# k-sheridan/ekf_vio

Hardware: AMD Instinct MI355X
Metric: filter steps/sec (predict+update) (higher is better)
Workload: dtype f32

## Files before the change

### ekf_vio_amd/capi.py

```python
import ctypes as C
import os

from . import _build

OK, EINVAL, ENUMERIC, ECAPACITY, EDEVICE, ESTATE, EABORTED = range(7)
_ERR = {EINVAL: "EKFVIO_EINVAL", ENUMERIC: "EKFVIO_ENUMERIC", ECAPACITY: "EKFVIO_ECAPACITY",
        EDEVICE: "EKFVIO_EDEVICE", ESTATE: "EKFVIO_ESTATE", EABORTED: "EKFVIO_EABORTED"}
PREDICT_STRUCTURED, PREDICT_DENSE = 0, 1


class Config(C.Structure):
    _fields_ = [("max_features", C.c_int32), ("default_point_depth", C.c_float),
                ("default_point_depth_variance", C.c_float), ("default_point_homogenous_variance", C.c_float),
                ("predict_mode", C.c_int32), ("klt_window_size", C.c_int32), ("klt_max_pyramid_level", C.c_int32),
                ("klt_max_iterations", C.c_int32), ("klt_epsilon", C.c_float), ("klt_min_eigen", C.c_float),
                ("kill_pad", C.c_int32), ("max_image_width", C.c_int32), ("max_image_height", C.c_int32),
                ("use_principal_point", C.c_int32), ("inverse_image_scale", C.c_int32), ("fast_threshold", C.c_int32),
                ("min_new_feature_dist", C.c_int32), ("fast_blur_sigma", C.c_float), ("replenish", C.c_int32),
                ("sample_based_uncertainty", C.c_int32), ("use_imu", C.c_int32), ("imu_gyro_variance", C.c_float),
                ("imu_accel_variance", C.c_float), ("gravity", C.c_float * 3),
                ("klt_fb_max_px", C.c_float), ("remove_lost", C.c_int32)]


class EkfvioError(RuntimeError):
    def __init__(self, code, msg=""):
        super().__init__("%s %s" % (_ERR.get(code, str(code)), msg))
        self.code = code


SYMBOLS = ["ekfvio_default_config", "ekfvio_create", "ekfvio_destroy", "ekfvio_reset", "ekfvio_last_error",
           "ekfvio_add_features", "ekfvio_process", "ekfvio_linearize", "ekfvio_update", "ekfvio_measurement_map",
           "ekfvio_num_features", "ekfvio_dim", "ekfvio_get_base_mu", "ekfvio_get_features", "ekfvio_get_sigma",
           "ekfvio_get_feature_cov", "ekfvio_get_depth_variance", "ekfvio_set_feature_cov", "ekfvio_metric2pixel_map",
           "ekfvio_pixel2metric_map", "ekfvio_get_odometry", "ekfvio_get_points", "ekfvio_check_sigma", "ekfvio_set_state",
           "ekfvio_remove_features", "ekfvio_klt_push_frame", "ekfvio_klt_track", "ekfvio_klt_track_points", "ekfvio_klt_get_level",
           "ekfvio_klt_uncertainty_points", "ekfvio_step_image", "ekfvio_replenish", "ekfvio_fast_detect", "ekfvio_imu", "ekfvio_imu_update",
           "ekfvio_upload_measurements", "ekfvio_run_uploaded", "ekfvio_synchronize", "ekfvio_profile_enable",
           "ekfvio_profile_reset", "ekfvio_profile_count", "ekfvio_profile_name", "ekfvio_profile_get",
           "ekfvio_profile_update_gemms", "ekfvio_get_counters", "ekfvio_set_gate", "ekfvio_get_gate",
           "ekfvio_set_klt_fb", "ekfvio_get_klt_fb", "ekfvio_klt_track_points_fb", "ekfvio_set_distortion", "ekfvio_rectify_map"]
HOOK_SYMBOLS = ["ekfvio_test_klt_padded_level", "ekfvio_test_blurred_level0", "ekfvio_test_gemm", "ekfvio_test_gemm_bench", "ekfvio_test_potrf_stamps",
                "ekfvio_test_sweep_stamps", "ekfvio_test_sweep_fault", "ekfvio_test_sweep_delay", "ekfvio_test_cholesky_solve", "ekfvio_test_plan", "ekfvio_test_persist_grid", "ekfvio_test_t2_pair",
                "ekfvio_test_gemm_plan", "ekfvio_test_predict_plan"]

_libs = {}


def lib_path():
    return _build.LIB_PATH


def load(build_if_missing=True, hooks=False):
    if hooks in _libs:
        return _libs[hooks]
    path = _build.HOOKS_LIB_PATH if hooks else _build.LIB_PATH
    if build_if_missing:
        _build.build(hooks=hooks)
    elif not os.path.exists(path):
        raise FileNotFoundError(path + " not built; run python -m ekf_vio_amd._build")
    lib = C.CDLL(path)
    vp, i32, f32 = C.c_void_p, C.c_int32, C.c_float
    fp, u8p, ip = C.POINTER(C.c_float), C.POINTER(C.c_uint8), C.POINTER(C.c_int32)
    sig = {
        "ekfvio_default_config": [C.POINTER(Config)],
        "ekfvio_create": [C.POINTER(Config), C.c_int, vp, C.POINTER(vp)],
        "ekfvio_destroy": [vp], "ekfvio_reset": [vp],
        "ekfvio_add_features": [vp, fp, i32], "ekfvio_process": [vp, f32], "ekfvio_linearize": [vp, f32, fp],
        "ekfvio_update": [vp, fp, fp, u8p, i32], "ekfvio_measurement_map": [vp, u8p, i32, ip, ip],
        "ekfvio_num_features": [vp], "ekfvio_dim": [vp], "ekfvio_get_base_mu": [vp, fp],
        "ekfvio_get_features": [vp, fp, fp, u8p], "ekfvio_get_sigma": [vp, fp, i32],
        "ekfvio_get_feature_cov": [vp, i32, fp], "ekfvio_get_depth_variance": [vp, i32, fp],
        "ekfvio_set_feature_cov": [vp, i32, fp], "ekfvio_metric2pixel_map": [fp, fp], "ekfvio_pixel2metric_map": [fp, fp],
        "ekfvio_get_odometry": [vp, fp, fp, fp, fp], "ekfvio_get_points": [vp, fp, fp],
        "ekfvio_check_sigma": [vp, fp, fp], "ekfvio_set_state": [vp, i32, fp, fp, fp, u8p, fp, i32],
        "ekfvio_remove_features": [vp, u8p, i32, ip],
        "ekfvio_klt_push_frame": [vp, u8p, i32, i32, i32, fp], "ekfvio_klt_track": [vp, fp, fp, u8p],
        "ekfvio_klt_track_points": [vp, fp, fp, i32, fp, u8p],
        "ekfvio_klt_uncertainty_points": [vp, fp, fp, i32, fp],
        "ekfvio_klt_get_level": [vp, i32, ip, ip, u8p, C.POINTER(C.c_int16)],
        "ekfvio_step_image": [vp, C.c_double, u8p, i32, i32, i32, fp], "ekfvio_imu": [vp, C.c_double, fp, fp], "ekfvio_imu_update": [vp, fp, fp],
        "ekfvio_replenish": [vp, ip, ip], "ekfvio_fast_detect": [vp, i32, i32, i32, ip, ip, ip],
        "ekfvio_upload_measurements": [vp, i32, fp, fp, u8p], "ekfvio_run_uploaded": [vp, i32, i32, f32],
        "ekfvio_synchronize": [vp], "ekfvio_profile_enable": [vp, i32], "ekfvio_profile_reset": [vp],
        "ekfvio_profile_count": [], "ekfvio_profile_name": [i32],
        "ekfvio_profile_get": [vp, i32, C.POINTER(C.c_double), C.POINTER(C.c_int64), C.POINTER(C.c_double)],
        "ekfvio_profile_update_gemms": [vp, i32, C.POINTER(C.c_double), C.POINTER(C.c_double)],
        "ekfvio_get_counters": [vp, C.POINTER(C.c_int64)],
        "ekfvio_set_gate": [vp, f32], "ekfvio_get_gate": [vp, fp, u8p, ip, ip, C.POINTER(C.c_int64)],
        "ekfvio_set_klt_fb": [vp, f32], "ekfvio_get_klt_fb": [vp, fp, u8p, ip, ip, C.POINTER(C.c_int64)],
        "ekfvio_klt_track_points_fb": [vp, fp, fp, i32, fp, u8p, fp, fp, u8p],
        "ekfvio_set_distortion": [vp, C.POINTER(C.c_double), i32],
        "ekfvio_rectify_map": [fp, C.POINTER(C.c_double), i32, i32, i32, ip, ip],
    }
    if hooks:
        sig.update({
            "ekfvio_test_klt_padded_level": [vp, i32, ip, u8p, C.POINTER(C.c_int16)],
            "ekfvio_test_blurred_level0": [vp, u8p],
            "ekfvio_test_gemm": [vp, i32, i32, i32, i32, f32, fp, i32, fp, i32, f32, fp, i32, i32],
            "ekfvio_test_cholesky_solve": [vp, i32, i32, fp, fp, fp, fp, ip],
            "ekfvio_test_potrf_stamps": [vp, C.POINTER(C.c_int64)],
            "ekfvio_test_sweep_stamps": [vp, C.c_int, C.POINTER(C.c_int64)],
            "ekfvio_test_sweep_fault": [vp, i32, i32],
            "ekfvio_test_sweep_delay": [vp, i32, i32, i32],
            "ekfvio_test_gemm_bench": [vp, i32, i32, i32, i32, i32, i32, i32, C.POINTER(C.c_double)],
            "ekfvio_test_plan": [i32] * 8 + [f32, ip],
            "ekfvio_test_persist_grid": [i32] * 8 + [f32, ip, i32, ip],
            "ekfvio_test_t2_pair": [i32, ip],
            "ekfvio_test_gemm_plan": [i32] * 11 + [ip],
            "ekfvio_test_predict_plan": [i32] * 5 + [ip],
        })
    for name, args in sig.items():
        fn = getattr(lib, name)
        fn.argtypes = args
        fn.restype = C.c_int
    lib.ekfvio_last_error.argtypes = [vp]
    lib.ekfvio_last_error.restype = C.c_char_p
    lib.ekfvio_profile_name.restype = C.c_char_p
    _libs[hooks] = lib
    return lib
```

### ekf_vio_amd/csrc/api.hip

```cpp
#include <math.h>
#include <stdio.h>
#include <string.h>

#include <algorithm>
#include <atomic>
#include <chrono>

#include <unistd.h>

#include "common.h"

namespace {
template <class T>
hipError_t dev_alloc(hipStream_t s, T** p, size_t count) {
    hipError_t e = hipMalloc((void**)p, sizeof(T) * (count ? count : 1));
    if (e == hipSuccess) e = hipMemsetAsync(*p, 0, sizeof(T) * (count ? count : 1), s);
    return e;
}

__global__ void init_sigma_kernel(float* P, int ld) {
    int i = threadIdx.x;
    if (i >= 7 && i <= 15) P[(size_t)i * ld + i] = 30.f;
    if (i >= 16 && i <= 21) P[(size_t)i * ld + i] = 0.5f;
}
// ... 122 lines not shown
    c->imu_gyro_variance = 1e-4f;
    c->imu_accel_variance = 1e-2f;
    c->gravity[0] = 0.f;
    c->gravity[1] = 9.81f;
    c->gravity[2] = 0.f;
    c->klt_fb_max_px = 0.f;
    c->remove_lost = 0;
    return EKFVIO_OK;
}

static int create_body(ekfvio_filter* f, const ekfvio_config* cfg, int device, void* stream) {
    HIP_TRY(f, hipSetDevice(device));
    if (stream) {
        f->stream = (hipStream_t)stream;
    } else {
        HIP_TRY(f, hipStreamCreateWithFlags(&f->stream, hipStreamNonBlocking));
        f->own_stream = true;
    }
    const int maxf = cfg->max_features;
    const FilterDims dims = filter_dims(maxf);
    f->n_cap = dims.n_cap, f->ldp = dims.ldp, f->m_cap = dims.m_cap, f->ld_aug = dims.ld_aug, f->sweep_sync_words = dims.sweep_sync_words;
    f->tune = tuning_from_env();
    const size_t pp = (size_t)f->ldp * f->ldp, pm = (size_t)f->ldp * f->m_cap;
    HIP_TRY(f, dev_alloc(f->stream, &f->mu, f->ldp));
    HIP_TRY(f, dev_alloc(f->stream, &f->mu_next, f->ldp));
    HIP_TRY(f, dev_alloc(f->stream, &f->last_klt, 2 * (size_t)maxf));
    HIP_TRY(f, dev_alloc(f->stream, &f->del_flag, (size_t)maxf));
    HIP_TRY(f, dev_alloc(f->stream, &f->P, pp));
    HIP_TRY(f, dev_alloc(f->stream, &f->P2, pp));
    HIP_TRY(f, dev_alloc(f->stream, &f->FA, EKF_BASE * EKF_BASE));
    HIP_TRY(f, dev_alloc(f->stream, &f->FB, 27 * (size_t)maxf));
    HIP_TRY(f, dev_alloc(f->stream, &f->FD, 9 * (size_t)maxf));
    HIP_TRY(f, dev_alloc(f->stream, &f->Fdense, pp));
    HIP_TRY(f, dev_alloc(f->stream, &f->idx, (size_t)f->m_cap));
    HIP_TRY(f, dev_alloc(f->stream, &f->inv_idx, (size_t)f->ldp));
    HIP_TRY(f, dev_alloc(f->stream, &f->zmeas, 2 * (size_t)maxf));
    HIP_TRY(f, dev_alloc(f->stream, &f->Rmeas, 4 * (size_t)maxf));
    HIP_TRY(f, dev_alloc(f->stream, &f->pass, (size_t)maxf));
    HIP_TRY(f, dev_alloc(f->stream, &f->yres, (size_t)f->m_cap));
    HIP_TRY(f, dev_alloc(f->stream, &f->Rm, 2 * (size_t)f->m_cap));
    HIP_TRY(f, dev_alloc(f->stream, &f->Saug, (size_t)f->ld_aug * f->m_cap));
    HIP_TRY(f, dev_alloc(f->stream, &f->Laug, (size_t)f->ld_aug * f->m_cap));
    HIP_TRY(f, dev_alloc(f->stream, &f->Linv, 64 * (size_t)f->m_cap));
    HIP_TRY(f, dev_alloc(f->stream, &f->Lsign, (size_t)(f->m_cap / 64 > 256 ? f->m_cap / 64 : 256)));
    HIP_TRY(f, dev_alloc(f->stream, &f->sweep_sync, f->sweep_sync_words));
    {
        hipDeviceProp_t prop;
        HIP_TRY(f, hipGetDeviceProperties(&prop, device));
        f->num_cus = prop.multiProcessorCount;
    }
    HIP_TRY(f, dev_alloc(f->stream, &f->Km, pm));
    HIP_TRY(f, dev_alloc(f->stream, &f->Wt, pm));
    HIP_TRY(f, dev_alloc(f->stream, &f->Gm, pm));
    HIP_TRY(f, dev_alloc(f->stream, &f->info, 4));
    HIP_TRY(f, dev_alloc(f->stream, &f->remove_words, 4));
    HIP_TRY(f, hipHostMalloc((void**)&f->h_info, 16 * sizeof(int), hipHostMallocMapped | hipHostMallocCoherent));
    memset(f->h_info, 0, 16 * sizeof(int));
    HIP_TRY(f, hipHostGetDevicePointer((void**)&f->d_hinfo, f->h_info, 0));
    {
        const size_t words = EKF_BASE + 4 * (size_t)(f->cfg.max_features > 0 ? f->cfg.max_features : 1);
        HIP_TRY(f, hipHostMalloc((void**)&f->h_out, words * sizeof(float), hipHostMallocMapped | hipHostMallocCoherent));
        HIP_TRY(f, hipHostGetDevicePointer((void**)&f->d_out, f->h_out, 0));
    }
    {
        const size_t cap = (size_t)(f->cfg.max_features > 0 ? f->cfg.max_features : 1);
        HIP_TRY(f, hipHostMalloc((void**)&f->h_meas, 25 * cap, hipHostMallocDefault));
        HIP_TRY(f, hipMalloc((void**)&f->d_meas, 25 * cap));
    }
    HIP_TRY(f, hipEventCreate(&f->ev0));
    HIP_TRY(f, hipEventCreate(&f->ev1));
    int rc = klt_alloc(f);
    if (rc != EKFVIO_OK) return rc;
    rc = fast_alloc(f);
    if (rc != EKFVIO_OK) return rc;
    return ekfvio_reset(f);
}

}

static std::atomic<int>* live_registry() {
    static std::atomic<int>* reg = [] {
        char name[64], val[32];
        snprintf(name, sizeof(name), "EKFVIO_LIVE_HANDLES_%ld", (long)getpid());
        if (const char* e = getenv(name)) {
            void* p = nullptr;
            if (sscanf(e, "%p", &p) == 1 && p) return static_cast<std::atomic<int>*>(p);
        }
        auto* a = new std::atomic<int>[64];
        for (int i = 0; i < 64; i++) a[i].store(0, std::memory_order_relaxed);
        snprintf(val, sizeof(val), "%p", static_cast<void*>(a));
        setenv(name, val, 1);
        return a;
    }();
    return reg;
}
int live_handles_on(int device) { return (device >= 0 && device < 64) ? live_registry()[device].load(std::memory_order_relaxed) : 2; }

extern "C" {

int ekfvio_create(const ekfvio_config* cfg, int device, void* stream, ekfvio_filter** out) {
    if (!out) return EKFVIO_EINVAL;
    *out = nullptr;
    if (!cfg || cfg->max_features < 0) return EKFVIO_EINVAL;
    if (cfg->remove_lost != 0 && cfg->remove_lost != 1) return EKFVIO_EINVAL;
    if (cfg->remove_lost && (size_t)cfg->max_features * 17 > 64 * 1024) return EKFVIO_ECAPACITY;
    if (!(cfg->klt_fb_max_px >= 0.f)) return EKFVIO_EINVAL;
    int ndev = 0;
    if (hipGetDeviceCount(&ndev) != hipSuccess || device < 0 || device >= ndev) return EKFVIO_EDEVICE;
    ekfvio_filter* f = new ekfvio_filter();
    f->cfg = *cfg;
    f->device = device;
    if (device < 64) live_registry()[device].fetch_add(1, std::memory_order_relaxed);
    const int rc = create_body(f, cfg, device, stream);
    if (rc != EKFVIO_OK) {
        fprintf(stderr, "ekfvio_create: %s\n", f->last_error.c_str());
        (void)ekfvio_destroy(f);
        return rc;
    }
    *out = f;
    return EKFVIO_OK;
}

int ekfvio_destroy(ekfvio_filter* f) {
    if (!f) return EKFVIO_EINVAL;
    (void)hipSetDevice(f->device);
    if (f->stream) (void)hipStreamSynchronize(f->stream);
    void* ptrs[] = {f->mu, f->mu_next, f->last_klt, f->del_flag, f->P,  f->P2, f->FA, f->FB, f->FD,   f->Fdense,
                    f->idx, f->inv_idx, f->zmeas,  f->Rmeas,    f->pass,     f->yres, f->Rm, f->Saug,  f->Laug,  f->Linv, f->Lsign, f->Km, f->sweep_sync, f->sweep_dbg,
                    f->Wt,  f->Gm,     f->info,     f->remove_words, f->seq_z,    f->seq_R, f->seq_pass, f->gate_words, f->fb_words};
    for (void* p : ptrs)
        if (p) hipFree(p);
    if (f->h_info) hipHostFree(f->h_info);
    if (f->h_out) hipHostFree(f->h_out);
    if (f->h_meas) hipHostFree(f->h_meas);
    if (f->d_meas) (void)hipFree(f->d_meas);
    klt_free(f);
    fast_free(f);
    drop_graph(f);
    if (f->ev0) hipEventDestroy(f->ev0);
    if (f->ev1) hipEventDestroy(f->ev1);
    if (f->own_stream && f->stream) hipStreamDestroy(f->stream);
    if (f->device >= 0 && f->device < 64) live_registry()[f->device].fetch_sub(1, std::memory_order_relaxed);
    delete f;
    return EKFVIO_OK;
}

const char* ekfvio_last_error(const ekfvio_filter* f) {
    return f ? f->last_error.c_str() : "null handle (a failed ekfvio_create leaves none behind: its return code says why)";
}

int ekfvio_reset(ekfvio_filter* f) {
    if (!f) return EKFVIO_EINVAL;
    f->out_fresh = false;
    HIP_TRY(f, hipSetDevice(f->device));
    f->N = 0;
    f->n = EKF_BASE;
    HIP_TRY(f, hipMemsetAsync(f->P, 0, sizeof(float) * (size_t)f->ldp * f->ldp, f->stream));
    HIP_TRY(f, hipMemsetAsync(f->P2, 0, sizeof(float) * (size_t)f->ldp * f->ldp, f->stream));
    HIP_TRY(f, hipMemsetAsync(f->mu, 0, sizeof(float) * f->ldp, f->stream));
    const float one = 1.f;
    HIP_TRY(f, hipMemcpyAsync(f->mu + 3, &one, sizeof(float), hipMemcpyHostToDevice, f->stream));
    hipLaunchKernelGGL(init_sigma_kernel, dim3(1), dim3(32), 0, f->stream, f->P, f->ldp);
    HIP_TRY(f, hipMemsetAsync(f->info, 0, 4 * sizeof(int), f->stream));
    if (f->gate_words) HIP_TRY(f, hipMemsetAsync(f->gate_words, 0, 4 * sizeof(int), f->stream));
    if (f->fb_words) HIP_TRY(f, hipMemsetAsync(f->fb_words, 0, 8 * sizeof(int), f->stream));
    HIP_TRY(f, hipStreamSynchronize(f->stream));
    f->have_stamp = false;
    f->frames[0].valid = f->frames[1].valid = false;
    return EKFVIO_OK;
}

int ekfvio_add_features(ekfvio_filter* f, const float* uv, int32_t count) {
    if (!f || count < 0 || (count > 0 && !uv)) return EKFVIO_EINVAL;
    f->out_fresh = false;
    if (count == 0) return EKFVIO_OK;
    if (f->N + count > f->cfg.max_features) return EKFVIO_ECAPACITY;
    HIP_TRY(f, hipSetDevice(f->device));
    HIP_TRY(f, hipMemcpyAsync(f->zmeas, uv, sizeof(float) * 2 * count, hipMemcpyHostToDevice, f->stream));
    return add_features_device(f, count);
}

int ekfvio_process(ekfvio_filter* f, float dt) {
// ... 654 lines not shown
    long long* dst;
    HIP_TRY(f, dev_alloc(f->stream, &dS, hs.size()));
    HIP_TRY(f, dev_alloc(f->stream, &dL, hs.size()));
    HIP_TRY(f, dev_alloc(f->stream, &dLi, 4096));
    HIP_TRY(f, dev_alloc(f->stream, &dst, 80));
    HIP_TRY(f, hipMemsetAsync(dst, 0, sizeof(long long) * 80, f->stream));
    HIP_TRY(f, hipMemcpyAsync(dS, hs.data(), sizeof(float) * hs.size(), hipMemcpyHostToDevice, f->stream));
    for (int rep = 0; rep < 3; rep++) launch_potrf_stamps(f, dS, 64, dL, dLi, dst);
    HIP_TRY(f, hipMemcpyAsync(stamps, dst, sizeof(long long) * 80, hipMemcpyDeviceToHost, f->stream));
    std::vector<uint32_t> hl(64 * 64), hi(4096);
    HIP_TRY(f, hipMemcpyAsync(hl.data(), dL, sizeof(float) * hl.size(), hipMemcpyDeviceToHost, f->stream));
    HIP_TRY(f, hipMemcpyAsync(hi.data(), dLi, sizeof(float) * hi.size(), hipMemcpyDeviceToHost, f->stream));
    HIP_TRY(f, hipStreamSynchronize(f->stream));
    uint64_t h1 = 1469598103934665603ull, h2 = h1;
    for (uint32_t v : hl) h1 = (h1 ^ v) * 1099511628211ull;
    for (uint32_t v : hi) h2 = (h2 ^ v) * 1099511628211ull;
    stamps[12] = (int64_t)h1;
    stamps[13] = (int64_t)h2;
    hipFree(dS); hipFree(dL); hipFree(dLi); hipFree(dst);
    return EKFVIO_OK;
}

int ekfvio_test_sweep_stamps(ekfvio_filter* f, int enable, int64_t* stamps ) {
    if (!f) return EKFVIO_EINVAL;
    HIP_TRY(f, hipSetDevice(f->device));
    if (enable && !f->sweep_dbg) {
        HIP_TRY(f, dev_alloc(f->stream, &f->sweep_dbg, 1024));
        HIP_TRY(f, hipMemsetAsync(f->sweep_dbg, 0, 1024 * sizeof(long long), f->stream));
    }
    if (stamps && f->sweep_dbg) {
        HIP_TRY(f, hipMemcpyAsync(stamps, f->sweep_dbg, 1024 * sizeof(long long), hipMemcpyDeviceToHost, f->stream));
        HIP_TRY(f, hipStreamSynchronize(f->stream));
    }
    return EKFVIO_OK;
}

int ekfvio_test_sweep_fault(ekfvio_filter* f, int32_t spin_limit, int32_t stall_workgroup) {
    if (!f || spin_limit < 0) return EKFVIO_EINVAL;
    f->sweep_spin_limit = spin_limit;
    f->sweep_stall_wg = stall_workgroup;
    drop_graph(f);
    return EKFVIO_OK;
}

int ekfvio_test_sweep_delay(ekfvio_filter* f, int32_t workgroup, int32_t point, int32_t ticks) {
    if (!f || (point != 0 && point != 1) || ticks < 0 || ticks > EKFVIO_TEST_SWEEP_DELAY_MAX_TICKS) return EKFVIO_EINVAL;
    f->sweep_delay_wg = workgroup >= 0 ? workgroup : -1;
    f->sweep_delay_point = point;
    f->sweep_delay_ticks = ticks;
    drop_graph(f);
    return EKFVIO_OK;
}

int ekfvio_test_cholesky_solve(ekfvio_filter* f, int32_t m, int32_t nrhs, const float* S, const float* Crhs,
                               float* L_out, float* X_out, int32_t* info) {
    if (!f || m <= 0 || nrhs <= 0 || !S || !Crhs) return EKFVIO_EINVAL;
    HIP_TRY(f, hipSetDevice(f->device));
    const int mp = round_up(m, 64), rp = round_up(nrhs, 64);
    const int ld = mp + rp + mp;
    std::vector<float> hs((size_t)ld * mp, 0.f);
    for (int c = 0; c < mp; c++) {
        for (int r = 0; r < mp; r++) hs[(size_t)c * ld + r] = (r < m && c < m) ? S[(size_t)c * m + r] : (r == c ? 1.f : 0.f);
        if (c < m)
            for (int r = 0; r < nrhs; r++) hs[(size_t)c * ld + mp + r] = Crhs[(size_t)c * nrhs + r];
        hs[(size_t)c * ld + mp + rp + c] = 1.f;
    }
    float *dS, *dL, *dLi, *dK, *dW;
    HIP_TRY(f, dev_alloc(f->stream, &dS, hs.size()));
    HIP_TRY(f, dev_alloc(f->stream, &dL, hs.size()));
    HIP_TRY(f, dev_alloc(f->stream, &dLi, (size_t)64 * mp));
    HIP_TRY(f, dev_alloc(f->stream, &dK, (size_t)rp * mp));
    HIP_TRY(f, dev_alloc(f->stream, &dW, (size_t)rp * mp));
    HIP_TRY(f, hipMemcpyAsync(dS, hs.data(), sizeof(float) * hs.size(), hipMemcpyHostToDevice, f->stream));
    UpdatePlan plan = plan_raw_sweep(f->tune, plan_shape(f), mp, rp);
    launch_chol_sweep(f, plan, dS, dL, dLi, ld, plan.persistent() && !f->sweep_flags_clean);
    if (plan.persistent()) f->sweep_flags_clean = false;
    std::vector<unsigned long long> hsign(mp / 64);
    HIP_TRY(f, hipMemcpyAsync(hsign.data(), f->Lsign, sizeof(unsigned long long) * hsign.size(), hipMemcpyDeviceToHost, f->stream));
    HIP_TRY(f, hipStreamSynchronize(f->stream));
    int refine = 1;
    for (unsigned long long v : hsign) refine &= (v == 0ull);
    if (refine) plan.gain = GAIN_GEMM;
    launch_gain_from_sweep(f, plan, dL, ld, nrhs, dK, dW, rp, refine);
    std::vector<float> hl(hs.size()), hk((size_t)rp * mp);
    HIP_TRY(f, hipMemcpyAsync(hl.data(), dL, sizeof(float) * hl.size(), hipMemcpyDeviceToHost, f->stream));
    HIP_TRY(f, hipMemcpyAsync(hk.data(), dK, sizeof(float) * hk.size(), hipMemcpyDeviceToHost, f->stream));
    if (info) {
        HIP_TRY(f, hipMemcpyAsync(info, f->info, sizeof(int), hipMemcpyDeviceToHost, f->stream));
        HIP_TRY(f, hipMemsetAsync(f->info, 0, sizeof(int), f->stream));
    }
    HIP_TRY(f, hipStreamSynchronize(f->stream));
    if (const char* dp = getenv("EKFVIO_DEBUG_DUMP_LAUG")) {
        if (FILE* fp = fopen(dp, "wb")) {
            const int hdr[3] = {ld, mp, rp};
            fwrite(hdr, sizeof(int), 3, fp);
            fwrite(hl.data(), sizeof(float), hl.size(), fp);
            fclose(fp);
        }
    }
    if (L_out)
        for (int c = 0; c < m; c++)
            for (int r = 0; r < m; r++) L_out[(size_t)c * m + r] = (r >= c) ? hl[(size_t)c * ld + r] : 0.f;
    if (X_out)
        for (int c = 0; c < m; c++)
            for (int r = 0; r < nrhs; r++) X_out[(size_t)c * nrhs + r] = hk[(size_t)c * rp + r];
    hipFree(dS);
// ... 77 lines not shown
```

### ekf_vio_amd/csrc/chol.hip

```cpp
#include "common.h"

#include <type_traits>

namespace {

typedef float f32x16 __attribute__((ext_vector_type(16)));
typedef float f32x4 __attribute__((ext_vector_type(4)));

#define PB 64
#ifndef PLD
#define PLD 68
#endif
#define ILD 17
#define INV_LDS (4 * 16 * ILD)

__device__ __forceinline__ float lane_bcast(float v, int src_lane) {
    return __int_as_float(__builtin_amdgcn_readlane(__float_as_int(v), src_lane));
}
__device__ __forceinline__ double lane_bcast_d(double v, int src_lane) {
    const int lo = __builtin_amdgcn_readlane(__double2loint(v), src_lane);
    const int hi = __builtin_amdgcn_readlane(__double2hiint(v), src_lane);
    return __hiloint2double(hi, lo);
}

// ... 830 lines not shown
    for (int c = 0; c < PB; c++)
        if ((neg >> c) & 1ull) {
            float* p = L + (size_t)(blockIdx.y * PB + c) * ldl + row0 + r;
            *p = -*p;
        }
}


#define SWEEP_SPIN_LIMIT (1 << 30)
#define SWEEP_WAIT_TICKS_UNRECOVERABLE 10000000

#include "chol_persist.inc"
#include "chol_step_la.inc"

}

#ifdef EKFVIO_TEST_HOOKS
void launch_potrf_stamps(ekfvio_filter* f, const float* S, int ld, float* L, float* Linv, long long* d_stamps) {
    const char* e = getenv("EKFVIO_POTRF_FV");
    const int fv = e ? atoi(e) : EKF_POTRF_FV;
    auto kern = fv == 0 ? potrf64_stamp_kernel<0> : fv == 10 ? potrf64_stamp_kernel<10> : fv == 12 ? potrf64_stamp_kernel<12>
              : fv == 13 ? potrf64_stamp_kernel<13> : potrf64_stamp_kernel<8>;
    const char* w = getenv("EKFVIO_POTRF_WARM");
    hipLaunchKernelGGL(kern, dim3(1), dim3(256), 0, f->stream, S, ld, L, ld, Linv, d_stamps, (w && atoi(w)) ? 2 : 1);
}
#endif

#define EKF_GATHER_POTRF_LDS (84 * 1024)
void launch_gather_potrf(ekfvio_filter* f, const UpdatePlan& p) {
    if (!f->gather_attr_set) {
        (void)hipFuncSetAttribute(reinterpret_cast<const void*>(gather_potrf_kernel), hipFuncAttributeMaxDynamicSharedMemorySize,
                                  EKF_GATHER_POTRF_LDS);
        f->gather_attr_set = true;
    }
    GatherArgs ga = make_gather_args(f, p);
    if (p.persistent()) {
        ga.zero_words = f->sweep_sync;
        ga.n_zero = (int)persist_flag_words(p.m_pad, p.n_pad);
    }
    const int nb2 = p.with_wt ? (p.m_pad / 64) * (f->ldp / 64) : 0;
    hipLaunchKernelGGL(gather_potrf_kernel, dim3(1 + ga.nb1 + nb2), dim3(256), EKF_GATHER_POTRF_LDS, f->stream, ga, f->Laug, f->ld_aug,
                       f->Linv, f->info, f->Lsign, f->sweep_dbg);
}

static PersistArgs persist_args(ekfvio_filter* f, const UpdatePlan& p, float* L, int ldl, float* K, int ldk, float* S = nullptr,
                                float* Linv = nullptr) {
    PersistArgs pa = PersistArgs();
    const PersistGrid g = persist_grid(p, f->ldp);
    const PersistFlags fl(p.m_pad, p.n_pad);
    const int mb = g.mb, nX = g.nX;
    pa.L = L, pa.ldl = ldl, pa.mb = mb, pa.idb0 = mb + nX, pa.grid = g;
    pa.K = K, pa.ldk = ldk, pa.Lsign = f->Lsign;
    pa.Sg = f->P, pa.ldsg = f->ldp, pa.T2 = t2_buffer(f), pa.ldt = f->ldp, pa.nstate = f->n;
    if (!S) return pa;
    pa.S = S, pa.lds = ldl, pa.Linv = Linv, pa.info = f->info;
    pa.ready = f->sweep_sync + fl.ready(), pa.fin = f->sweep_sync + fl.fin(), pa.pan = f->sweep_sync + fl.pan(), pa.abort_flag = f->sweep_sync + fl.abort_word();
    pa.dbg = f->sweep_dbg;
    pa.bound.spin_limit = f->sweep_spin_limit > 0 ? f->sweep_spin_limit : SWEEP_SPIN_LIMIT;
    pa.bound.wait_ticks = p.recoverable ? f->tune.sweep_wait_ticks : std::max(f->tune.sweep_wait_ticks, SWEEP_WAIT_TICKS_UNRECOVERABLE);
    pa.early_sources = f->tune.persist_early;
    pa.stall_wg = f->sweep_stall_wg >= 0 ? g.owner_block(f->sweep_stall_wg - 1) : -1;
#ifdef EKFVIO_TEST_HOOKS
    pa.delay_wg = f->sweep_delay_wg >= 0 ? g.owner_block(f->sweep_delay_wg - 1) : -1;
    pa.delay_point = f->sweep_delay_point, pa.delay_ticks = f->sweep_delay_ticks;
#endif
    return pa;
}

#define EKF_PERSIST_FUSED_DYN_LDS (28 * 1024)
const int* launch_persist_fused(ekfvio_filter* f, const UpdatePlan& p, bool zero_flags) {
    const int m_pad = p.m_pad, n_pad = p.n_pad;
    ProfScope ps(f, PC_CHOL, (double)m_pad * m_pad * m_pad / 3.0 + (double)(n_pad + m_pad / 2) * m_pad * m_pad);
    if (!f->persist_attr_set) {
        (void)hipFuncSetAttribute(reinterpret_cast<const void*>(chol_persist_kernel), hipFuncAttributeMaxDynamicSharedMemorySize,
                                  EKF_PERSIST_FUSED_DYN_LDS);
        f->persist_attr_set = true;
    }
    PersistArgs pa = persist_args(f, p, f->Laug, f->ld_aug, f->Km, f->ldp, f->Saug, f->Linv);
    pa.gain = p.gain == GAIN_SWEEP, pa.t2 = p.t2_by_sweep;
    if (zero_flags) (void)hipMemsetAsync(f->sweep_sync, 0, sizeof(int) * persist_flag_words(m_pad, n_pad), f->stream);
    hipLaunchKernelGGL(chol_persist_kernel, dim3(pa.grid.total()), dim3(256), EKF_PERSIST_FUSED_DYN_LDS,
                       f->stream, pa, make_gather_args(f, p));
    f->persistent_sweeps++;
    return pa.abort_flag;
}

const int* launch_chol_sweep(ekfvio_filter* f, const UpdatePlan& p, float* Saug, float* Laug, float* Linv, int ld, bool zero_flags) {
    const int m_pad = p.m_pad, n_pad = p.n_pad;
    const bool schur = p.sweep == SWEEP_SCHUR, split = p.sweep == SWEEP_SPLIT || p.sweep == SWEEP_SPLIT_LA;
    ProfScope ps(f, PC_CHOL, (double)m_pad * m_pad * m_pad / 3.0 + (double)(n_pad + m_pad / 2) * m_pad * m_pad +
                                 (schur ? (double)n_pad * n_pad * m_pad + (double)n_pad * m_pad * m_pad : 0.0));
    const int mb = m_pad / PB, idb0 = mb + n_pad / PB;
    const int rb = n_pad / PB + mb;
    if (!p.fused_gather)
        hipLaunchKernelGGL(potrf64_kernel, dim3(1), dim3(256), 0, f->stream, Saug, ld, Laug, ld, Linv, f->info, f->Lsign);
    if (p.sweep == SWEEP_PERSIST) {
        const PersistArgs pa = persist_args(f, p, Laug, ld, nullptr, 0, Saug, Linv);
        if (zero_flags) (void)hipMemsetAsync(f->sweep_sync, 0, sizeof(int) * persist_flag_words(m_pad, n_pad), f->stream);
        hipLaunchKernelGGL(chol_persist_kernel, dim3(pa.grid.total()), dim3(256), 0, f->stream, pa, GatherArgs());
        f->persistent_sweeps++;
        return pa.abort_flag;
    }
    SchurArgs sc;
    if (schur) {
        f->schur_sweeps++;
        sc.P = f->P, sc.ldp = f->ldp, sc.K = f->Km, sc.ldk = f->ldp, sc.nb = n_pad / PB;
// ... 43 lines not shown
}

__global__ __launch_bounds__(256) void joseph_g_kernel(float* __restrict__ K, int ldk, const float* __restrict__ T, int ldp,
                                                       const int* __restrict__ idx, const float* __restrict__ Rm,
                                                       const float* __restrict__ zrow, const float* __restrict__ mu, int m,
                                                       const int* __restrict__ m_dev, float* __restrict__ G, int ldg,
                                                       float* __restrict__ Kyp) {
    __shared__ float s_t[64 * 65];
    __shared__ float s_part[4][64];
    if (m_dev) m = *m_dev;
    const int rl = threadIdx.x & 63, ph = threadIdx.x >> 6;
    const int i0 = blockIdx.x * 64, c0 = blockIdx.y * 64;
    const int i = i0 + rl;
    float kq[16], kp[16];
#pragma unroll
    for (int u = 0; u < 16; u++) {
        const int q = c0 + ph + 4 * u;
        kq[u] = K[(size_t)q * ldk + i];
        kp[u] = K[(size_t)(q ^ 1) * ldk + i];
    }
    {
        const int q = c0 + rl;
        const int sq = (q < m) ? idx[q] : 0;
        float tv[16];
#pragma unroll
        for (int u = 0; u < 16; u++) tv[u] = T[(size_t)(i0 + ph + 4 * u) * ldp + sq];
#pragma unroll
        for (int u = 0; u < 16; u++) s_t[(ph + 4 * u) * 65 + rl] = tv[u];
    }
    __syncthreads();
    float acc = 0.f;
#pragma unroll
    for (int u = 0; u < 16; u++) {
        const int q = c0 + ph + 4 * u;
        const float a = (fabsf(kq[u]) > EKF_FLUSH_THRESH) ? kq[u] : 0.f;
        const float b = (fabsf(kp[u]) > EKF_FLUSH_THRESH) ? kp[u] : 0.f;
        K[(size_t)q * ldk + i] = a;
        float g = 0.f;
        if (q < m) {
            const float x = a * Rm[2 * q], y = b * Rm[2 * (q ^ 1) + 1];
            const float kr = ((q ^ 1) < q) ? (y + x) : (x + y);
            g = kr - s_t[rl * 65 + ph + 4 * u];
            acc = acc + a * (zrow[q] - mu[idx[q]]);
        }
        G[(size_t)q * ldg + i] = g;
    }
    s_part[ph][rl] = acc;
    __syncthreads();
    if (ph == 0) Kyp[(size_t)blockIdx.y * ldg + i] = ((s_part[0][rl] + s_part[1][rl]) + s_part[2][rl]) + s_part[3][rl];
}

void launch_gain2_tiles(ekfvio_filter* f, const UpdatePlan& p) {
    const int m_pad = p.m_pad, n_pad = p.n_pad;
    ProfScope ps(f, PC_SOLVE, 2.0 * n_pad * (double)m_pad * m_pad + (double)n_pad * n_pad * m_pad);
    const PersistArgs pa = persist_args(f, p, f->Laug, f->ld_aug, f->Km, f->ldp);
    const int gain_wgs = pa.grid.nX * pa.mb;
    const int total = gain_wgs + t2_pairs(pa.grid.nX);
    const int dyn = total <= f->num_cus ? 30 * 1024 : 0;
    if (dyn && !f->gain2_attr_set) {
        (void)hipFuncSetAttribute(reinterpret_cast<const void*>(gain2_t2_tiles_kernel), hipFuncAttributeMaxDynamicSharedMemorySize, 30 * 1024);
        f->gain2_attr_set = true;
    }
    hipLaunchKernelGGL(gain2_t2_tiles_kernel, dim3(total), dim3(256), dyn, f->stream, pa, make_gather_args(f, p), gain_wgs);
}

void launch_joseph_g(ekfvio_filter* f, int m, int m_pad, int n_pad, bool m_on_device, const float* T) {
    ProfScope ps(f, PC_SOLVE, 3.0 * n_pad * (double)m_pad);
    hipLaunchKernelGGL(joseph_g_kernel, dim3(n_pad / 64, m_pad / 64), dim3(256), 0, f->stream, f->Km, f->ldp, T ? T : f->P, f->ldp, f->idx,
                       f->Rm, f->yres, f->mu, m, m_on_device ? f->info + 2 : nullptr, f->Gm, f->ldp, f->Wt);
}

void launch_gain_from_sweep(ekfvio_filter* f, const UpdatePlan& p, const float* Laug, int ld, int n, float* K, float* scratch, int ldk, int refine) {
    const int m_pad = p.m_pad, n_pad = p.n_pad;
    ProfScope ps(f, PC_SOLVE, (refine ? 3.0 : 1.0) * n * (double)m_pad * m_pad);
    if (p.gain == GAIN_TILES) {
        const PersistArgs pa = persist_args(f, p, const_cast<float*>(Laug), ld, K, ldk);
        hipLaunchKernelGGL(gain_tiles_kernel, dim3((n_pad / PB) * pa.mb), dim3(256), 0, f->stream, pa);
        return;
    }
    const float* Lf = Laug;
    const float* Y = Laug + m_pad;
    const float* LinvT = Laug + m_pad + n_pad;
    GemmCall g;
    g.M = n, g.N = g.K = m_pad, g.transB = true, g.lowerB = true;
    g.A = Y, g.lda = ld, g.B = LinvT, g.ldb = ld, g.C = K, g.ldc = ldk, g.flush = !refine;
    launch_gemm(f, g);
    if (refine) {
        GemmCall r = g;
        r.transB = false, r.alpha = -1.f, r.A = K, r.lda = ldk, r.B = Lf, r.beta = 1.f, r.Cin = Y, r.ldcin = ld, r.C = scratch, r.flush = false;
        launch_gemm(f, r);
        g.A = scratch, g.lda = ldk, g.beta = 1.f, g.Cin = K, g.ldcin = ldk, g.flush = true;
        launch_gemm(f, g);
    }
}
```

### ekf_vio_amd/csrc/chol_persist.inc

```

#ifndef PERSIST_POLL_SLEEP_LAZY
#define PERSIST_POLL_SLEEP_LAZY 12
#endif
#ifndef PERSIST_POLL_SLEEP
#define PERSIST_POLL_SLEEP 2
#endif

struct PollBound {
    int spin_limit, wait_ticks;
};
struct PersistArgs {
    float* S;
    int lds;
    float* L;
    int ldl;
    float* Linv;
    int mb, idb0;
    int* info;
    unsigned long long* Lsign;
    int* ready;
    int* fin;
    int* abort_flag;
    long long* dbg;
    PersistGrid grid;
    int gain;
    float* K;
    int ldk;
    int* pan;
    int early_sources;
    PollBound bound;
    int stall_wg;
    int t2;
    const float* Sg;
    int ldsg;
    float* T2;
    int ldt;
    int nstate;
#ifdef EKFVIO_TEST_HOOKS
    int delay_wg;
    int delay_point;
    int delay_ticks;
#endif
};

typedef unsigned int u32x4 __attribute__((ext_vector_type(4)));
__device__ __forceinline__ __amdgpu_buffer_rsrc_t persist_rsrc(const float* p, unsigned floats) {
    return __builtin_amdgcn_make_buffer_rsrc(const_cast<float*>(p), 0, floats * 4u, 0x00020000);
}
__device__ __forceinline__ float4 ld_sc1(__amdgpu_buffer_rsrc_t b, unsigned off) {
    const f32x4 v = __builtin_bit_cast(f32x4, __builtin_amdgcn_raw_buffer_load_b128(b, off * 4u, 0, 16));
    return make_float4(v[0], v[1], v[2], v[3]);
}
__device__ __forceinline__ void st_sc1(__amdgpu_buffer_rsrc_t b, unsigned off, float4 q) {
    const f32x4 v = {q.x, q.y, q.z, q.w};
    __builtin_amdgcn_raw_buffer_store_b128(__builtin_bit_cast(u32x4, v), b, off * 4u, 0, 16);
}
__device__ __forceinline__ void wait_vm0() { asm volatile("s_waitcnt vmcnt(0)" ::: "memory"); }

struct RegTile {
    float4 v[4];
    __device__ __forceinline__ void request(__amdgpu_buffer_rsrc_t b, unsigned base, int ld, int tid) {
#pragma unroll
        for (int it = 0; it < 4; it++) {
            const int e = tid + it * 256;
            v[it] = ld_sc1(b, base + (unsigned)(e >> 4) * (unsigned)ld + (unsigned)(e & 15) * 4u);
        }
    }
    __device__ __forceinline__ void put(float* T, int tid) const {
#pragma unroll
        for (int it = 0; it < 4; it++) {
            const int e = tid + it * 256;
            *reinterpret_cast<float4*>(T + (e >> 4) * PLD + (e & 15) * 4) = v[it];
        }
    }
};
__device__ __forceinline__ void inv_put(float4 v, float* Tinv, int tid) {
    const int p = tid >> 6, c = (tid >> 2) & 15, r4 = (tid & 3) * 4;
    float* t = Tinv + p * 16 * ILD + c * ILD + r4;
    t[0] = v.x; t[1] = v.y; t[2] = v.z; t[3] = v.w;
}
__device__ __forceinline__ void load_tile_sc1(float* T, __amdgpu_buffer_rsrc_t b, unsigned base, int ld, int tid) {
    RegTile t;
    t.request(b, base, ld, tid);
    t.put(T, tid);
}
__device__ __forceinline__ void load_inv_sc1(float* Tinv, __amdgpu_buffer_rsrc_t b, unsigned base, int tid) {
    inv_put(ld_sc1(b, base + tid * 4), Tinv, tid);
}
template <bool LOWER>
__device__ __forceinline__ void store_tile_sc1(const float* T, __amdgpu_buffer_rsrc_t b, unsigned base, int ld, int tid) {
#pragma unroll
    for (int it = 0; it < 4; it++) {
        const int e = tid + it * 256;
        const int c = e >> 4, r4 = (e & 15) * 4;
        const float4 q = *reinterpret_cast<const float4*>(T + c * PLD + r4);
// ... 102 lines not shown
    const __amdgpu_buffer_rsrc_t bL = persist_rsrc(a.L, (unsigned)ldl * (unsigned)(mb * PB));
    float kv[16];
#pragma unroll
    for (int q = 0; q < 16; q++) kv[q] = 0.f;
    const int iy = mb + ib, iz = a.idb0 + cb;
    for (int kb = cb; kb < mb; kb++) {
        bool signed_last = false;
        unsigned long long negl = 0ull;
        if (kb == mb - 1) {
            const __amdgpu_buffer_rsrc_t bS = persist_rsrc(a.S, (unsigned)a.lds * (unsigned)(mb * PB));
            const __amdgpu_buffer_rsrc_t bI = persist_rsrc(a.Linv, (unsigned)(mb * PB * PB));
            const bool zi = a.grid.compact() && cb == kb;
            persist_wait(a, nullptr, a.fin + iy * mb + kb, zi ? nullptr : a.fin + iz * mb + kb, tid, 1, true);
            load_tile_sc1(Ti, bS, (unsigned)(kb * PB) * (unsigned)a.lds + (unsigned)(iy * PB), a.lds, tid);
            if (zi) identity_tile(Tj, tid);
            else load_tile_sc1(Tj, bS, (unsigned)(kb * PB) * (unsigned)a.lds + (unsigned)(iz * PB), a.lds, tid);
            persist_wait(a, a.ready + kb, nullptr, nullptr, tid, 4, false);
            load_tile_sc1(Tl, bL, (unsigned)(kb * PB) * (unsigned)ldl + (unsigned)(kb * PB), ldl, tid);
            load_inv_sc1(Tinv, bI, (unsigned)(kb * PB * PB), tid);
            negl = ld_sign_sc1(a.Lsign + kb);
            __syncthreads();
            tri_solve_fwd2(Ti, Tj, Tl, Tinv, wave, lane);
            if (a.dbg && tid == 0 && ib * mb + cb < 104) a.dbg[400 + ib * mb + cb] = (long long)__builtin_amdgcn_s_memrealtime();
            signed_last = negl != 0ull;
        } else {
            persist_wait(a, nullptr, a.pan + iy * mb + kb, a.pan + iz * mb + kb, tid, 1, true);
            load_tile_sc1(Ti, bL, (unsigned)(kb * PB) * (unsigned)ldl + (unsigned)(iy * PB), ldl, tid);
            load_tile_sc1(Tj, bL, (unsigned)(kb * PB) * (unsigned)ldl + (unsigned)(iz * PB), ldl, tid);
        }
        __syncthreads();
        const f32x16 up = signed_last ? mma64_signed(Ti, 1, PLD, Tj, 1, PLD, wr, wc, lane, negl) : mma64(Ti, 1, PLD, Tj, 1, PLD, wr, wc, lane);
#pragma unroll
        for (int q = 0; q < 16; q++) kv[q] = kv[q] + up[q];
    }
    float* Kt = a.K + (size_t)(cb * PB) * a.ldk + (size_t)ib * PB;
#pragma unroll
    for (int q = 0; q < 16; q++) {
        const int c = mma64_col(wc, lane, q);
        Kt[(size_t)c * a.ldk + r] = (fabsf(kv[q]) > EKF_FLUSH_THRESH) ? kv[q] : 0.f;
    }
}

__device__ __forceinline__ void sign_cols(float* dst, const float* src, unsigned long long neg, int tid) {
#pragma unroll
    for (int it = 0; it < 4; it++) {
        const int e = tid + it * 256;
        const int c = e >> 4, r4 = (e & 15) * 4;
        const float sg = ((neg >> c) & 1ull) ? -1.f : 1.f;
        const float4 v = *reinterpret_cast<const float4*>(src + c * PLD + r4);
        *reinterpret_cast<float4*>(dst + c * PLD + r4) = make_float4(sg * v.x, sg * v.y, sg * v.z, sg * v.w);
    }
}

template <bool WAIT>
__device__ __forceinline__ void gain_tile2(const PersistArgs& a, const GatherArgs& ga, float* Ti, float* Tj, float* Tl, float* Tinv, float* Th, float* tab,
                                           int ib, int cb, int tid) {
    const int lane = tid & 63, wave = tid >> 6, wr = wave & 1, wc = wave >> 1;
    const int r = wr * 32 + (lane & 31);
    const int mb = a.mb, ldl = a.ldl;
    const int m = ga.m_dev ? *ga.m_dev : ga.m;
    const __amdgpu_buffer_rsrc_t bL = persist_rsrc(a.L, (unsigned)ldl * (unsigned)(mb * PB));
    const __amdgpu_buffer_rsrc_t bS = persist_rsrc(a.S, (unsigned)a.lds * (unsigned)(mb * PB));
    const int iy = mb + ib, iz = a.idb0 + cb;
    const int cq = cb * PB + lane;
    const int sq = (cq < m) ? ga.idx[cq] : -1;
    const unsigned sqc = (unsigned)max(sq, 0);
    int alo = 0, ahi = -1;
    if (cb * PB < m) {
        alo = ga.idx[cb * PB] / PB;
        ahi = ga.idx[min(cb * PB + PB - 1, m - 1)] / PB;
    }
    if (tid < 64) {
        float yq = 0.f, rd = 0.f, ro = 0.f;
        if (sq >= 0) {
            yq = ga.zrow[cq] - ga.mu[sq];
            rd = ga.Rm[2 * cq];
            ro = ga.Rm[2 * (cq ^ 1) + 1];
        }
        tab[tid] = yq, tab[64 + tid] = rd, tab[128 + tid] = ro;
    }
    auto column_flags = [&](int kb, const int* zflag) -> PollLane {
        const int ax = alo + tid - 2;
        return {tid == 0 ? a.pan + iy * mb + kb : tid == 1 ? zflag : (tid >= 2 && ax <= ahi) ? a.pan + (mb + ax) * mb + kb : nullptr, 1};
    };
    float kv[16], w2[16];
    {
        float wv[16];
        const int scl = max(sq, 0);
#pragma unroll
        for (int ps = 0; ps < 16; ps++) wv[ps] = ga.P[(size_t)min(ib * PB + wave + 4 * ps, ga.n - 1) * ga.ld + scl];
#pragma unroll
        for (int ps = 0; ps < 16; ps++) asm volatile("" : "+v"(wv[ps]));
#pragma unroll
        for (int ps = 0; ps < 16; ps++) Th[(wave + 4 * ps) * 65 + lane] = (sq >= 0 && ib * PB + wave + 4 * ps < ga.n) ? wv[ps] : 0.f;
        __syncthreads();
#pragma unroll
        for (int q = 0; q < 16; q++) {
            kv[q] = 0.f;
            w2[q] = Th[r * 65 + mma64_col(wc, lane, q)];
        }
    }
    auto fetch = [&](int kb) -> unsigned long long {
        const bool gk = kb >= cb;
        float hv[16];
        unsigned long long neg;
        if constexpr (WAIT) {
            persist_wait(a, column_flags(kb, gk ? a.pan + iz * mb + kb : nullptr), tid, kb < mb - 2);
            load_tile_sc1(Ti, bL, (unsigned)(kb * PB) * (unsigned)ldl + (unsigned)(iy * PB), ldl, tid);
            if (gk) load_tile_sc1(Tj, bL, (unsigned)(kb * PB) * (unsigned)ldl + (unsigned)(iz * PB), ldl, tid);
#pragma unroll
            for (int ps = 0; ps < 16; ps++)
                hv[ps] = __builtin_bit_cast(float, __builtin_amdgcn_raw_buffer_load_b32(bL, ((unsigned)(kb * PB + wave + 4 * ps) * (unsigned)ldl + (unsigned)(mb * PB) + sqc) * 4u, 0, 16));
#pragma unroll
            for (int ps = 0; ps < 16; ps++) hv[ps] = (sq >= 0) ? hv[ps] : 0.f;
#pragma unroll
            for (int ps = 0; ps < 16; ps++) Th[(wave + 4 * ps) * PLD + lane] = hv[ps];
            neg = ld_sign_sc1(a.Lsign + kb);
        } else {
            load_tile(Ti, a.L + (size_t)kb * PB * ldl + (size_t)iy * PB, ldl, tid);
            if (gk) load_tile(Tj, a.L + (size_t)kb * PB * ldl + (size_t)iz * PB, ldl, tid);
#pragma unroll
            for (int ps = 0; ps < 16; ps++) hv[ps] = a.L[(size_t)(kb * PB + wave + 4 * ps) * ldl + (size_t)(mb * PB) + sqc];
#pragma unroll
            for (int ps = 0; ps < 16; ps++) hv[ps] = (sq >= 0) ? hv[ps] : 0.f;
#pragma unroll
            for (int ps = 0; ps < 16; ps++) Th[(wave + 4 * ps) * PLD + lane] = hv[ps];
            neg = a.Lsign[kb];
        }
        return neg;
    };
    auto products = [&](int kb, unsigned long long neg, bool z_unsigned) {
        if (kb >= cb) {
            const f32x16 up = (z_unsigned && neg != 0ull) ? mma64_signed(Ti, 1, PLD, Tj, 1, PLD, wr, wc, lane, neg) : mma64(Ti, 1, PLD, Tj, 1, PLD, wr, wc, lane);
#pragma unroll
            for (int q = 0; q < 16; q++) kv[q] = kv[q] + up[q];
        }
        if (alo <= ahi) {
            f32x16 up;
            if constexpr (WAIT) {
                up = (neg == 0ull) ? mma64(Ti, 1, PLD, Th, 1, PLD, wr, wc, lane) : mma64_signed(Ti, 1, PLD, Th, 1, PLD, wr, wc, lane, neg);
            } else {
                if (__builtin_amdgcn_readfirstlane((int)(neg != 0ull))) {
                    __syncthreads();
                    sign_cols(Ti, Ti, neg, tid);
                    __syncthreads();
                }
                up = mma64(Ti, 1, PLD, Th, 1, PLD, wr, wc, lane);
            }
#pragma unroll
            for (int q = 0; q < 16; q++) w2[q] = w2[q] - up[q];
        }
        if (WAIT && a.dbg && tid == 0 && mb <= 8 && (ib == 0 || ib == 6) && (cb == 0 || cb == 3 || cb == 7))
            a.dbg[100 + 8 * ((ib ? 3 : 0) + (cb == 0 ? 0 : cb == 3 ? 1 : 2)) + kb] = (long long)__builtin_amdgcn_s_memrealtime();
    };
    if constexpr (WAIT) {
        for (int kb = 0; kb < mb - 2; kb++) {
            __syncthreads();
            const unsigned long long neg = fetch(kb);
            __syncthreads();
            products(kb, neg, false);
        }
    } else {
        for (int kb = 0; kb < mb; kb++) {
            __syncthreads();
            const unsigned long long neg = fetch(kb);
            __syncthreads();
            products(kb, neg, false);
        }
    }
    if constexpr (WAIT) {
        const int kl = mb - 1, k6 = mb - 2;
        const bool gk6 = k6 >= cb;
        const __amdgpu_buffer_rsrc_t bI = persist_rsrc(a.Linv, (unsigned)(mb * PB * PB));
        const bool zi = a.grid.compact() && cb == kl;
        __syncthreads();
        persist_wait(a, column_flags(k6, gk6 ? a.pan + iz * mb + k6 : (zi ? nullptr : a.fin + iz * mb + kl)), tid, false);
        RegTile ql, qi, qj;
        float hq[16];
        unsigned long long neg6;
        {
            RegTile pi6, pj6;
            float h6[16];
            pi6.request(bL, (unsigned)(k6 * PB) * (unsigned)ldl + (unsigned)(iy * PB), ldl, tid);
            if (gk6) pj6.request(bL, (unsigned)(k6 * PB) * (unsigned)ldl + (unsigned)(iz * PB), ldl, tid);
#pragma unroll
            for (int ps = 0; ps < 16; ps++)
                h6[ps] = __builtin_bit_cast(float, __builtin_amdgcn_raw_buffer_load_b32(bL, ((unsigned)(k6 * PB + wave + 4 * ps) * (unsigned)ldl + (unsigned)(mb * PB) + sqc) * 4u, 0, 16));
            neg6 = ld_sign_sc1(a.Lsign + k6);
            pi6.put(Ti, tid);
            if (gk6) pj6.put(Tj, tid);
#pragma unroll
            for (int ps = 0; ps < 16; ps++) Th[(wave + 4 * ps) * PLD + lane] = (sq >= 0) ? h6[ps] : 0.f;
        }
        persist_wait(a, a.ready + kl, nullptr, nullptr, tid, 4, false);
        ql.request(bL, (unsigned)(kl * PB) * (unsigned)ldl + (unsigned)(kl * PB), ldl, tid);
        qi.request(bS, (unsigned)(kl * PB) * (unsigned)a.lds + (unsigned)(iy * PB), a.lds, tid);
        if (!zi) qj.request(bS, (unsigned)(kl * PB) * (unsigned)a.lds + (unsigned)(iz * PB), a.lds, tid);
        const float4 qv = ld_sc1(bI, (unsigned)(kl * PB * PB) + tid * 4);
        const unsigned long long neg7 = ld_sign_sc1(a.Lsign + kl);
#pragma unroll
        for (int ps = 0; ps < 16; ps++)
            hq[ps] = __builtin_bit_cast(float, __builtin_amdgcn_raw_buffer_load_b32(bS, ((unsigned)(kl * PB + wave + 4 * ps) * (unsigned)a.lds + (unsigned)(mb * PB) + sqc) * 4u, 0, 16));
        products(mb - 2, neg6, false);
        __syncthreads();
        ql.put(Tl, tid);
        qi.put(Ti, tid);
        if (zi) identity_tile(Tj, tid);
        else qj.put(Tj, tid);
        inv_put(qv, Tinv, tid);
#pragma unroll
        for (int ps = 0; ps < 16; ps++) Th[(wave + 4 * ps) * PLD + lane] = (sq >= 0) ? hq[ps] : 0.f;
        __syncthreads();
        float* const t3[3] = {Ti, Tj, Th};
        tri_solve_fwd_n<3>(t3, Tl, Tinv, wave, lane);
        __syncthreads();
        products(kl, neg7, true);
    }
#pragma unroll
    for (int q = 0; q < 16; q++) kv[q] = (fabsf(kv[q]) > EKF_FLUSH_THRESH) ? kv[q] : 0.f;
    float* Kt = a.K + (size_t)(cb * PB) * a.ldk + (size_t)ib * PB;
    float* Gt = ga.G + (size_t)(cb * PB) * ga.ld + (size_t)ib * PB;
    float acc = 0.f;
#pragma unroll
    for (int q = 0; q < 16; q++) {
        const int c = mma64_col(wc, lane, q), cg = cb * PB + c;
        Kt[(size_t)c * a.ldk + r] = kv[q];
        float g = 0.f;
        if (cg < m) {
            const float x = kv[q] * tab[64 + c], y = kv[q ^ 1] * tab[128 + c];
            const float kr = ((cg ^ 1) < cg) ? (y + x) : (x + y);
            g = kr - w2[q];
            acc = acc + kv[q] * tab[c];
        }
        Gt[(size_t)c * ga.ld + r] = g;
    }
    __syncthreads();
    float* part = Th;
    part[(wc * 2 + (lane >> 5)) * 64 + r] = acc;
    __syncthreads();
    if (tid < 64) ga.Wt[(size_t)cb * ga.ld + (size_t)ib * PB + tid] = ((part[tid] + part[64 + tid]) + part[128 + tid]) + part[192 + tid];
}

template <bool WAIT>
__device__ __forceinline__ void t2_tile(const PersistArgs& a, float* Ti, float* Tj, float* Tl, float* Tinv, int ta, int tb, int tid, long long* dbg = nullptr) {
    const int lane = tid & 63, wave = tid >> 6, wr = wave & 1, wc = wave >> 1;
    const int r = wr * 32 + (lane & 31);
    const int mb = a.mb, ldl = a.ldl;
    const bool diag = ta == tb;
    const __amdgpu_buffer_rsrc_t bL = persist_rsrc(a.L, (unsigned)ldl * (unsigned)(mb * PB));
    float tab[16], tba[16];
    {
        const float* sab = a.Sg + (size_t)tb * PB * a.ldsg + (size_t)ta * PB;
        const float* sba = a.Sg + (size_t)ta * PB * a.ldsg + (size_t)tb * PB;
#pragma unroll
        for (int q = 0; q < 16; q++) {
            const int c = mma64_col(wc, lane, q);
            tab[q] = sab[(size_t)c * a.ldsg + r];
            tba[q] = diag ? 0.f : sba[(size_t)c * a.ldsg + r];
        }
    }
    const int ia = mb + ta, ib = mb + tb;
    auto apply = [&](int kb, unsigned long long neg) {
        const float* Bj = diag ? Ti : Tj;
        f32x16 up;
        if constexpr (WAIT) {
            up = (neg == 0ull) ? mma64(Ti, 1, PLD, Bj, 1, PLD, wr, wc, lane) : mma64_signed(Ti, 1, PLD, Bj, 1, PLD, wr, wc, lane, neg);
        } else if (__builtin_amdgcn_readfirstlane((int)(neg != 0ull))) {
            sign_cols(Tl, Ti, neg, tid);
            __syncthreads();
            up = mma64(Tl, 1, PLD, Bj, 1, PLD, wr, wc, lane);
            __syncthreads();
        } else {
            up = mma64(Ti, 1, PLD, Bj, 1, PLD, wr, wc, lane);
        }
#pragma unroll
        for (int q = 0; q < 16; q++) tab[q] = tab[q] - up[q];
        if (!diag) {
#pragma unroll
            for (int q = 0; q < 16; q++) Tl[r * PLD + mma64_col(wc, lane, q)] = up[q];
            __syncthreads();
#pragma unroll
            for (int q = 0; q < 16; q++) tba[q] = tba[q] - Tl[mma64_col(wc, lane, q) * PLD + r];
        }
        if (dbg && tid == 0) dbg[kb] = (long long)__builtin_amdgcn_s_memrealtime();
    };
    if constexpr (WAIT) {
        for (int kb = 0; kb < mb - 2; kb++) {
            __syncthreads();
            persist_wait(a, nullptr, a.pan + ia * mb + kb, diag ? nullptr : a.pan + ib * mb + kb, tid, 1, true);
            load_tile_sc1(Ti, bL, (unsigned)(kb * PB) * (unsigned)ldl + (unsigned)(ia * PB), ldl, tid);
            if (!diag) load_tile_sc1(Tj, bL, (unsigned)(kb * PB) * (unsigned)ldl + (unsigned)(ib * PB), ldl, tid);
            const unsigned long long neg = ld_sign_sc1(a.Lsign + kb);
            __syncthreads();
            apply(kb, neg);
        }
    } else {
        for (int kb = 0; kb < mb; kb++) {
            __syncthreads();
            load_tile(Ti, a.L + (size_t)kb * PB * ldl + (size_t)ia * PB, ldl, tid);
            if (!diag) load_tile(Tj, a.L + (size_t)kb * PB * ldl + (size_t)ib * PB, ldl, tid);
            const unsigned long long neg = a.Lsign[kb];
            __syncthreads();
            apply(kb, neg);
        }
    }
    if constexpr (WAIT) {
        const int kl = mb - 1, k6 = mb - 2;
        const __amdgpu_buffer_rsrc_t bS = persist_rsrc(a.S, (unsigned)a.lds * (unsigned)(mb * PB));
        const __amdgpu_buffer_rsrc_t bI = persist_rsrc(a.Linv, (unsigned)(mb * PB * PB));
        __syncthreads();
        persist_wait(a, a.ready + kl, a.pan + ia * mb + k6, diag ? nullptr : a.pan + ib * mb + k6, tid, 4, false);
        RegTile pi6, pj6, ql, qi, qj;
        pi6.request(bL, (unsigned)(k6 * PB) * (unsigned)ldl + (unsigned)(ia * PB), ldl, tid);
        if (!diag) pj6.request(bL, (unsigned)(k6 * PB) * (unsigned)ldl + (unsigned)(ib * PB), ldl, tid);
        const unsigned long long neg6 = ld_sign_sc1(a.Lsign + k6);
        ql.request(bL, (unsigned)(kl * PB) * (unsigned)ldl + (unsigned)(kl * PB), ldl, tid);
        qi.request(bS, (unsigned)(kl * PB) * (unsigned)a.lds + (unsigned)(ia * PB), a.lds, tid);
        if (!diag) qj.request(bS, (unsigned)(kl * PB) * (unsigned)a.lds + (unsigned)(ib * PB), a.lds, tid);
        const float4 qv = ld_sc1(bI, (unsigned)(kl * PB * PB) + tid * 4);
        const unsigned long long neg7 = ld_sign_sc1(a.Lsign + kl);
        pi6.put(Ti, tid);
        if (!diag) pj6.put(Tj, tid);
        __syncthreads();
        apply(k6, neg6);
        __syncthreads();
        ql.put(Tl, tid);
        qi.put(Ti, tid);
        if (!diag) qj.put(Tj, tid);
        inv_put(qv, Tinv, tid);
        __syncthreads();
        if (diag) tri_solve_fwd(Ti, Tl, Tinv, wave, lane);
        else tri_solve_fwd2(Ti, Tj, Tl, Tinv, wave, lane);
        __syncthreads();
        apply(kl, neg7);
    }
    __syncthreads();
#pragma unroll
    for (int q = 0; q < 16; q++) {
        const int c = mma64_col(wc, lane, q);
        Ti[c * PLD + r] = (ta * PB + r < a.nstate && tb * PB + c < a.nstate) ? tab[q] : 0.f;
        if (!diag) Tj[c * PLD + r] = (tb * PB + r < a.nstate && ta * PB + c < a.nstate) ? tba[q] : 0.f;
    }
    __syncthreads();
    store_tile(Ti, a.T2 + (size_t)tb * PB * a.ldt + (size_t)ta * PB, a.ldt, tid);
    if (!diag) store_tile(Tj, a.T2 + (size_t)ta * PB * a.ldt + (size_t)tb * PB, a.ldt, tid);
    if (dbg && tid == 0) dbg[15] = (long long)__builtin_amdgcn_s_memrealtime();
}

template <bool SC1>
__device__ __forceinline__ float persist_ldf(const float* p) {
    if constexpr (SC1) return __hip_atomic_load(p, __ATOMIC_RELAXED, __HIP_MEMORY_SCOPE_AGENT);
    else return *p;
}
template <bool SC1>
__device__ __forceinline__ void persist_tile_x(f32x4 (&x)[4], const float* G, int ld, int wave, int lane) {
    const int li = lane & 15, g = lane >> 4;
#pragma unroll
    for (int b = 0; b < 4; b++)
#pragma unroll
        for (int v = 0; v < 4; v++) x[b][v] = persist_ldf<SC1>(G + (size_t)(16 * b + 4 * g + v) * ld + 16 * wave + li);
}
__device__ __forceinline__ void persist_diag_block(float* D, const float* P, int tr, int tc, int lane, unsigned long long neg) {
    const int li = lane & 15, lk = lane >> 4;
    const int rb = 16 * tr, cb = 16 * tc;
    const float* ap = P + rb + li + lk * PLD;
    const float* bp = P + cb + li + lk * PLD;
    f32x4 u = {0.f, 0.f, 0.f, 0.f};
    if (neg == 0ull) {
#pragma unroll
        for (int q = 0; q < PB; q += 4) u = __builtin_amdgcn_mfma_f32_16x16x4f32(bp[q * PLD], ap[q * PLD], u, 0, 0, 0);
    } else {
#pragma unroll 4
        for (int q = 0; q < PB; q += 4) {
            float av = ap[q * PLD];
            if ((neg >> (q + lk)) & 1ull) av = -av;
            u = __builtin_amdgcn_mfma_f32_16x16x4f32(bp[q * PLD], av, u, 0, 0, 0);
        }
    }
    float t[4];
#pragma unroll
    for (int gq = 0; gq < 4; gq++) t[gq] = D[(cb + 4 * lk + gq) * PLD + rb + li];
#pragma unroll
    for (int gq = 0; gq < 4; gq++) D[(cb + 4 * lk + gq) * PLD + rb + li] = t[gq] - u[gq];
}


struct GTile {
    int ia[16];
    int ib;
    float v[16], rd[16], ro[16];
};
__device__ __forceinline__ void gtile_idx(GTile& t, const GatherArgs& ga, int m, int rb, int cb, int mb, int idb0, int tid) {
    if (rb < mb) {
        const int c = cb * PB + (tid & 63);
        t.ib = (c < m) ? ga.idx[c] : 0;
#pragma unroll
        for (int ps = 0; ps < 16; ps++) {
            const int rc = max(min(rb * PB + (tid >> 6) + 4 * ps, m - 1), 0);
// ... 253 lines not shown
            seen = 1;
            if (k + 2 < mb && lane < 2)
                seen = __hip_atomic_load(lane == 0 ? a.fin + (i + 1) * mb + i : a.fin + (i + 1) * mb + (i + 1), __ATOMIC_RELAXED, __HIP_MEMORY_SCOPE_AGENT);
            if (bad) {
                __syncthreads();
                if (k >= kf) load_tile_sc1(Dn, bS, oii, lds, tid);
                else load_tile(Dn, S + oii, lds, tid);
                __syncthreads();
                const f32x16 up = (neg == 0ull) ? mma64(Ti, 1, PLD, Ti, 1, PLD, wr, wc, lane) : mma64_signed(Ti, 1, PLD, Ti, 1, PLD, wr, wc, lane, neg);
#pragma unroll
                for (int q = 0; q < 16; q++) {
                    const int c = mma64_col(wc, lane, q);
                    Dn[c * PLD + r] = Dn[c * PLD + r] - up[q];
                }
                neg1 = potrf64_signed(Dn, Tinv, tid);
            }
            store_tile_sc1<true>(Dn, bL, (unsigned)(i * PB) * (unsigned)ldl + (unsigned)(i * PB), ldl, tid);
            store_inv_sc1(Tinv, bI, (unsigned)(i * PB * PB), tid);
            if (tid == 0) {
                __hip_atomic_store(a.Lsign + i, neg1, __ATOMIC_RELAXED, __HIP_MEMORY_SCOPE_AGENT);
                if (bad) atomicOr(a.info, 1);
            }
            asm volatile("" ::: "memory");
            neg = neg1;
            float* t = Lk;
            Lk = Dn;
            Dn = t;
        }
        persist_publish_wave(a.ready + (mb - 1), lane);
        PSTAMP(32 + 8 * (mb - 1));
        if (a.dbg && tid == 0) a.dbg[897] = (long long)__builtin_amdgcn_s_memrealtime();
        PEXIT();
    }

    if (role.kind == ROLE_LEAD || role.kind == ROLE_LEAD_GATHER0) {
        if (!compact) gather_body<false>(ga, ga.nb1 + role.n, persist_dyn_lds);
        else if (role.kind == ROLE_LEAD_GATHER0) {
            const int cb = role.a;
            const int m = ga.m_dev ? *ga.m_dev : ga.m;
            GTile t;
            gtile_idx(t, ga, m, 1, cb, mb, a.idb0, tid);
            gtile_pin(t);
            gtile_val(t, ga, m, 1, cb, mb, a.idb0, tid);
            gtile_pinv(t);
            gtile_put(t, Tl, ga, m, 1, cb, mb, a.idb0, tid);
            __syncthreads();
            store_tile_sc1<false>(Tl, bS, (unsigned)(cb * PB) * (unsigned)lds + (unsigned)PB, lds, tid);
            persist_publish(a.fin + 1 * mb + cb, tid);
        }
        if (a.gain) {
            const int tb = role.n;
            __syncthreads();
            if (role.a < a.idb0 - mb) {
                if (a.t2) gain_tile2<true>(a, ga, Ti, Tj, Tl, Tinv, persist_dyn_lds, persist_dyn_lds + PB * PLD, role.a, role.b, tid);
                else gain_tile(a, Ti, Tj, Tl, Tinv, role.a, role.b, tid);
                if (a.dbg && tid == 0 && tb < 104) a.dbg[200 + tb] = (long long)__builtin_amdgcn_s_memrealtime();
            }
        }
        PEXIT();
    }
    const int idb0 = a.idb0;
    if (role.kind == ROLE_GATHER0) {
        const int cb = role.a;
        const int m = ga.m_dev ? *ga.m_dev : ga.m;
        GTile t;
        gtile_idx(t, ga, m, 1, cb, mb, idb0, tid);
        gtile_pin(t);
        gtile_val(t, ga, m, 1, cb, mb, idb0, tid);
        gtile_pinv(t);
        gtile_put(t, Tl, ga, m, 1, cb, mb, idb0, tid);
        __syncthreads();
        store_tile_sc1<false>(Tl, bS, (unsigned)(cb * PB) * (unsigned)lds + (unsigned)PB, lds, tid);
        persist_publish(a.fin + 1 * mb + cb, tid);
        PEXIT();
    }
    const int i = role.a, j = role.b, hidx = role.n;
    const int k0 = (i >= idb0) ? (i - idb0) : 0;
    const int klast = (i == j) ? j - 2 : j - 1;
    const unsigned oij = (unsigned)(j * PB) * (unsigned)lds + (unsigned)(i * PB);
    float tv[16];
    if (fused) {
        const int m = ga.m_dev ? *ga.m_dev : ga.m;
        const bool step0 = k0 == 0 && klast >= 0;
        GTile tn, ti_, tj_;
        gtile_idx(tn, ga, m, i, j, mb, idb0, tid);
        if (step0) {
            gtile_idx(ti_, ga, m, i, 0, mb, idb0, tid);
            if (i != j) gtile_idx(tj_, ga, m, j, 0, mb, idb0, tid);
        }
        gtile_pin(tn);
        if (step0) gtile_pin(ti_);
        gtile_val(tn, ga, m, i, j, mb, idb0, tid);
        if (step0) {
            gtile_val(ti_, ga, m, i, 0, mb, idb0, tid);
            if (i != j) gtile_val(tj_, ga, m, j, 0, mb, idb0, tid);
        }
        gtile_pinv(tn);
        gtile_put(tn, Tl, ga, m, i, j, mb, idb0, tid);
        if (step0) {
            gtile_put(ti_, Ti, ga, m, i, 0, mb, idb0, tid);
            if (i != j) gtile_put(tj_, Tj, ga, m, j, 0, mb, idb0, tid);
        }
        __syncthreads();
#pragma unroll
        for (int q = 0; q < 16; q++) tv[q] = Tl[mma64_col(wc, lane, q) * PLD + r];
        __syncthreads();
    } else {
// ... 42 lines not shown
        HSTAMP(2);
        if (i != j)
            tri_solve_fwd2(Ti, Tj, Tl, Tinv, wave, lane);
        else
            tri_solve_fwd(Ti, Tl, Tinv, wave, lane);
        __syncthreads();
        HSTAMP(3);
        const float* Bj = (i != j) ? Tj : Ti;
        const f32x16 up = (neg == 0ull) ? mma64(Ti, 1, PLD, Bj, 1, PLD, wr, wc, lane) : mma64_signed(Ti, 1, PLD, Bj, 1, PLD, wr, wc, lane, neg);
#pragma unroll
        for (int q = 0; q < 16; q++) tv[q] = tv[q] - up[q];
        HSTAMP(4);
    }
    k = klast;
    if (klast >= k0 || fused) {
        if (klast < k0) __syncthreads();
#pragma unroll
        for (int q = 0; q < 16; q++) Tl[mma64_col(wc, lane, q) * PLD + r] = tv[q];
        __syncthreads();
        PERSIST_TEST_DELAY(a, 0);
        store_tile_sc1<false>(Tl, bS, oij, lds, tid);
    }
    if ((int)blockIdx.x != a.stall_wg) persist_publish(a.fin + i * mb + j, tid);
    else __syncthreads();
    HSTAMP(5);
    if (a.dbg && tid == 0 && i < mb && (i == j + 1 || i == j)) a.dbg[(i == j ? 740 : 720) + j] = (long long)__builtin_amdgcn_s_memrealtime();
    if (klast >= k0 && i != j) {
        if (a.gain && i >= mb) {
            const unsigned od = (unsigned)(klast * PB) * (unsigned)ldl + (unsigned)(i * PB);
            PERSIST_TEST_DELAY(a, 1);
            if (neg != 0ull && i >= idb0) store_tile_signed_sc1(Ti, bL, od, ldl, tid, neg);
            else store_tile_sc1<false>(Ti, bL, od, ldl, tid);
            persist_publish(a.pan + i * mb + klast, tid);
        } else {
            float* dst = L + (size_t)klast * PB * ldl + (size_t)i * PB;
            if (neg != 0ull && i >= idb0) store_tile_signed(Ti, dst, ldl, tid, neg);
            else store_tile(Ti, dst, ldl, tid);
        }
    }
    if (a.t2) {
        const int p = a.grid.t2_pair_of(hidx);
        if (a.dbg && tid == 0 && hidx < 8) {
            a.dbg[192 + hidx] = (long long)__builtin_amdgcn_s_memrealtime();
        }
        if (p >= 0) {
            int ta, tb;
            t2_pair(p, ta, tb);
            long long* td = nullptr;
            const int np_ = t2_pairs(a.grid.nX);
            if (a.dbg && (p == 0 || p == np_ / 2 || p == np_ - 1)) {
                td = a.dbg + 840 + 16 * (p == 0 ? 0 : p == np_ - 1 ? 2 : 1);
                if (tid == 0) td[14] = (long long)__builtin_amdgcn_s_memrealtime();
            }
            t2_tile<true>(a, Ti, Tj, Tl, Tinv, ta, tb, tid, td);
            if (a.dbg && tid == 0 && p < 91) a.dbg[304 + p] = (long long)__builtin_amdgcn_s_memrealtime();
        }
        PEXIT();
    }
    if (j == mb - 1 && i >= mb) {
        if (i >= idb0 && i - idb0 > j) PEXIT();
        if (a.gain) PEXIT();
        persist_wait(a, a.ready + j, nullptr, nullptr, tid, 4, false);
        load_tile_sc1(Tj, bL, (unsigned)(j * PB) * (unsigned)ldl + (unsigned)(j * PB), ldl, tid);
        load_inv_sc1(Tinv, bI, (unsigned)(j * PB * PB), tid);
        const unsigned long long negl = ld_sign_sc1(a.Lsign + j);
        if (klast < k0) {
#pragma unroll
            for (int q = 0; q < 16; q++) Tl[mma64_col(wc, lane, q) * PLD + r] = tv[q];
        }
        __syncthreads();
        tri_solve_fwd(Tl, Tj, Tinv, wave, lane);
        __syncthreads();
        if (a.gain) {
            const unsigned od = (unsigned)(j * PB) * (unsigned)ldl + (unsigned)(i * PB);
            if (negl != 0ull && i >= idb0) store_tile_signed_sc1(Tl, bL, od, ldl, tid, negl);
            else store_tile_sc1<false>(Tl, bL, od, ldl, tid);
            persist_publish(a.pan + i * mb + j, tid);
        } else {
            float* dst = L + (size_t)j * PB * ldl + (size_t)i * PB;
            if (negl != 0ull && i >= idb0) store_tile_signed(Tl, dst, ldl, tid, negl);
            else store_tile(Tl, dst, ldl, tid);
        }
    }
    PEXIT();
#undef PEXIT
#undef HSTAMP
#undef PSTAMP
}

__global__ __launch_bounds__(256) void gain_tiles_kernel(PersistArgs a) {
    __shared__ __attribute__((aligned(16))) float Ti[PB * PLD];
    __shared__ __attribute__((aligned(16))) float Tj[PB * PLD];
    const int tid = threadIdx.x, lane = tid & 63, wave = tid >> 6, wr = wave & 1, wc = wave >> 1;
    const int r = wr * 32 + (lane & 31);
    const int mb = a.mb, ldl = a.ldl;
    const int ib = (int)blockIdx.x / mb, cb = (int)blockIdx.x % mb;
    const int iy = mb + ib, iz = a.idb0 + cb;
    float kv[16];
#pragma unroll
    for (int q = 0; q < 16; q++) kv[q] = 0.f;
#define GT_DECL(S) float4 ya##S##0, ya##S##1, ya##S##2, ya##S##3, za##S##0, za##S##1, za##S##2, za##S##3;
#define GT_REQ1(S, IT, KB)                                                                                                                    \
    ya##S##IT = *reinterpret_cast<const float4*>(a.L + (size_t)(KB) * PB * ldl + (size_t)iy * PB + (size_t)((tid + IT * 256) >> 4) * ldl + ((tid + IT * 256) & 15) * 4); \
    za##S##IT = *reinterpret_cast<const float4*>(a.L + (size_t)(KB) * PB * ldl + (size_t)iz * PB + (size_t)((tid + IT * 256) >> 4) * ldl + ((tid + IT * 256) & 15) * 4);
#define GT_REQ(S, KB) GT_REQ1(S, 0, KB) GT_REQ1(S, 1, KB) GT_REQ1(S, 2, KB) GT_REQ1(S, 3, KB)
#define GT_PUT1(S, IT)                                                                                        \
    *reinterpret_cast<float4*>(Ti + ((tid + IT * 256) >> 4) * PLD + ((tid + IT * 256) & 15) * 4) = ya##S##IT; \
    *reinterpret_cast<float4*>(Tj + ((tid + IT * 256) >> 4) * PLD + ((tid + IT * 256) & 15) * 4) = za##S##IT;
#define GT_STEP(S, KB)                                                      \
    do {                                                                    \
        __syncthreads();                                                    \
        GT_PUT1(S, 0) GT_PUT1(S, 1) GT_PUT1(S, 2) GT_PUT1(S, 3)             \
        __syncthreads();                                                    \
        if ((KB) + 2 < mb) { GT_REQ(S, (KB) + 2) }                          \
        const f32x16 up = mma64(Ti, 1, PLD, Tj, 1, PLD, wr, wc, lane);      \
        _Pragma("unroll") for (int q = 0; q < 16; q++) kv[q] = kv[q] + up[q]; \
    } while (0)
    GT_DECL(0)
    GT_DECL(1)
    GT_REQ(0, cb)
    if (cb + 1 < mb) { GT_REQ(1, cb + 1) }
    else { ya10 = ya11 = ya12 = ya13 = za10 = za11 = za12 = za13 = make_float4(0.f, 0.f, 0.f, 0.f); }
    for (int kb = cb; kb < mb; kb += 2) {
        GT_STEP(0, kb);
        if (kb + 1 < mb) GT_STEP(1, kb + 1);
    }
#undef GT_DECL
#undef GT_REQ1
#undef GT_REQ
#undef GT_PUT1
#undef GT_STEP
    float* Kt = a.K + (size_t)(cb * PB) * a.ldk + (size_t)ib * PB;
#pragma unroll
    for (int q = 0; q < 16; q++) {
        const int c = mma64_col(wc, lane, q);
        Kt[(size_t)c * a.ldk + r] = (fabsf(kv[q]) > EKF_FLUSH_THRESH) ? kv[q] : 0.f;
    }
}

__global__ __launch_bounds__(256) void gain2_t2_tiles_kernel(PersistArgs a, GatherArgs ga, int gain_wgs) {
    extern __shared__ float g2_dyn_lds[];
    __shared__ __attribute__((aligned(16))) float Ti[PB * PLD];
    __shared__ __attribute__((aligned(16))) float Tj[PB * PLD];
    __shared__ __attribute__((aligned(16))) float Th[PB * PLD];
    __shared__ float tab[192];
    if ((int)blockIdx.x < gain_wgs) {
        gain_tile2<false>(a, ga, Ti, Tj, nullptr, nullptr, Th, tab, (int)blockIdx.x / a.mb, (int)blockIdx.x % a.mb, threadIdx.x);
    } else {
        int ta, tb;
        t2_pair((int)blockIdx.x - gain_wgs, ta, tb);
        t2_tile<false>(a, Ti, Tj, Th, nullptr, ta, tb, threadIdx.x);
    }
}
```

### ekf_vio_amd/csrc/common.h

```cpp
#pragma once
#include <hip/hip_runtime.h>
#include <stdint.h>

#include <chrono>
#include <string>
#include <vector>

#include "../../include/ekfvio.h"
#include "plan.h"
#ifdef EKFVIO_TEST_HOOKS
#include "../../include/ekfvio_test_hooks.h"
#endif

#ifndef EKF_POTRF_FV
#define EKF_POTRF_FV 12
#endif
#define EKF_FLUSH_THRESH (1e-8f * 1e-5f)

#define HIP_TRY(f, expr)                                                           \
    do {                                                                           \
        hipError_t e__ = (expr);                                                   \
        if (e__ != hipSuccess) {                                                   \
            (f)->last_error = std::string(#expr) + ": " + hipGetErrorString(e__);  \
            return EKFVIO_EDEVICE;                                                 \
// ... 44 lines not shown

struct RectifyKey {
    float K[4];
    double D[5];
    int w, h;
};

struct ekfvio_filter {
    ekfvio_config cfg;
    int device = 0;
    hipStream_t stream = nullptr;
    bool own_stream = false;
    std::string last_error;

    int N = 0;
    int n = EKF_BASE;
    int n_cap = 0, ldp = 0, m_cap = 0;
    Tuning tune;

    float* mu = nullptr;
    float* mu_next = nullptr;
    float* last_klt = nullptr;
    uint8_t* del_flag = nullptr;
    float* P = nullptr;
    float* P2 = nullptr;
    float* FA = nullptr;
    float* FB = nullptr;
    float* FD = nullptr;
    float* Fdense = nullptr;
    int* idx = nullptr;
    int* inv_idx = nullptr;
    float* zmeas = nullptr;
    float* Rmeas = nullptr;
    uint8_t* pass = nullptr;
    float* yres = nullptr;
    float* Rm = nullptr;
    float* Saug = nullptr;
    float* Laug = nullptr;
    int ld_aug = 0;
    float* Linv = nullptr;
    unsigned long long* Lsign = nullptr;
    int* sweep_sync = nullptr;
    size_t sweep_sync_words = 0;
    bool sweep_latched_off = false;
    bool prelinearized = false;
    long long persistent_sweeps = 0;
    long long schur_sweeps = 0;
    long long sweep_recoveries = 0;
    long long early_output_frames = 0;
    int sweep_spin_limit = 0;
    int sweep_stall_wg = -1;
#ifdef EKFVIO_TEST_HOOKS
    int sweep_delay_wg = -1, sweep_delay_point = 0, sweep_delay_ticks = 0;
#endif
    bool sweep_retry_armed = false;
    double sweep_retry_pause_s = 0.0;
    int sweep_probation = 0;
    std::chrono::steady_clock::time_point sweep_retry_at;
    bool graph_leaves_flags_clean = false;
    bool sweep_flags_clean = false;
    bool persist_attr_set = false;
    bool gain2_attr_set = false;
    bool gather_attr_set = false;
    long long t2_updates = 0;
    long long graph_steps = 0;
    long long prelinearized_steps = 0;
    int num_cus = 0;
    int last_m = 0;
    long long* sweep_dbg = nullptr;
    long long* gemm_stamps = nullptr;
    float* Km = nullptr;
    float* Wt = nullptr;
    float* Gm = nullptr;
    int* info = nullptr;
    float gate_chi2 = 0.f;
    float* gate_d2 = nullptr;
    uint8_t* gate_flag = nullptr;
    uint8_t* gate_pass = nullptr;
    int* gate_words = nullptr;
    int* fb_words = nullptr;
    float* fb_err2 = nullptr;
    uint8_t* fb_flag = nullptr;
    float* fb_pt_err2 = nullptr;
    float* fb_pt_back = nullptr;
    uint8_t* fb_pt_flag = nullptr;
    int* remove_words = nullptr;
    int* h_info = nullptr;
    int* d_hinfo = nullptr;
    int status_seq = 0;
    float* h_out = nullptr;
    float* d_out = nullptr;
    bool out_fresh = false;
    unsigned char* h_meas = nullptr;
    unsigned char* d_meas = nullptr;
    float* seq_z = nullptr;
    float* seq_R = nullptr;
    uint8_t* seq_pass = nullptr;
    int seq_frames = 0;
    int seq_N = 0;
    std::vector<int> seq_m;
    std::vector<std::vector<uint8_t>> seq_pass_host;

    KltFrame frames[2];
    int cur = 0;
    int klt_border = 0;
    float* klt_prev_px = nullptr;
    float* klt_next_px = nullptr;
    uint8_t* klt_status = nullptr;
    float* klt_cov_px = nullptr;
    uint8_t* staging = nullptr;
    uint8_t* h_image = nullptr;
    size_t src_cap = 0;
    double dist[5] = {0, 0, 0, 0, 0};
    bool rect_on = false;
    int* rect_sx = nullptr;
    int* rect_sy = nullptr;
    uint8_t* rect_img = nullptr;
    size_t rect_cap = 0;
    RectifyKey rect_key;
    bool rect_key_valid = false;
    uint8_t* blurred = nullptr;
    unsigned* fast_row_kp = nullptr;
    int* fast_kp_xy = nullptr;
    short* fast_kp_score = nullptr;
    int fast_kp_cap = 0;
    uint8_t* occ_mask = nullptr;
// ... 9 lines not shown
    hipGraphExec_t step_graph_pair = nullptr;
    int graph_pre = 0, graph_pre_big = 0, graph_pre_pair = 0;
    int graph_N = -1, graph_m = -1, graph_frames = -1;
    bool graph_sole = true;
    float graph_dt = -1.f;
    float* graph_mu = nullptr;
    float* graph_P = nullptr;
    const void* graph_seq = nullptr;

    bool prof_on = false;
    float prof_overhead_ms = 0.f;
    ProfSlot prof[PC_COUNT];
    hipEvent_t ev0 = nullptr, ev1 = nullptr;
};

struct GemmEpi {
    int mode = 0;
    const int* inv_idx = nullptr;
    const float* Rm = nullptr;
    float* G = nullptr;
    int ldg = 0;
    float* mu = nullptr;
    float* Pcol = nullptr;
    const float* Kyp = nullptr;
    int kyp_blocks = 0, kyp_ld = 0;
    int n = 0;
    int* frame_counter = nullptr;
    int frames = 0;
    long long* stamps = nullptr;
    int* zero_words = nullptr;
    int n_zero = 0;
    int order2d = 0;
    int lin_blocks = 0;
    int lin_N = 0;
    float lin_dt = 0.f;
    float* lin_FA = nullptr;
    float* lin_FB = nullptr;
    float* lin_FD = nullptr;
    float* lin_mu_next = nullptr;
    int mean_keep = 0;
    int sym_w = 1;
    int sym = 0;
    const int* abort = nullptr;
};
struct GemmCall {
    int M = 0, N = 0, K = 0;
    bool transB = false;
    bool flush = false, lowerB = false;
    float alpha = 1.f, beta = 0.f;
    const float *A = nullptr, *B = nullptr, *Cin = nullptr;
    float* C = nullptr;
    int lda = 0, ldb = 0, ldcin = 0, ldc = 0;
    GemmEpi epi;
    int variant = 0;
};
inline GemmShape gemm_shape(const GemmCall& c) {
    GemmShape s;
    s.M = c.M, s.N = c.N, s.K = c.K, s.transB = c.transB, s.lowerB = c.lowerB;
    s.epi = c.epi.mode, s.mean = c.epi.n > 0, s.lin_blocks = c.epi.lin_blocks, s.sym = c.epi.sym != 0, s.variant = c.variant;
    return s;
}
void launch_gemm(ekfvio_filter* f, const GemmCall& c);

struct BookArgs {
    int enabled = 0;
    int N = 0, m_pad = 0;
    const float* z = nullptr;
    const float* R = nullptr;
    const uint8_t* pass = nullptr;
    float* last_klt = nullptr;
    uint8_t* del_flag = nullptr;
    int* idx = nullptr;
    int* inv_idx = nullptr;
    float* zrow = nullptr;
    float* Rm = nullptr;
    const int* frame_counter = nullptr;
    int* m_out = nullptr;
    uint8_t* pass_eff = nullptr;
    const float* mu = nullptr;
    const float* P = nullptr;
    int ldp = 0;
    float chi2 = 0.f;
    float* d2 = nullptr;
    uint8_t* gated = nullptr;
    int* gate_words = nullptr;
    int count_total = 0;
};
BookArgs make_book_args(ekfvio_filter* f, int m, const float* d_z, const float* d_R, const uint8_t* d_pass, const int* d_frame_counter);
void launch_linearize(ekfvio_filter* f, float dt, const BookArgs* book = nullptr);
void launch_build_dense_F(ekfvio_filter* f, float* Fdense);
void launch_predict(ekfvio_filter* f, float dt, const BookArgs* book = nullptr);
struct UpdateInputs {
    int m = 0;
    const float *z = nullptr, *R = nullptr;
    const uint8_t* pass = nullptr;
    int* frame_counter = nullptr;
    int frames = 0;
    bool bookkeeping_done = false;
    bool m_on_device = false;
    bool gate_counted = false;
    float next_dt = -1.f;
    int publish_seq = 0;
    int (*between)(ekfvio_filter*, int kyp_blocks) = nullptr;
    bool recoverable = true;
};
struct UpdateResult {
    bool published = false;
    int between_seq = 0;
};
UpdateResult launch_update(ekfvio_filter* f, const UpdateInputs& in);
void launch_check_sigma(ekfvio_filter* f, float* d_out);
int klt_level_pitch(int w);
int klt_border();
void klt_intrinsics(const ekfvio_filter* f, const float* K, float* fx, float* fy, float* cx, float* cy);
struct Level0View {
    const uint8_t* img = nullptr;
    int pitch = 0, w = 0, h = 0;
    float fx = 0.f, fy = 0.f, cx = 0.f, cy = 0.f;
};
Level0View klt_level0(const ekfvio_filter* f);
int push_frame_check(ekfvio_filter* f, const uint8_t* image, int32_t width, int32_t height, int32_t stride, const float K[9]);
int push_frame_enqueue(ekfvio_filter* f, const uint8_t* image, int32_t width, int32_t height, int32_t stride, const float K[9]);
int klt_track_device(ekfvio_filter* f);
void launch_imu_update(ekfvio_filter* f, const float gyro[3], const float accel[3]);
int fast_alloc(ekfvio_filter* f);
void fast_free(ekfvio_filter* f);
int fast_ensure(ekfvio_filter* f, int w, int h);
void launch_publish_status(ekfvio_filter* f, int seq);
int wait_status(ekfvio_filter* f, int* status, const int* extra_dev = nullptr, int* extra_out = nullptr);
int next_status_seq(ekfvio_filter* f);
void sweep_abort_latch(ekfvio_filter* f);
void sweep_clean_update(ekfvio_filter* f);
int read_status(ekfvio_filter* f, int seq, const int* extra_dev, int* bad, int* extra);
int settle_update(ekfvio_filter* f, int bad, void (*rerun)(ekfvio_filter*, void*), void* ctx, bool counts_as_clean);
void sweep_maybe_retry(ekfvio_filter* f);
int poll_status(ekfvio_filter* f, int seq, int* status, int* extra_out);
int add_features_device(ekfvio_filter* f, int k);
void add_features_enqueue_device_count(ekfvio_filter* f, const int* count_dev);
int replenish_enqueue(ekfvio_filter* f, int* enqueued);

int live_handles_on(int device);
inline PlanShape plan_shape(const ekfvio_filter* f) {
    PlanShape s;
    s.num_cus = f->num_cus, s.ldp = f->ldp, s.sweep_sync_words = f->sweep_sync_words, s.N = f->N, s.n = f->n;
    s.dense_predict = f->cfg.predict_mode == EKFVIO_PREDICT_DENSE;
    s.sole_handle = live_handles_on(f->device) <= 1;
    s.latched_off = f->sweep_latched_off;
    return s;
}
inline UpdatePlan plan_update(const ekfvio_filter* f, int m, bool m_on_device = false, float next_dt = -1.f, bool recoverable = true) {
    return plan_update(f->tune, plan_shape(f), m, m_on_device, next_dt, recoverable);
}
int launch_update_gemms_scratch(ekfvio_filter* f, const UpdatePlan& p, int reps, double* last_flops);
const int* launch_chol_sweep(ekfvio_filter* f, const UpdatePlan& p, float* Saug, float* Laug, float* Linv, int ld, bool zero_flags);
const int* launch_persist_fused(ekfvio_filter* f, const UpdatePlan& p, bool zero_flags);
void launch_joseph_g(ekfvio_filter* f, int m, int m_pad, int n_pad, bool m_on_device, const float* T = nullptr);
inline float* t2_buffer(ekfvio_filter* f) { return f->Fdense; }
void launch_gain2_tiles(ekfvio_filter* f, const UpdatePlan& p);
void launch_gather_potrf(ekfvio_filter* f, const UpdatePlan& p);
void launch_potrf_stamps(ekfvio_filter* f, const float* S, int ld, float* L, float* Linv, long long* d_stamps);
void launch_gain_from_sweep(ekfvio_filter* f, const UpdatePlan& p, const float* Laug, int ld, int n, float* K, float* scratch, int ldk, int refine);

void launch_remove_features(ekfvio_filter* f, const uint8_t* remove, const int* added, bool abort_aware, bool host_removed);
size_t remove_lds_bytes(const ekfvio_filter* f);
void remove_applied(ekfvio_filter* f, int delta, int removed);
int rectify_ensure(ekfvio_filter* f, size_t src);
void rectify_free(ekfvio_filter* f);
const uint8_t* rectify_enqueue(ekfvio_filter* f, const uint8_t* src, int w, int h, const float K[9], hipStream_t st);
int klt_alloc(ekfvio_filter* f);
void klt_free(ekfvio_filter* f);

struct ProfScope {
    ekfvio_filter* f;
    int cls;
    int launches;
    ProfScope(ekfvio_filter* f_, int cls_, double flops = 0, int launches_ = 1) : f(f_), cls(cls_), launches(launches_) {
        if (f->prof_on) {
            (void)hipEventRecord(f->ev0, f->stream);
            f->prof[cls].flops += flops;
        }
    }
    ~ProfScope() {
        if (f->prof_on) {
            (void)hipEventRecord(f->ev1, f->stream);
            (void)hipEventSynchronize(f->ev1);
            float ms = 0;
            (void)hipEventElapsedTime(&ms, f->ev0, f->ev1);
            f->prof[cls].ms += ms;
            f->prof[cls].launches += launches;
        }
    }
};
```

### ekf_vio_amd/csrc/ekf_kernels.hip

```cpp
#include <algorithm>
#include <utility>

#include "common.h"

namespace {

#include "motion_model.inc"

template <int NT, bool EFF = false>
__device__ __forceinline__ void bookkeeping_body(const BookArgs& a) {
    __shared__ int s_cnt[32];
    __shared__ int s_total;
    const int tid = threadIdx.x;
    const int N = a.N, m_pad = a.m_pad;
    const float* z = a.z;
    const float* R = a.R;
    const uint8_t* pass = a.pass;
    if (a.frame_counter) {
        const int fi = *a.frame_counter;
        z += (size_t)fi * 2 * N;
        R += (size_t)fi * 4 * N;
        pass += (size_t)fi * N;
    }
    if (EFF) pass = a.pass_eff;
// ... 627 lines not shown
                       Fdense);
}

void launch_predict(ekfvio_filter* f, float dt, const BookArgs* book) {
    const PredictPlan p = plan_predict(f->tune, plan_shape(f), f->prelinearized);
    f->prelinearized = false;
    if (p.pre) f->prelinearized_steps++;
    if (p.lin_in_front) launch_linearize(f, dt, book);
    const int n = f->n, ld = f->ldp;
    if (p.dense) {
        launch_build_dense_F(f, f->Fdense);
        {
            ProfScope ps(f, PC_GEMM_PREDICT, 4.0 * n * (double)n * n);
            GemmCall g;
            g.M = g.N = n, g.K = round_up(n, 32), g.A = f->Fdense, g.lda = ld, g.B = f->P, g.ldb = ld, g.C = f->P2, g.ldc = ld;
            launch_gemm(f, g);
            g.transB = true, g.A = f->P2, g.B = f->Fdense, g.C = f->P;
            launch_gemm(f, g);
        }
        ProfScope ps(f, PC_PREDICT);
        hipLaunchKernelGGL(add_noise_flush_kernel, dim3((n + 255) / 256, n), dim3(256), 0, f->stream, f->P, ld, n, dt);
    } else {
        ProfScope ps(f, PC_PREDICT, 4.0 * n * (358.0 + 36.0 * f->N));
        BookArgs b;
        if (book && p.book_rides()) b = *book;
        const dim3 grid(p.grid(b.enabled != 0));
        if (p.lin_inside)
            hipLaunchKernelGGL(predict_fused_kernel<true>, grid, dim3(256), 0, f->stream, f->P, ld, f->N, n, f->FA, f->FB, f->FD, dt, f->P2,
                               p.ts, p.chunks, f->mu, f->mu_next, b, f->sweep_dbg);
        else
            hipLaunchKernelGGL(predict_fused_kernel<false>, grid, dim3(256), 0, f->stream, f->P, ld, f->N, n, f->FA, f->FB, f->FD, dt, f->P2,
                               p.ts, p.chunks, f->mu, f->mu_next, b, f->sweep_dbg);
        std::swap(f->P, f->P2);
    }
    std::swap(f->mu, f->mu_next);
}

struct TailGemms {
    int count;
    GemmCall g[2];
    GemmCall& last() { return g[count - 1]; }
};
static TailGemms update_tail_gemms(ekfvio_filter* f, const UpdatePlan& p, const float* from, float* to) {
    const int n = f->n, ld = f->ldp;
    TailGemms t;
    GemmCall c;
    c.M = c.N = n, c.K = p.m_pad, c.transB = true, c.lda = c.ldb = c.ldcin = c.ldc = ld, c.beta = 1.f, c.Cin = from, c.C = to;
    t.g[0] = t.g[1] = c;
    GemmCall& g2 = t.g[1];
    if (p.tail != TAIL_JOSEPH) {
        t.count = 1;
        GemmCall& g = t.g[0];
        g.A = f->Km, g.B = f->Gm, g.flush = true, g.epi.mode = EPI_MEAN;
        return t;
    }
    t.count = 2;
    GemmCall& g1 = t.g[0];
    g1.N = n + 1, g1.alpha = -1.f, g1.A = f->Km, g1.B = f->Wt;
    g1.epi.mode = EPI_JOSEPH1, g1.epi.inv_idx = f->inv_idx, g1.epi.Rm = f->Rm, g1.epi.G = f->Gm, g1.epi.ldg = ld;
    g2.A = f->Gm, g2.B = f->Km, g2.Cin = to, g2.flush = true, g2.epi.mode = EPI_MEAN, g2.epi.sym = 1;
    return t;
}

UpdateResult launch_update(ekfvio_filter* f, const UpdateInputs& in) {
    const bool gate = f->gate_chi2 > 0.f && f->N > 0;
    const UpdatePlan p = plan_update(f, in.m, in.m_on_device || (gate && in.m > 0), in.next_dt, in.recoverable);
    const int m = p.m, m_pad = p.m_pad, n_pad = p.n_pad, n = f->n, ld = f->ldp;
    UpdateResult out;
    f->last_m = m;
    {
        ProfScope ps(f, PC_GATHER);
        if (!in.bookkeeping_done) {
            BookArgs bk = make_book_args(f, m, in.z, in.R, in.pass, in.frame_counter);
            if (p.m_on_device) bk.m_out = f->info + 2;
            if (gate) {
                bk.pass_eff = f->gate_pass, bk.mu = f->mu, bk.P = f->P, bk.ldp = ld, bk.chi2 = f->gate_chi2;
                bk.d2 = f->gate_d2, bk.gated = f->gate_flag, bk.gate_words = f->gate_words, bk.count_total = in.gate_counted ? 0 : 1;
                hipLaunchKernelGGL(gate_bookkeeping_kernel, dim3(1), dim3(1024), 0, f->stream, bk);
            } else
                hipLaunchKernelGGL(update_bookkeeping_kernel, dim3(1), dim3(1024), 0, f->stream, bk);
        }
        if (p.fused_gather) {
            launch_gather_potrf(f, p);
        } else if (m > 0 && p.sweep != SWEEP_PERSIST_FUSED) {
            const GatherArgs ga = make_gather_args(f, p);
            const int nb2 = p.with_wt ? (m_pad / 64) * (ld / 64) : 0;
            hipLaunchKernelGGL(gather_kernel, dim3(ga.nb1 + nb2), dim3(256), 0, f->stream, ga);
        }
    }
    if (m <= 0) {
        ProfScope ps(f, PC_UPDATE_MISC);
        hipLaunchKernelGGL(mean_update_kernel, dim3((n + 63) / 64), dim3(256), 0, f->stream, f->Km, ld, n, 0, f->yres, f->mu,
                           in.frame_counter, in.frames);
        return out;
    }
    const bool zero_flags = p.persistent() && !p.fused_gather && !f->sweep_flags_clean;
    const int* abort = p.sweep == SWEEP_PERSIST_FUSED ? launch_persist_fused(f, p, zero_flags)
                                                      : launch_chol_sweep(f, p, f->Saug, f->Laug, f->Linv, f->ld_aug, zero_flags);
    if (in.publish_seq) launch_publish_status(f, in.publish_seq), out.published = true;
    TailGemms tail = update_tail_gemms(f, p, p.tail == TAIL_T2 ? t2_buffer(f) : f->P, f->P);
    GemmEpi& e2 = tail.last().epi;
    e2.mu = f->mu, e2.Pcol = f->P + (size_t)n * ld, e2.n = n;
    e2.frame_counter = in.frame_counter, e2.frames = in.frames;
    e2.abort = abort;
    if (p.persistent()) {
        e2.zero_words = f->sweep_sync, e2.n_zero = persist_zero_words(m_pad, n_pad);
        f->sweep_flags_clean = true;
    }
    if (p.tail == TAIL_T2) f->t2_updates++;
    if (p.gain == GAIN_SCHUR) launch_joseph_g(f, m, m_pad, n_pad, p.m_on_device);
    else if (p.gain == GAIN2_T2_TILES) launch_gain2_tiles(f, p);
    else if (p.gain != GAIN_SWEEP) launch_gain_from_sweep(f, p, f->Laug, f->ld_aug, n, f->Km, f->Gm, ld, 0);
    if (p.tail == TAIL_JOSEPH) {
        tail.g[0].epi.abort = abort;
        ProfScope ps(f, PC_GEMM_UPDATE, 2.0 * n * (double)(n + 1) * m_pad + 2.0 * n * (double)n * m_pad, 2);
        launch_gemm(f, tail.g[0]);
        if (in.between) out.between_seq = in.between(f, 0);
        launch_gemm(f, tail.g[1]);
        return out;
    }
    if (p.tail == TAIL_T2 && in.between) out.between_seq = in.between(f, m_pad / 64);
    ProfScope ps(f, PC_GEMM_UPDATE, 2.0 * n * (double)n * m_pad, 1);
    e2.mode = EPI_MEAN_PARTIAL;
    e2.Kyp = f->Wt, e2.kyp_blocks = m_pad / 64, e2.kyp_ld = ld;
    if (p.lin_blocks) {
        e2.lin_blocks = p.lin_blocks, e2.lin_N = f->N, e2.lin_dt = in.next_dt;
        e2.lin_FA = f->FA, e2.lin_FB = f->FB, e2.lin_FD = f->FD, e2.lin_mu_next = f->mu_next;
        f->prelinearized = true;
    }
    launch_gemm(f, tail.last());
    return out;
}

int launch_update_gemms_scratch(ekfvio_filter* f, const UpdatePlan& p, int reps, double* last_flops) {
    TailGemms tail = update_tail_gemms(f, p, f->P, f->P2);
    for (int r = 0; r < reps; r++)
        for (int k = 0; k < tail.count; k++) launch_gemm(f, tail.g[k]);
    const GemmShape sh = gemm_shape(tail.last());
    *last_flops = gemm_executed_flops(sh, plan_gemm(f->tune, f->num_cus, sh));
    return tail.count;
}

void launch_check_sigma(ekfvio_filter* f, float* d_out) {
    hipLaunchKernelGGL(check_sigma_kernel, dim3(1), dim3(256), 0, f->stream, f->P, f->ldp, f->n, d_out);
}
```

### ekf_vio_amd/csrc/gemm.hip

```cpp
#include "common.h"

#include <algorithm>

typedef float f32x16 __attribute__((ext_vector_type(16)));
typedef float f32x4 __attribute__((ext_vector_type(4)));

namespace {
#include "motion_model.inc"
}

#ifdef EKF_GEMM_STAMPS
#define GSTAMP(i)                                                                                  \
    do {                                                                                           \
        if (stamps_ && (i) < 40) stamps_[i] = (long long)__builtin_amdgcn_s_memtime();             \
    } while (0)
#else
#define GSTAMP(i) do { } while (0)
#endif

#define BM 64
#define BN 64
#define BK 32
#define LDS_A (BM)
#define LDS_BT (BN)
// ... 333 lines not shown
#pragma unroll
    for (int u = 0; u < 4; u++) {
        if (keep) break;
        const int e = min((int)threadIdx.x + 256 * u, epi.n - 1);
        if (EPI == 3) {
            float pk[16];
#pragma unroll
            for (int cb = 0; cb < 16; cb++) pk[cb] = epi.Kyp[(size_t)min(cb, epi.kyp_blocks - 1) * epi.kyp_ld + e];
            const float m0 = epi.mu[e];
            float ky = pk[0];
#pragma unroll
            for (int cb = 1; cb < 16; cb++) ky = (cb < epi.kyp_blocks) ? ky + pk[cb] : ky;
            for (int cb = 16; cb < epi.kyp_blocks; cb++) ky = ky + epi.Kyp[(size_t)cb * epi.kyp_ld + e];
            v4[u] = m0 + ky;
        } else {
            v4[u] = epi.mu[e] + epi.Pcol[e];
        }
    }
    if (aborted) return;
#pragma unroll
    for (int u = 0; u < 4; u++) {
        const int e = (int)threadIdx.x + 256 * u;
        if (e < epi.n && !keep) {
            if (EPI != 3) epi.Pcol[e] = 0.f;
            if (e >= 3 && e <= 6) s_q[e - 3] = v4[u];
            else epi.mu[e] = v4[u];
        }
    }
    for (int e = threadIdx.x + 1024; e < (keep ? 0 : epi.n); e += 256) {
        float v;
        if (EPI == 3) {
            float ky = epi.Kyp[e];
            for (int cb = 1; cb < epi.kyp_blocks; cb++) ky = ky + epi.Kyp[(size_t)cb * epi.kyp_ld + e];
            v = epi.mu[e] + ky;
        } else {
            v = epi.mu[e] + epi.Pcol[e];
            epi.Pcol[e] = 0.f;
        }
        epi.mu[e] = v;
    }
    __builtin_amdgcn_s_waitcnt(0xc07f);
    __builtin_amdgcn_s_barrier();
    if (threadIdx.x < 4 && !keep) {
        const float qn = sqrtf(s_q[0] * s_q[0] + s_q[1] * s_q[1] + s_q[2] * s_q[2] + s_q[3] * s_q[3]);
        epi.mu[3 + threadIdx.x] = s_q[threadIdx.x] / qn;
    }
    if (threadIdx.x == 0 && epi.frame_counter) {
        const int fi = *epi.frame_counter + 1;
        *epi.frame_counter = (fi >= epi.frames) ? 0 : fi;
    }
    for (int e = threadIdx.x; e < epi.n_zero; e += 256) epi.zero_words[e] = 0;
}

template <int BMt, int WPS, int EPI>
__global__ __launch_bounds__(256 * WPS) void gemm16_kernel(int M, int N, int K, float alpha, const float* __restrict__ A, int lda,
                                                     const float* __restrict__ B, int ldb, float beta, const float* Cin,
                                                     int ldcin, float* C, int ldc, int flush, int lowerB, GemmEpi epi,
                                                     int tiles_x, int tiles_y) {
    constexpr int RB = BMt / 16;
    constexpr int SA = (BMt % 32 == 16) ? BMt : BMt + 16;
    constexpr int SB = 80;
    constexpr int BKK = 64;
    constexpr int NT = 256 * WPS;
    constexpr int AVT = BKK * BMt / 4;
    constexpr int AV = (AVT + NT - 1) / NT;
    constexpr int BV = BKK * 64 / 4 / NT;
    constexpr int BKS = NT / 16;
    constexpr int NS = BKK / 4 / WPS;
    __shared__ __attribute__((aligned(16))) float As[3][BKK * SA];
    __shared__ __attribute__((aligned(16))) float Bs[3][BKK * SB];

    if ((EPI == 2 || EPI == 3) && (int)blockIdx.x == tiles_x * tiles_y) {
        if (threadIdx.x >= 256) return;
        if (epi.n > 0) gemm16_finish_mean<EPI>(epi);
        return;
    }
    if (EPI == 3 && (int)blockIdx.x > tiles_x * tiles_y) {
        if (threadIdx.x >= 256) return;
        const int tid = threadIdx.x;
        const int lb = (int)blockIdx.x - tiles_x * tiles_y - 1;
        LinLds& l = *reinterpret_cast<LinLds*>(&As[0][0]);
        static_assert(sizeof(LinLds) <= sizeof(As), "linearisation scratch");
        float* s_mu = &Bs[0][0];
        int aborted = 0;
        if (epi.abort) aborted = *epi.abort;
        constexpr int NE = EKF_BASE + 3 * LIN_LM;
        if (tid < NE) {
            const int e = (tid < EKF_BASE) ? tid : min(EKF_BASE + 3 * LIN_LM * lb + (tid - EKF_BASE), epi.n - 1);
            float pk[16];
#pragma unroll
            for (int cb = 0; cb < 16; cb++) pk[cb] = epi.Kyp[(size_t)min(cb, epi.kyp_blocks - 1) * epi.kyp_ld + e];
            const float m0 = epi.mu[e];
            float ky = pk[0];
#pragma unroll
            for (int cb = 1; cb < 16; cb++) ky = (cb < epi.kyp_blocks) ? ky + pk[cb] : ky;
            for (int cb = 16; cb < epi.kyp_blocks; cb++) ky = ky + epi.Kyp[(size_t)cb * epi.kyp_ld + e];
            s_mu[tid] = aborted ? m0 : m0 + ky;
        }
        __syncthreads();
        if (tid < 4 && !aborted) {
            const float qn = sqrtf(s_mu[3] * s_mu[3] + s_mu[4] * s_mu[4] + s_mu[5] * s_mu[5] + s_mu[6] * s_mu[6]);
            const float qv = s_mu[3 + tid] / qn;
            s_mu[3 + tid] = qv;
        }
        __syncthreads();
        const int e0 = EKF_BASE + 3 * LIN_LM * lb;
        auto mean = [s_mu, e0](int e) { return (e < EKF_BASE) ? s_mu[e] : s_mu[EKF_BASE + (e - e0)]; };
        linearize_block(mean, epi.lin_N, epi.lin_dt, epi.lin_FA, epi.lin_FB, epi.lin_FD, epi.lin_mu_next, lb, epi.lin_blocks - 1, l, tid);
        return;
    }
    const int nwg = tiles_x * tiles_y;
    const int bq = nwg >> 3, br = nwg & 7, xcd = blockIdx.x & 7;
    const int swz = xcd * bq + min(xcd, br) + (blockIdx.x >> 3);
    const int ti = swz % tiles_x, tj = swz / tiles_x;
    const int i0 = ti * BMt;
    const int j0 = tj * 64;

#ifdef EKF_GEMM_STAMPS
    long long* stamps_ = (blockIdx.x == 9 && threadIdx.x == 0) ? epi.stamps : nullptr;
#endif
    GSTAMP(0);
    const int tid = threadIdx.x, lane = tid & 63;
    const int wave = (tid >> 6) & 3;
    const int kg = tid >> 8;
    const int li = lane & 15, g = lane >> 4;
    const int Mread = (M + 63) & ~63;

    const int kbeg = lowerB ? min(j0, K) : 0;
    const int KT = (K - kbeg) / BKK;

#define G16_ACOORD(u)                                                                       \
    const int ea##u = min(tid + NT * u, AVT - 1);                                           \
    const int ao##u = ((ea##u / (BMt / 4)) * lda + min(i0 + (ea##u % (BMt / 4)) * 4, Mread - 4)) * 4;  \
    const int al##u = (ea##u / (BMt / 4)) * SA + (ea##u % (BMt / 4)) * 4;
    G16_ACOORD(0) G16_ACOORD(1) G16_ACOORD(2) G16_ACOORD(3)
#undef G16_ACOORD
    const __amdgpu_buffer_rsrc_t rsA = __builtin_amdgcn_make_buffer_rsrc(const_cast<float*>(A), 0, K * lda * 4, 0x00020000);
    const __amdgpu_buffer_rsrc_t rsB = __builtin_amdgcn_make_buffer_rsrc(const_cast<float*>(B), 0, K * ldb * 4, 0x00020000);
    const int bo = ((tid >> 4) * ldb + j0 + (tid & 15) * 4) * 4;
    const int bl = (tid >> 4) * SB + (tid & 15) * 4;
    const int a_step = BKK * lda * 4, b_step = BKK * ldb * 4, b_rows = BKS * ldb * 4;
    const int a_base = kbeg * lda * 4, b_base = kbeg * ldb * 4;
    static_assert((BV == 4 || BV == 2) && AV >= 1 && AV <= 4, "staging is written for 1..4 float4 of A and 2 or 4 of B per thread");

    f32x4 acc[RB];
#pragma unroll
    for (int a = 0; a < RB; a++) acc[a] = f32x4{0.f, 0.f, 0.f, 0.f};
    int sweep_aborted = 0;
    if (EPI != 0 && epi.abort) sweep_aborted = *epi.abort;

    float cpre[RB][4];
#pragma unroll
    for (int a = 0; a < RB; a++)
#pragma unroll
        for (int v = 0; v < 4; v++) {
            const int i = i0 + 16 * a + li, j = j0 + 16 * wave + 4 * g + v;
            cpre[a][v] = (beta != 0.f && i < M && j < N) ? Cin[(size_t)j * ldcin + i] : 0.f;
        }

    int qv[4] = {-1, -1, -1, -1};
    float kq[RB][4], kp[RB][4];
    if (EPI == 1 && kg == 0) {
        const int jbq = j0 + 16 * wave + 4 * g;
#pragma unroll
        for (int v = 0; v < 4; v++) qv[v] = epi.inv_idx[min(jbq + v, N - 1)];
#pragma unroll
        for (int a = 0; a < RB; a++) {
            const int ic = min(i0 + 16 * a + li, M - 1);
#pragma unroll
            for (int v = 0; v < 4; v++) {
                const int q = max(qv[v], 0);
                kq[a][v] = A[(size_t)q * lda + ic] * epi.Rm[2 * q];
                kp[a][v] = A[(size_t)(q ^ 1) * lda + ic] * epi.Rm[2 * q + 1];
            }
        }
    }
    float4 Xa0, Xa1, Xa2, Xa3, Xb0, Xb1, Xb2, Xb3, Ya0, Ya1, Ya2, Ya3, Yb0, Yb1, Yb2, Yb3;
    float4 Za0, Za1, Za2, Za3, Zb0, Zb1, Zb2, Zb3;
    Xa0 = Xa1 = Xa2 = Xa3 = Xb0 = Xb1 = Xb2 = Xb3 = make_float4(0.f, 0.f, 0.f, 0.f);
    Ya0 = Ya1 = Ya2 = Ya3 = Yb0 = Yb1 = Yb2 = Yb3 = make_float4(0.f, 0.f, 0.f, 0.f);
    Za0 = Za1 = Za2 = Za3 = Zb0 = Zb1 = Zb2 = Zb3 = make_float4(0.f, 0.f, 0.f, 0.f);
#define G16_LOAD(S, kt)                                                                                \
    do {                                                                                               \
        const int sa_ = a_base + (kt) * a_step, sb_ = b_base + (kt) * b_step;                          \
        S##a0 = __builtin_bit_cast(float4, __builtin_amdgcn_raw_buffer_load_b128(rsA, ao0, sa_, 0));                                                               \
        if constexpr (AV > 1) S##a1 = __builtin_bit_cast(float4, __builtin_amdgcn_raw_buffer_load_b128(rsA, ao1, sa_, 0));                                         \
        if constexpr (AV > 2) S##a2 = __builtin_bit_cast(float4, __builtin_amdgcn_raw_buffer_load_b128(rsA, ao2, sa_, 0));                                         \
        if constexpr (AV > 3) S##a3 = __builtin_bit_cast(float4, __builtin_amdgcn_raw_buffer_load_b128(rsA, ao3, sa_, 0));                                         \
        S##b0 = __builtin_bit_cast(float4, __builtin_amdgcn_raw_buffer_load_b128(rsB, bo, sb_, 0));                                                                \
        S##b1 = __builtin_bit_cast(float4, __builtin_amdgcn_raw_buffer_load_b128(rsB, bo + b_rows, sb_, 0));                                                       \
        if constexpr (BV > 2) S##b2 = __builtin_bit_cast(float4, __builtin_amdgcn_raw_buffer_load_b128(rsB, bo + 2 * b_rows, sb_, 0));                             \
        if constexpr (BV > 2) S##b3 = __builtin_bit_cast(float4, __builtin_amdgcn_raw_buffer_load_b128(rsB, bo + 3 * b_rows, sb_, 0));                             \
    } while (0)
#define G16_LOADI(S, j, kt)                                                                            \
    do {                                                                                               \
        const int sa_ = a_base + (kt) * a_step, sb_ = b_base + (kt) * b_step;                          \
        if ((j) == 0) S##a0 = __builtin_bit_cast(float4, __builtin_amdgcn_raw_buffer_load_b128(rsA, ao0, sa_, 0));                                                 \
        if ((j) == 1 && AV > 1) S##a1 = __builtin_bit_cast(float4, __builtin_amdgcn_raw_buffer_load_b128(rsA, ao1, sa_, 0));                                       \
        if ((j) == 2 && AV > 2) S##a2 = __builtin_bit_cast(float4, __builtin_amdgcn_raw_buffer_load_b128(rsA, ao2, sa_, 0));                                       \
        if ((j) == 3 && AV > 3) S##a3 = __builtin_bit_cast(float4, __builtin_amdgcn_raw_buffer_load_b128(rsA, ao3, sa_, 0));                                       \
        if ((j) == AV) S##b0 = __builtin_bit_cast(float4, __builtin_amdgcn_raw_buffer_load_b128(rsB, bo, sb_, 0));                                                 \
        if ((j) == AV + 1) S##b1 = __builtin_bit_cast(float4, __builtin_amdgcn_raw_buffer_load_b128(rsB, bo + b_rows, sb_, 0));                                    \
        if ((j) == AV + 2 && BV > 2) S##b2 = __builtin_bit_cast(float4, __builtin_amdgcn_raw_buffer_load_b128(rsB, bo + 2 * b_rows, sb_, 0));                      \
        if ((j) == AV + 3 && BV > 2) S##b3 = __builtin_bit_cast(float4, __builtin_amdgcn_raw_buffer_load_b128(rsB, bo + 3 * b_rows, sb_, 0));                      \
    } while (0)
#define G16_STAGEI(S, j, buf)                                                                          \
    do {                                                                                               \
        if ((j) == 0) *reinterpret_cast<float4*>(&As[buf][al0]) = S##a0;                               \
        if ((j) == 1 && AV > 1) *reinterpret_cast<float4*>(&As[buf][al1]) = S##a1;                     \
        if ((j) == 2 && AV > 2) *reinterpret_cast<float4*>(&As[buf][al2]) = S##a2;                     \
        if ((j) == 3 && AV > 3) *reinterpret_cast<float4*>(&As[buf][al3]) = S##a3;                     \
        if ((j) == AV) *reinterpret_cast<float4*>(&Bs[buf][bl]) = S##b0;                               \
        if ((j) == AV + 1) *reinterpret_cast<float4*>(&Bs[buf][bl + BKS * SB]) = S##b1;                \
        if ((j) == AV + 2 && BV > 2) *reinterpret_cast<float4*>(&Bs[buf][bl + 2 * BKS * SB]) = S##b2;  \
        if ((j) == AV + 3 && BV > 2) *reinterpret_cast<float4*>(&Bs[buf][bl + 3 * BKS * SB]) = S##b3;  \
    } while (0)
#define G16_STAGE_A(S, buf)                                                                            \
    do {                                                                                               \
        *reinterpret_cast<float4*>(&As[buf][al0]) = S##a0;  \
        if constexpr (AV > 1) *reinterpret_cast<float4*>(&As[buf][al1]) = S##a1;                       \
        if constexpr (AV > 2) *reinterpret_cast<float4*>(&As[buf][al2]) = S##a2;                       \
        if constexpr (AV > 3) *reinterpret_cast<float4*>(&As[buf][al3]) = S##a3;                       \
    } while (0)
#define G16_STAGE_B(S, buf)                                                                            \
    do {                                                                                               \
        *reinterpret_cast<float4*>(&Bs[buf][bl]) = S##b0;                                              \
        *reinterpret_cast<float4*>(&Bs[buf][bl + BKS * SB]) = S##b1;                                   \
        if constexpr (BV > 2) *reinterpret_cast<float4*>(&Bs[buf][bl + 2 * BKS * SB]) = S##b2;         \
        if constexpr (BV > 2) *reinterpret_cast<float4*>(&Bs[buf][bl + 3 * BKS * SB]) = S##b3;         \
    } while (0)
#define G16_MFMA(c, b, a) c = __builtin_amdgcn_mfma_f32_16x16x4f32(b, a, c, 0, 0, 0)
#ifndef G16X_NOLOAD
#define G16X_NOLOAD 0
#endif
#ifndef G16X_NOSTAGE
#define G16X_NOSTAGE 0
#endif
#ifndef G16X_NOBAR
#define G16X_NOBAR 0
#endif
#ifndef G16X_NOFR
#define G16X_NOFR 0
#endif
#define G16_FR(P, st, slot)                                                               \
    do {                                                                                  \
        if (G16X_NOFR) break;                                                             \
        fb[slot] = P##b[(4 * WPS * (st)) * SB];                                           \
        _Pragma("unroll") for (int a = 0; a < RB; a++) fa[slot][a] = P##a[(4 * WPS * (st)) * SA + 16 * a]; \
    } while (0)
#define G16_TILE(S1, S2, tcur)                                                            \
    do {                                                                                  \
        const int nxt = (cb == 2) ? 0 : cb + 1;                                           \
        na = &As[nxt][(g + 4 * kg) * SA + li];                                            \
        nb = &Bs[nxt][(g + 4 * kg) * SB + 16 * wave + li];                                \
        _Pragma("unroll") for (int st = 0; st < NS; st++) {                               \
            if (st + 2 < NS) G16_FR(p, st + 2, (st + 2) % 4);                             \
            _Pragma("unroll") for (int a = 0; a < RB; a++)                                \
                G16_MFMA(acc[a], fb[st % 4], fa[st % 4][a]);                              \
               \
                   \
            if (!G16X_NOLOAD) G16_LOADI(S2, st, (tcur) + 3);                              \
            if (!G16X_NOSTAGE) G16_STAGEI(S1, st, nxt);                                   \
            if (st == BAR && !G16X_NOBAR) __syncthreads();                                \
            if (st == NS - 2) G16_FR(n, 0, 0);                                            \
            if (st == NS - 1) G16_FR(n, 1, 1);                                            \
            __builtin_amdgcn_sched_barrier(0);                                            \
        }                                                                                 \
        cb = nxt;                                                                         \
        pa = na;                                                                          \
        pb = nb;                                                                          \
    } while (0)

    if (KT > 0) {
        constexpr int BAR = AV + BV;
        static_assert(BAR <= NS - 3 && NS % 4 == 0, "step schedule");
        G16_LOAD(Z, 0);
        G16_LOAD(X, 1);
        G16_LOAD(Y, 2);
        G16_STAGE_A(Z, 0);
        G16_STAGE_B(Z, 0);
        __syncthreads();
        float fa[4][RB], fb[4];
        int cb = 0;
        const float* pa = &As[0][(g + 4 * kg) * SA + li];
        const float* pb = &Bs[0][(g + 4 * kg) * SB + 16 * wave + li];
        const float* na = pa;
        const float* nb = pb;
        G16_FR(n, 0, 0);
        G16_FR(n, 1, 1);
        GSTAMP(1);
        int t = 0;
        for (; t + 2 < KT; t += 3) {
            G16_TILE(X, Z, t);
            GSTAMP(2 + t);
            G16_TILE(Y, X, t + 1);
            GSTAMP(3 + t);
            G16_TILE(Z, Y, t + 2);
            GSTAMP(4 + t);
        }
        if (t < KT) {
            G16_TILE(X, Z, t);
            t++;
        }
        if (t < KT) G16_TILE(Y, X, t);
        GSTAMP(36);
        __syncthreads();
    }
#undef G16_TILE
#undef G16_FR
#undef G16_LOAD
#undef G16_LOADI
#undef G16_STAGEI
#undef G16_STAGE_A
#undef G16_STAGE_B
    if constexpr (WPS > 1) {
        float* red = &As[0][0];
        static_assert(3 * BKK * SA >= RB * 4 * 256, "reduction scratch");
        if (kg == 1) {
#pragma unroll
            for (int a = 0; a < RB; a++)
#pragma unroll
                for (int v = 0; v < 4; v++) red[(a * 4 + v) * 256 + (tid & 255)] = acc[a][v];
        }
        __syncthreads();
        if (kg == 1) return;
#pragma unroll
        for (int a = 0; a < RB; a++)
#pragma unroll
            for (int v = 0; v < 4; v++) acc[a][v] += red[(a * 4 + v) * 256 + tid];
    }

    GSTAMP(37);
    if (EPI != 0 && sweep_aborted) return;
    float vout[RB][4];
#pragma unroll
    for (int a = 0; a < RB; a++)
#pragma unroll
        for (int v = 0; v < 4; v++) {
            float x = alpha * acc[a][v];
            x = x + beta * cpre[a][v];
            if (flush) x = (fabsf(x) > EKF_FLUSH_THRESH) ? x : 0.f;
            vout[a][v] = x;
        }
    const int jb = j0 + 16 * wave + 4 * g;
    if (EPI == 1) {
#pragma unroll
        for (int a = 0; a < RB; a++) {
            const int i = i0 + 16 * a + li;
#pragma unroll
            for (int v = 0; v < 4; v++) {
                const int q = qv[v];
                const float kr = ((q ^ 1) < q) ? (kp[a][v] + kq[a][v]) : (kq[a][v] + kp[a][v]);
                if (q >= 0 && jb + v < N && i < M) epi.G[(size_t)q * epi.ldg + i] = kr - vout[a][v];
            }
        }
    }
    float* cp = C + (size_t)jb * ldc + i0 + li;
    if (i0 + BMt <= M && j0 + 64 <= N) {
#pragma unroll
        for (int a = 0; a < RB; a++)
#pragma unroll
            for (int v = 0; v < 4; v++) cp[(size_t)v * ldc + 16 * a] = vout[a][v];
    } else {
#pragma unroll
        for (int a = 0; a < RB; a++) {
            if (i0 + 16 * a + li < M) {
#pragma unroll
                for (int v = 0; v < 4; v++)
                    if (jb + v < N) cp[(size_t)v * ldc + 16 * a] = vout[a][v];
            }
        }
    }
    GSTAMP(38);
}

void launch_gemm(ekfvio_filter* f, const GemmCall& c) {
    const int M = c.M, N = c.N, K = c.K;
    if (M <= 0 || N <= 0 || K <= 0) return;
    GemmEpi e = c.epi;
    const GemmPlan p = plan_gemm(f->tune, f->num_cus, gemm_shape(c));
    hipStream_t s = f->stream;
    e.stamps = f->gemm_stamps;
    e.lin_blocks = p.lin_blocks, e.mean_keep = p.mean_keep;
    const dim3 grid(p.grid_x, p.grid_y), block(p.threads());
    const int flush = c.flush, lowerB = c.lowerB;
    if (p.k16) {
#define GEMM16_GO(BMv, W, EP)                                                                                                     \
    hipLaunchKernelGGL((gemm16_kernel<BMv, W, EP>), grid, block, 0, s, M, N, K, c.alpha, c.A, c.lda, c.B, c.ldb, c.beta, c.Cin, c.ldcin, \
                       c.C, c.ldc, flush, lowerB, e, p.tiles_x, p.tiles_y)
#define GEMM16_BM(W, EP)                            \
    do {                                            \
        if (p.bm == 32) GEMM16_GO(32, W, EP);       \
        else if (p.bm == 48) GEMM16_GO(48, W, EP);  \
        else GEMM16_GO(64, W, EP);                  \
    } while (0)
        if (e.mode == EPI_JOSEPH1) GEMM16_BM(2, 1);
        else if (e.mode == EPI_MEAN) GEMM16_BM(2, 2);
        else if (e.mode == EPI_MEAN_PARTIAL) GEMM16_BM(2, 3);
        else if (p.wps == 2) GEMM16_BM(2, 0);
        else GEMM16_BM(1, 0);
#undef GEMM16_BM
#undef GEMM16_GO
        return;
    }
    e.sym = p.sym, e.sym_w = p.sym_w, e.order2d = p.order2d;
#define GEMM_GO(TB, G, EP)                                                                                                        \
    hipLaunchKernelGGL((gemm_f32_mfma_kernel<TB, G, EP>), grid, block, 0, s, M, N, K, c.alpha, c.A, c.lda, c.B, c.ldb, c.beta, c.Cin, \
                       c.ldcin, c.C, c.ldc, flush, lowerB, e)
    if (e.mode == EPI_JOSEPH1) {
        GEMM_GO(true, 1, 1);
    } else if (e.mode == EPI_MEAN) {
        GEMM_GO(true, 1, 2);
    } else if (e.mode == EPI_MEAN_PARTIAL) {
        GEMM_GO(true, 1, 3);
    } else if (p.groups == 2) {
        if (c.transB) GEMM_GO(true, 2, 0);
        else GEMM_GO(false, 2, 0);
    } else {
        if (c.transB) GEMM_GO(true, 1, 0);
        else GEMM_GO(false, 1, 0);
    }
#undef GEMM_GO
}
```

### ekf_vio_amd/csrc/plan.h

```cpp
#ifndef EKFVIO_PLAN_H_
#define EKFVIO_PLAN_H_
#include <stddef.h>
#include <stdlib.h>

#include <algorithm>

#define EKF_BASE 22
#define EKF_TILE 64
#ifndef EKF_SWEEP_SPLIT_MB
#define EKF_SWEEP_SPLIT_MB 16
#endif
#define LIN_LM 8
#define GC 4
#define GCI 4

static inline int round_up(int x, int m) { return (x + m - 1) / m * m; }

struct Tuning {
    int early_status = 1;
    int upload_kernel = 1;
    int sweep_wait_ticks = 300000;
    double sweep_retry_first_s = 2.0;
    int persist_sweep = 1;
    int sweep_la = 1;
// ... 165 lines not shown
    } else {
        p.grid_x = p.tiles_x, p.grid_y = p.tiles_y;
        p.tiles = p.tiles_x * p.tiles_y;
    }
    p.order2d = (!p.sym && t.gemm_order2d && !s.lowerB && p.tiles >= 2 * cus) ? 1 : 0;
    return p;
}
inline double gemm_executed_flops(const GemmShape& s, const GemmPlan& p) {
    return p.sym ? 2.0 * 64.0 * 64.0 * s.K * p.tiles : 2.0 * s.M * (double)s.N * s.K;
}

#define PREDICT_PT 16
#define PREDICT_PC 3
struct PredictPlan {
    bool dense = false;
    bool pre = false;
    bool lin_inside = false;
    bool lin_in_front = false;
    int ts = 0, chunks = 0;
    bool book_rides() const { return lin_inside || pre; }
    int grid(bool bookkeeping) const { return ts * ts + 1 + 2 * chunks + (bookkeeping && book_rides() ? 1 : 0); }
};
inline PredictPlan plan_predict(const Tuning& t, const PlanShape& s, bool prelinearized) {
    PredictPlan p;
    p.dense = s.dense_predict;
    p.pre = prelinearized && !p.dense;
    p.ts = (s.N + PREDICT_PT - 1) / PREDICT_PT, p.chunks = (s.N + PREDICT_PC - 1) / PREDICT_PC;
    p.lin_inside = !p.pre && !p.dense && t.fuse_linearize && p.ts * p.ts <= 4 * s.num_cus;
    p.lin_in_front = !p.lin_inside && !p.pre;
    return p;
}

inline int gather_gx(int ldp, int m_pad) { return (std::max(ldp, m_pad) + 255) / 256; }
inline int gather_element_wgs(int ldp, int m_pad) { return gather_gx(ldp, m_pad) * ((m_pad + GC * GCI - 1) / (GC * GCI)); }

enum SweepKind { SWEEP_NONE,
                 SWEEP_SCHUR,
                 SWEEP_PERSIST_FUSED,
                 SWEEP_PERSIST,
                 SWEEP_STEP,
                 SWEEP_SPLIT, SWEEP_SPLIT_LA };
enum GainBy { GAIN_SWEEP, GAIN_TILES, GAIN2_T2_TILES, GAIN_GEMM, GAIN_SCHUR };
enum UpdateTail { TAIL_NONE, TAIL_SCHUR, TAIL_T2, TAIL_JOSEPH };
struct UpdatePlan {
    int m = 0, m_pad = 64, n_pad = 0;
    bool m_on_device = false, recoverable = true;
    SweepKind sweep = SWEEP_NONE;
    bool fused_gather = false;
    bool with_wt = false;
    GainBy gain = GAIN_GEMM;
    UpdateTail tail = TAIL_NONE;
    int t2_skip = -1;
    bool t2_by_sweep = false, compact = false;
    int lin_blocks = 0;
    bool persistent() const { return sweep == SWEEP_PERSIST_FUSED || sweep == SWEEP_PERSIST; }
};

enum PersistGridKind { GRID_PLAIN,
                       GRID_FUSED,
                       GRID_COMPACT };
enum PersistRoleKind { ROLE_CHAIN, ROLE_LEAD, ROLE_LEAD_GATHER0, ROLE_GATHER0, ROLE_OWNER, ROLE_NONE };
struct PersistRole {
    int kind, a, b, n;
};
PLAN_HD constexpr int t2_pairs(int nX) { return nX * (nX + 1) / 2; }
PLAN_HD void t2_pair(int p, int& ta, int& tb) {
    ta = 0;
    while ((ta + 1) * (ta + 2) / 2 <= p) ta++;
    tb = p - ta * (ta + 1) / 2;
}
struct PersistGrid {
    int kind = GRID_PLAIN;
    int mb = 0, nX = 0;
    int lead_rows = 0;
    int t2_skip = 0;
    PLAN_HD bool fused() const { return kind != GRID_PLAIN; }
    PLAN_HD bool compact() const { return kind == GRID_COMPACT; }
    PLAN_HD int lead() const { return fused() ? mb * lead_rows : 0; }
    PLAN_HD int gatherers() const { return kind == GRID_FUSED ? 2 : 0; }
    PLAN_HD int a_rows(int j) const { return mb - j - (j == 1 ? 1 : 0); }
    PLAN_HD int column_owners(int j) const { return a_rows(j) + nX + (j + 1 - (compact() ? 1 : 0)); }
    PLAN_HD int owners() const {
        int h = 0;
        for (int j = 1; j < mb; j++) h += column_owners(j);
        return h;
    }
    PLAN_HD int owner_block(int h) const { return 1 + lead() + gatherers() + h; }
    PLAN_HD int total() const { return owner_block(owners()); }
    PLAN_HD int t2_pair_of(int h) const { return (h >= t2_skip && h - t2_skip < t2_pairs(nX)) ? h - t2_skip : -1; }
    PLAN_HD PersistRole role(int block) const {
        if (block == 0) return {ROLE_CHAIN, 0, 0, 0};
        int h = block - 1;
        if (h < lead()) {
            const int ib = h / mb, cb = h % mb;
            if (compact() && cb == mb - 1 && ib < 2) return {ROLE_LEAD_GATHER0, ib, cb, h};
            return {ROLE_LEAD, ib, cb, h};
        }
        h -= lead();
        if (h < gatherers()) return {ROLE_GATHER0, h, 0, h};
        h -= gatherers();
        const int n = h;
        for (int j = 1; j < mb; j++) {
            const int nA = a_rows(j);
            if (h < column_owners(j)) {
                const int i = h < nA ? j + h + (j == 1 ? 1 : 0) : h < nA + nX ? mb + (h - nA) : mb + nX + (h - nA - nX);
                return {ROLE_OWNER, i, j, n};
            }
            h -= column_owners(j);
        }
        return {ROLE_NONE, 0, 0, n};
    }
};
#ifndef EKF_PERSIST_OVERSUB
#define EKF_PERSIST_OVERSUB 1
#endif
inline bool persist_shape(const Tuning& t, const PlanShape& s, int m_pad, int n_pad) {
    const int mb = m_pad / EKF_TILE;
    const int over = t.persist_oversub > 0 ? t.persist_oversub : EKF_PERSIST_OVERSUB;
    return mb >= 3 && mb < EKF_SWEEP_SPLIT_MB && PersistGrid{GRID_PLAIN, mb, n_pad / EKF_TILE}.total() <= (over > 1 ? over : 1) * s.num_cus &&
           persist_flag_words(m_pad, n_pad) <= s.sweep_sync_words;
}
inline bool gain_in_sweep_shape(const Tuning& t, const PlanShape& s, int m_pad, int n_pad) {
    const int mb = m_pad / EKF_TILE;
    return persist_shape(t, s, m_pad, n_pad) && PersistGrid{GRID_FUSED, mb, n_pad / EKF_TILE, s.ldp / 64}.total() <= s.num_cus + 8;
}
inline int t2_skip_owners(const Tuning& t, const PlanShape& s, int m_pad, int n_pad) {
    if (!t.t2_flow || !t.persist_gain || t.schur || !gain_in_sweep_shape(t, s, m_pad, n_pad)) return -1;
    const PersistGrid g{GRID_COMPACT, m_pad / EKF_TILE, n_pad / EKF_TILE, s.ldp / 64};
    if (g.total() > s.num_cus) return -1;
    if (g.nX + 2 > PERSIST_POLL_FLAGS) return -1;
    return (t2_pairs(g.nX) <= g.owners()) ? 0 : -1;
}
inline PersistGrid persist_grid(const UpdatePlan& p, int ldp) {
    return {p.sweep != SWEEP_PERSIST_FUSED ? GRID_PLAIN : p.compact ? GRID_COMPACT : GRID_FUSED, p.m_pad / EKF_TILE, p.n_pad / EKF_TILE, ldp / 64, p.t2_skip};
}
inline SweepKind choose_sweep(const Tuning& t, const PlanShape& s, int m_pad, int n_pad, bool filter_update) {
    const int mb = m_pad / EKF_TILE;
    const bool schur_shape = t.schur && mb < EKF_SWEEP_SPLIT_MB;
    if (schur_shape && filter_update) return SWEEP_SCHUR;
    if (t.persist_sweep && !s.latched_off && !schur_shape && s.sole_handle && persist_shape(t, s, m_pad, n_pad))
        return (filter_update && t.fuse_sweep && t.fuse_gather) ? SWEEP_PERSIST_FUSED : SWEEP_PERSIST;
    return mb < EKF_SWEEP_SPLIT_MB ? SWEEP_STEP : t.sweep_la ? SWEEP_SPLIT_LA : SWEEP_SPLIT;
}
inline bool gain_tiles_shape(const Tuning& t, const PlanShape& s, int m_pad, int n_pad) { return t.persist_gain && gain_in_sweep_shape(t, s, m_pad, n_pad); }

inline UpdatePlan plan_raw_sweep(const Tuning& t, const PlanShape& s, int m_pad, int n_pad) {
    UpdatePlan p;
    p.m = p.m_pad = m_pad, p.n_pad = n_pad;
    p.sweep = choose_sweep(t, s, m_pad, n_pad, false);
    p.gain = gain_tiles_shape(t, s, m_pad, n_pad) ? GAIN_TILES : GAIN_GEMM;
    return p;
}

inline GemmShape tail_gemm_shape(int n, int m_pad, int lin_blocks) {
    GemmShape g;
    g.M = g.N = n, g.K = m_pad, g.transB = true, g.epi = EPI_MEAN_PARTIAL, g.mean = true, g.lin_blocks = lin_blocks;
    return g;
}
inline UpdatePlan plan_update(const Tuning& t, const PlanShape& s, int m, bool m_on_device = false, float next_dt = -1.f, bool recoverable = true) {
    UpdatePlan p;
    if (m_on_device) m = 2 * s.N;
    const int n = s.n, ld = s.ldp, m_pad = round_up(m > 0 ? m : 1, EKF_TILE), n_pad = round_up(n, EKF_TILE);
    p.m = m, p.m_pad = m_pad, p.n_pad = n_pad, p.m_on_device = m_on_device, p.recoverable = recoverable;
    if (m <= 0) return p;
    p.sweep = choose_sweep(t, s, m_pad, n_pad, true);
    const bool schur = p.sweep == SWEEP_SCHUR, fused = p.sweep == SWEEP_PERSIST_FUSED;
    p.with_wt = !schur;
    if (t.fuse_gather && !fused)
        p.fused_gather = 1 + gather_element_wgs(ld, m_pad) + (schur ? 0 : (m_pad / 64) * (ld / 64)) <= s.num_cus;
    if (schur) return p.gain = GAIN_SCHUR, p.tail = TAIL_SCHUR, p;
    p.t2_skip = t2_skip_owners(t, s, m_pad, n_pad);
    if (p.t2_skip < 0) {
        p.gain = !gain_tiles_shape(t, s, m_pad, n_pad) ? GAIN_GEMM : fused ? GAIN_SWEEP : GAIN_TILES;
        return p.tail = TAIL_JOSEPH, p;
    }
    p.tail = TAIL_T2;
    p.t2_by_sweep = p.compact = fused;
    p.gain = fused ? GAIN_SWEEP : GAIN2_T2_TILES;
    const int lin_blocks = (s.N + LIN_LM - 1) / LIN_LM + 1;
    if (next_dt >= 0.f && t.lin_overlap && !s.dense_predict && t.fuse_linearize)
        p.lin_blocks = plan_gemm(t, s.num_cus, tail_gemm_shape(n, m_pad, lin_blocks)).lin_blocks;
    return p;
}
#endif
```

### ekf_vio_amd/filter.py

```python
import ctypes as C

import numpy as np

from . import capi

BASE_STATE_SIZE = 22


def _fp(a):
    return a.ctypes.data_as(C.POINTER(C.c_float))


def _u8(a):
    return a.ctypes.data_as(C.POINTER(C.c_uint8))


class TightlyCoupledEKF:
    def __init__(self, max_features=100, device=0, stream=None, predict_mode=capi.PREDICT_STRUCTURED,
                 default_point_depth=0.5, default_point_depth_variance=100.0,
                 default_point_homogenous_variance=1e-5, hooks=False, gate_chi2=0.0, klt_fb_max_px=0.0, distortion=None, **cfg_overrides):
        self.hooks = bool(hooks)
        self.lib = capi.load(hooks=self.hooks)
        cfg = capi.Config()
        self._chk(self.lib.ekfvio_default_config(C.byref(cfg)))
# ... 200 lines not shown
        if on:
            self._chk(self.lib.ekfvio_profile_reset(self.h))

    def profile_report(self):
        out = {}
        for c in range(self.lib.ekfvio_profile_count()):
            ms, n, fl = C.c_double(0), C.c_int64(0), C.c_double(0)
            self._chk(self.lib.ekfvio_profile_get(self.h, c, C.byref(ms), C.byref(n), C.byref(fl)))
            out[self.lib.ekfvio_profile_name(c).decode()] = dict(ms=ms.value, launches=n.value, flops=fl.value)
        return out

    def profile_update_gemms(self, reps=50):
        us, fl = C.c_double(0), C.c_double(0)
        self._chk(self.lib.ekfvio_profile_update_gemms(self.h, int(reps), C.byref(us), C.byref(fl)))
        return us.value, fl.value

    def test_gemm(self, A, B, C0, alpha=1.0, beta=0.0, transB=True, variant=0):
        self._need_hooks()
        A = np.asarray(A, np.float32)
        B = np.asarray(B, np.float32)
        M, K = A.shape
        N = B.shape[0] if transB else B.shape[1]
        Ac, Bc = np.array(A.T, order="C", copy=True), np.array(B.T, order="C", copy=True)
        Cc = np.array(np.asarray(C0, np.float32).T, order="C", copy=True)
        self._chk(self.lib.ekfvio_test_gemm(self.h, int(transB), M, N, K, alpha, _fp(Ac), M, _fp(Bc), B.shape[0], beta,
                                            _fp(Cc), M, int(variant)))
        return Cc.T.copy()

    def counters(self):
        c = (C.c_int64 * 8)()
        self._chk(self.lib.ekfvio_get_counters(self.h, c))
        return dict(persistent=int(c[0]), schur=int(c[1]), recoveries=int(c[2]), mode=int(c[3]), early_output_frames=int(c[4]), t2_updates=int(c[5]),
                    graph_steps=int(c[6]), prelinearized_steps=int(c[7]))

    def _need_hooks(self):
        if not self.hooks:
            raise RuntimeError("this entry point exists only in the hooks build: construct the filter with hooks=True")

    def persistent_sweeps(self):
        return self.counters()["persistent"]

    def sweep_counts(self):
        c = self.counters()
        return {k: c[k] for k in ("persistent", "schur", "recoveries", "mode")}

    def sweep_fault(self, spin_limit=0, stall_workgroup=-1):
        self._need_hooks()
        self._chk(self.lib.ekfvio_test_sweep_fault(self.h, int(spin_limit), int(stall_workgroup)))

    def sweep_delay(self, workgroup=-1, point=0, ticks=0):
        self._need_hooks()
        self._chk(self.lib.ekfvio_test_sweep_delay(self.h, int(workgroup), int(point), int(ticks)))

    def test_cholesky_solve(self, S, Crhs):
        self._need_hooks()
        S = np.asarray(S, np.float32)
        Crhs = np.asarray(Crhs, np.float32)
        m, nr = S.shape[0], Crhs.shape[0]
        Sc, Cc = np.array(S.T, order="C", copy=True), np.array(Crhs.T, order="C", copy=True)
        L = np.zeros((m, m), np.float32)
        X = np.zeros((m, nr), np.float32)
        info = C.c_int32(0)
        self._chk(self.lib.ekfvio_test_cholesky_solve(self.h, m, nr, _fp(Sc), _fp(Cc), _fp(L), _fp(X), C.byref(info)))
        return L.T.copy(), X.T.copy(), info.value


class KLTTracker:

    def __init__(self, ekf):
        self.ekf = ekf
        self.lib = ekf.lib

    def push_frame(self, img, K):
        img = np.ascontiguousarray(img, dtype=np.uint8)
        h, w = img.shape
        K = np.ascontiguousarray(K, dtype=np.float32).reshape(9)
        self.ekf._chk(self.lib.ekfvio_klt_push_frame(self.ekf.h, _u8(img), w, h, w, _fp(K)))

    def findNewFeaturePositions(self):
        N = self.ekf.num_features
        z = np.zeros((N, 2), np.float32)
        R = np.zeros((N, 4), np.float32)
        p = np.zeros(N, np.uint8)
        self.ekf._chk(self.lib.ekfvio_klt_track(self.ekf.h, _fp(z), _fp(R), _u8(p)))
        return z, R, p

    def track_points(self, prev_px, init_px):
        pp = np.ascontiguousarray(prev_px, dtype=np.float32).reshape(-1, 2)
        ii = np.ascontiguousarray(init_px, dtype=np.float32).reshape(-1, 2)
        out = np.zeros_like(pp)
        st = np.zeros(pp.shape[0], np.uint8)
        self.ekf._chk(self.lib.ekfvio_klt_track_points(self.ekf.h, _fp(pp), _fp(ii), pp.shape[0], _fp(out), _u8(st)))
        return out, st

    def track_points_fb(self, prev_px, init_px):
        pp = np.ascontiguousarray(prev_px, dtype=np.float32).reshape(-1, 2)
        ii = np.ascontiguousarray(init_px, dtype=np.float32).reshape(-1, 2)
        out, back = np.zeros_like(pp), np.zeros_like(pp)
        st, ok = np.zeros(pp.shape[0], np.uint8), np.zeros(pp.shape[0], np.uint8)
        e2 = np.zeros(pp.shape[0], np.float32)
        self.ekf._chk(self.lib.ekfvio_klt_track_points_fb(self.ekf.h, _fp(pp), _fp(ii), pp.shape[0], _fp(out), _u8(st), _fp(back), _fp(e2),
                                                          _u8(ok)))
        return out, st, back, e2, ok

    def uncertainty_points(self, ref_px, cur_px):
        rp = np.ascontiguousarray(ref_px, dtype=np.float32).reshape(-1, 2)
# ... 143 lines not shown
```

### include/ekfvio_test_hooks.h

```cpp
#ifndef EKFVIO_TEST_HOOKS_H_
#define EKFVIO_TEST_HOOKS_H_
#include "ekfvio.h"
#ifdef __cplusplus
extern "C" {
#endif

EKFVIO_API int ekfvio_test_klt_padded_level(ekfvio_filter* f, int32_t level, int32_t* border, uint8_t* img, int16_t* deriv);
EKFVIO_API int ekfvio_test_blurred_level0(ekfvio_filter* f, uint8_t* out);
EKFVIO_API int ekfvio_test_gemm(ekfvio_filter* f, int32_t transB, int32_t M, int32_t N, int32_t K, float alpha, const float* A,
                     int32_t lda, const float* B, int32_t ldb, float beta, float* C, int32_t ldc, int32_t variant);
EKFVIO_API int ekfvio_test_gemm_bench(ekfvio_filter* f, int32_t transB, int32_t lowerB, int32_t M, int32_t N, int32_t K,
                           int32_t reps, int32_t variant, double* mean_us);
EKFVIO_API int ekfvio_test_potrf_stamps(ekfvio_filter* f, int64_t stamps[80]);
EKFVIO_API int ekfvio_test_sweep_stamps(ekfvio_filter* f, int enable, int64_t stamps[1024]);
EKFVIO_API int ekfvio_test_sweep_fault(ekfvio_filter* f, int32_t spin_limit, int32_t stall_workgroup);
#define EKFVIO_TEST_SWEEP_DELAY_MAX_TICKS 100000
EKFVIO_API int ekfvio_test_sweep_delay(ekfvio_filter* f, int32_t workgroup, int32_t point, int32_t ticks);
EKFVIO_API int ekfvio_test_cholesky_solve(ekfvio_filter* f, int32_t m, int32_t nrhs, const float* S, const float* Crhs,
                               float* L_out, float* X_out, int32_t* info);
EKFVIO_API int ekfvio_test_plan(int32_t num_cus, int32_t max_features, int32_t N, int32_t m, int32_t m_on_device, int32_t sole_handle,
                                int32_t latched_off, int32_t dense_predict, float next_dt, int32_t plan[12]);
EKFVIO_API int ekfvio_test_gemm_plan(int32_t num_cus, int32_t M, int32_t N, int32_t K, int32_t transB, int32_t lowerB, int32_t epi, int32_t mean,
                                     int32_t lin_blocks, int32_t sym, int32_t variant, int32_t plan[18]);
EKFVIO_API int ekfvio_test_predict_plan(int32_t num_cus, int32_t N, int32_t dense_predict, int32_t prelinearized, int32_t bookkeeping,
                                        int32_t plan[8]);
EKFVIO_API int ekfvio_test_persist_grid(int32_t num_cus, int32_t max_features, int32_t N, int32_t m, int32_t m_on_device, int32_t sole_handle,
                                        int32_t latched_off, int32_t dense_predict, float next_dt, int32_t* roles, int32_t max_blocks,
                                        int32_t out[10]);
EKFVIO_API int ekfvio_test_t2_pair(int32_t p, int32_t pair[2]);

#ifdef __cplusplus
}
#endif
#endif
```

Measured before the change: 11040.

## Move W2 subtraction from gain tiles into tail GEMM on-load path

```diff
diff --git a/ekf_vio_amd/capi.py b/ekf_vio_amd/capi.py
--- a/ekf_vio_amd/capi.py
+++ b/ekf_vio_amd/capi.py
@@ -40,7 +40,7 @@
            "ekfvio_profile_update_gemms", "ekfvio_get_counters", "ekfvio_set_gate", "ekfvio_get_gate",
            "ekfvio_set_klt_fb", "ekfvio_get_klt_fb", "ekfvio_klt_track_points_fb", "ekfvio_set_distortion", "ekfvio_rectify_map"]
 HOOK_SYMBOLS = ["ekfvio_test_klt_padded_level", "ekfvio_test_blurred_level0", "ekfvio_test_gemm", "ekfvio_test_gemm_bench", "ekfvio_test_potrf_stamps",
-                "ekfvio_test_sweep_stamps", "ekfvio_test_sweep_fault", "ekfvio_test_sweep_delay", "ekfvio_test_cholesky_solve", "ekfvio_test_plan", "ekfvio_test_persist_grid", "ekfvio_test_t2_pair",
+                "ekfvio_test_sweep_stamps", "ekfvio_test_sweep_fault", "ekfvio_test_sweep_delay", "ekfvio_test_w2_in_tile", "ekfvio_test_cholesky_solve", "ekfvio_test_plan", "ekfvio_test_persist_grid", "ekfvio_test_t2_pair",
                 "ekfvio_test_gemm_plan", "ekfvio_test_predict_plan"]
 
 _libs = {}
@@ -102,6 +102,7 @@
             "ekfvio_test_sweep_stamps": [vp, C.c_int, C.POINTER(C.c_int64)],
             "ekfvio_test_sweep_fault": [vp, i32, i32],
             "ekfvio_test_sweep_delay": [vp, i32, i32, i32],
+            "ekfvio_test_w2_in_tile": [vp, i32],
             "ekfvio_test_gemm_bench": [vp, i32, i32, i32, i32, i32, i32, i32, C.POINTER(C.c_double)],
             "ekfvio_test_plan": [i32] * 8 + [f32, ip],
             "ekfvio_test_persist_grid": [i32] * 8 + [f32, ip, i32, ip],
diff --git a/ekf_vio_amd/csrc/api.hip b/ekf_vio_amd/csrc/api.hip
--- a/ekf_vio_amd/csrc/api.hip
+++ b/ekf_vio_amd/csrc/api.hip
@@ -198,6 +198,7 @@
     HIP_TRY(f, dev_alloc(f->stream, &f->Km, pm));
     HIP_TRY(f, dev_alloc(f->stream, &f->Wt, pm));
     HIP_TRY(f, dev_alloc(f->stream, &f->Gm, pm));
+    HIP_TRY(f, dev_alloc(f->stream, &f->Wm, pm));
     HIP_TRY(f, dev_alloc(f->stream, &f->info, 4));
     HIP_TRY(f, dev_alloc(f->stream, &f->remove_words, 4));
     HIP_TRY(f, hipHostMalloc((void**)&f->h_info, 16 * sizeof(int), hipHostMallocMapped | hipHostMallocCoherent));
@@ -273,7 +274,7 @@
     if (f->stream) (void)hipStreamSynchronize(f->stream);
     void* ptrs[] = {f->mu, f->mu_next, f->last_klt, f->del_flag, f->P,  f->P2, f->FA, f->FB, f->FD,   f->Fdense,
                     f->idx, f->inv_idx, f->zmeas,  f->Rmeas,    f->pass,     f->yres, f->Rm, f->Saug,  f->Laug,  f->Linv, f->Lsign, f->Km, f->sweep_sync, f->sweep_dbg,
-                    f->Wt,  f->Gm,     f->info,     f->remove_words, f->seq_z,    f->seq_R, f->seq_pass, f->gate_words, f->fb_words};
+                    f->Wt,  f->Gm,     f->Wm,  f->info,     f->remove_words, f->seq_z,    f->seq_R, f->seq_pass, f->gate_words, f->fb_words};
     for (void* p : ptrs)
         if (p) hipFree(p);
     if (f->h_info) hipHostFree(f->h_info);
@@ -1034,6 +1035,13 @@
     return EKFVIO_OK;
 }
 
+int ekfvio_test_w2_in_tile(ekfvio_filter* f, int32_t on) {
+    if (!f || on < -1 || on > 1) return EKFVIO_EINVAL;
+    f->w2_force = on;
+    drop_graph(f);
+    return EKFVIO_OK;
+}
+
 int ekfvio_test_cholesky_solve(ekfvio_filter* f, int32_t m, int32_t nrhs, const float* S, const float* Crhs,
                                float* L_out, float* X_out, int32_t* info) {
     if (!f || m <= 0 || nrhs <= 0 || !S || !Crhs) return EKFVIO_EINVAL;
diff --git a/ekf_vio_amd/csrc/chol.hip b/ekf_vio_amd/csrc/chol.hip
--- a/ekf_vio_amd/csrc/chol.hip
+++ b/ekf_vio_amd/csrc/chol.hip
@@ -906,6 +906,8 @@
     pa.L = L, pa.ldl = ldl, pa.mb = mb, pa.idb0 = mb + nX, pa.grid = g;
     pa.K = K, pa.ldk = ldk, pa.Lsign = f->Lsign;
     pa.Sg = f->P, pa.ldsg = f->ldp, pa.T2 = t2_buffer(f), pa.ldt = f->ldp, pa.nstate = f->n;
+    pa.W = f->Wm, pa.ldw = f->ldp, pa.inv_idx = f->inv_idx;
+    pa.w2_in_tile = p.w_on_load ? 0 : 1;
     if (!S) return pa;
     pa.S = S, pa.lds = ldl, pa.Linv = Linv, pa.info = f->info;
     pa.ready = f->sweep_sync + fl.ready(), pa.fin = f->sweep_sync + fl.fin(), pa.pan = f->sweep_sync + fl.pan(), pa.abort_flag = f->sweep_sync + fl.abort_word();
@@ -1055,7 +1057,7 @@
 
 void launch_gain2_tiles(ekfvio_filter* f, const UpdatePlan& p) {
     const int m_pad = p.m_pad, n_pad = p.n_pad;
-    ProfScope ps(f, PC_SOLVE, 2.0 * n_pad * (double)m_pad * m_pad + (double)n_pad * n_pad * m_pad);
+    ProfScope ps(f, PC_SOLVE, (double)n_pad * m_pad * m_pad + (double)n_pad * n_pad * m_pad);
     const PersistArgs pa = persist_args(f, p, f->Laug, f->ld_aug, f->Km, f->ldp);
     const int gain_wgs = pa.grid.nX * pa.mb;
     const int total = gain_wgs + t2_pairs(pa.grid.nX);
diff --git a/ekf_vio_amd/csrc/chol_persist.inc b/ekf_vio_amd/csrc/chol_persist.inc
--- a/ekf_vio_amd/csrc/chol_persist.inc
+++ b/ekf_vio_amd/csrc/chol_persist.inc
@@ -36,11 +36,15 @@
     float* T2;
     int ldt;
     int nstate;
+    float* W;
+    int ldw;
+    const int* inv_idx;
 #ifdef EKFVIO_TEST_HOOKS
     int delay_wg;
     int delay_point;
     int delay_ticks;
 #endif
+    int w2_in_tile;
 };
 
 typedef unsigned int u32x4 __attribute__((ext_vector_type(4)));
@@ -249,25 +253,10 @@
     }
 }
 
-template <bool WAIT>
-__device__ __forceinline__ void gain_tile2(const PersistArgs& a, const GatherArgs& ga, float* Ti, float* Tj, float* Tl, float* Tinv, float* Th, float* tab,
-                                           int ib, int cb, int tid) {
-    const int lane = tid & 63, wave = tid >> 6, wr = wave & 1, wc = wave >> 1;
-    const int r = wr * 32 + (lane & 31);
-    const int mb = a.mb, ldl = a.ldl;
-    const int m = ga.m_dev ? *ga.m_dev : ga.m;
-    const __amdgpu_buffer_rsrc_t bL = persist_rsrc(a.L, (unsigned)ldl * (unsigned)(mb * PB));
-    const __amdgpu_buffer_rsrc_t bS = persist_rsrc(a.S, (unsigned)a.lds * (unsigned)(mb * PB));
-    const int iy = mb + ib, iz = a.idb0 + cb;
-    const int cq = cb * PB + lane;
-    const int sq = (cq < m) ? ga.idx[cq] : -1;
-    const unsigned sqc = (unsigned)max(sq, 0);
-    int alo = 0, ahi = -1;
-    if (cb * PB < m) {
-        alo = ga.idx[cb * PB] / PB;
-        ahi = ga.idx[min(cb * PB + PB - 1, m - 1)] / PB;
-    }
+__device__ __forceinline__ void gain_tile2_tab(const GatherArgs& ga, float* tab, int cb, int m, int tid) {
     if (tid < 64) {
+        const int cq = cb * PB + tid;
+        const int sq = (cq < m) ? ga.idx[cq] : -1;
         float yq = 0.f, rd = 0.f, ro = 0.f;
         if (sq >= 0) {
             yq = ga.zrow[cq] - ga.mu[sq];
@@ -276,147 +265,17 @@
         }
         tab[tid] = yq, tab[64 + tid] = rd, tab[128 + tid] = ro;
     }
-    auto column_flags = [&](int kb, const int* zflag) -> PollLane {
-        const int ax = alo + tid - 2;
-        return {tid == 0 ? a.pan + iy * mb + kb : tid == 1 ? zflag : (tid >= 2 && ax <= ahi) ? a.pan + (mb + ax) * mb + kb : nullptr, 1};
-    };
-    float kv[16], w2[16];
-    {
-        float wv[16];
-        const int scl = max(sq, 0);
-#pragma unroll
-        for (int ps = 0; ps < 16; ps++) wv[ps] = ga.P[(size_t)min(ib * PB + wave + 4 * ps, ga.n - 1) * ga.ld + scl];
-#pragma unroll
-        for (int ps = 0; ps < 16; ps++) asm volatile("" : "+v"(wv[ps]));
-#pragma unroll
-        for (int ps = 0; ps < 16; ps++) Th[(wave + 4 * ps) * 65 + lane] = (sq >= 0 && ib * PB + wave + 4 * ps < ga.n) ? wv[ps] : 0.f;
-        __syncthreads();
-#pragma unroll
-        for (int q = 0; q < 16; q++) {
-            kv[q] = 0.f;
-            w2[q] = Th[r * 65 + mma64_col(wc, lane, q)];
-        }
-    }
-    auto fetch = [&](int kb) -> unsigned long long {
-        const bool gk = kb >= cb;
-        float hv[16];
-        unsigned long long neg;
-        if constexpr (WAIT) {
-            persist_wait(a, column_flags(kb, gk ? a.pan + iz * mb + kb : nullptr), tid, kb < mb - 2);
-            load_tile_sc1(Ti, bL, (unsigned)(kb * PB) * (unsigned)ldl + (unsigned)(iy * PB), ldl, tid);
-            if (gk) load_tile_sc1(Tj, bL, (unsigned)(kb * PB) * (unsigned)ldl + (unsigned)(iz * PB), ldl, tid);
-#pragma unroll
-            for (int ps = 0; ps < 16; ps++)
-                hv[ps] = __builtin_bit_cast(float, __builtin_amdgcn_raw_buffer_load_b32(bL, ((unsigned)(kb * PB + wave + 4 * ps) * (unsigned)ldl + (unsigned)(mb * PB) + sqc) * 4u, 0, 16));
-#pragma unroll
-            for (int ps = 0; ps < 16; ps++) hv[ps] = (sq >= 0) ? hv[ps] : 0.f;
-#pragma unroll
-            for (int ps = 0; ps < 16; ps++) Th[(wave + 4 * ps) * PLD + lane] = hv[ps];
-            neg = ld_sign_sc1(a.Lsign + kb);
-        } else {
-            load_tile(Ti, a.L + (size_t)kb * PB * ldl + (size_t)iy * PB, ldl, tid);
-            if (gk) load_tile(Tj, a.L + (size_t)kb * PB * ldl + (size_t)iz * PB, ldl, tid);
-#pragma unroll
-            for (int ps = 0; ps < 16; ps++) hv[ps] = a.L[(size_t)(kb * PB + wave + 4 * ps) * ldl + (size_t)(mb * PB) + sqc];
-#pragma unroll
-            for (int ps = 0; ps < 16; ps++) hv[ps] = (sq >= 0) ? hv[ps] : 0.f;
-#pragma unroll
-            for (int ps = 0; ps < 16; ps++) Th[(wave + 4 * ps) * PLD + lane] = hv[ps];
-            neg = a.Lsign[kb];
-        }
-        return neg;
-    };
-    auto products = [&](int kb, unsigned long long neg, bool z_unsigned) {
-        if (kb >= cb) {
-            const f32x16 up = (z_unsigned && neg != 0ull) ? mma64_signed(Ti, 1, PLD, Tj, 1, PLD, wr, wc, lane, neg) : mma64(Ti, 1, PLD, Tj, 1, PLD, wr, wc, lane);
-#pragma unroll
-            for (int q = 0; q < 16; q++) kv[q] = kv[q] + up[q];
-        }
-        if (alo <= ahi) {
-            f32x16 up;
-            if constexpr (WAIT) {
-                up = (neg == 0ull) ? mma64(Ti, 1, PLD, Th, 1, PLD, wr, wc, lane) : mma64_signed(Ti, 1, PLD, Th, 1, PLD, wr, wc, lane, neg);
-            } else {
-                if (__builtin_amdgcn_readfirstlane((int)(neg != 0ull))) {
-                    __syncthreads();
-                    sign_cols(Ti, Ti, neg, tid);
-                    __syncthreads();
-                }
-                up = mma64(Ti, 1, PLD, Th, 1, PLD, wr, wc, lane);
-            }
-#pragma unroll
-            for (int q = 0; q < 16; q++) w2[q] = w2[q] - up[q];
-        }
-        if (WAIT && a.dbg && tid == 0 && mb <= 8 && (ib == 0 || ib == 6) && (cb == 0 || cb == 3 || cb == 7))
-            a.dbg[100 + 8 * ((ib ? 3 : 0) + (cb == 0 ? 0 : cb == 3 ? 1 : 2)) + kb] = (long long)__builtin_amdgcn_s_memrealtime();
-    };
-    if constexpr (WAIT) {
-        for (int kb = 0; kb < mb - 2; kb++) {
-            __syncthreads();
-            const unsigned long long neg = fetch(kb);
-            __syncthreads();
-            products(kb, neg, false);
-        }
-    } else {
-        for (int kb = 0; kb < mb; kb++) {
-            __syncthreads();
-            const unsigned long long neg = fetch(kb);
-            __syncthreads();
-            products(kb, neg, false);
-        }
-    }
-    if constexpr (WAIT) {
-        const int kl = mb - 1, k6 = mb - 2;
-        const bool gk6 = k6 >= cb;
-        const __amdgpu_buffer_rsrc_t bI = persist_rsrc(a.Linv, (unsigned)(mb * PB * PB));
-        const bool zi = a.grid.compact() && cb == kl;
-        __syncthreads();
-        persist_wait(a, column_flags(k6, gk6 ? a.pan + iz * mb + k6 : (zi ? nullptr : a.fin + iz * mb + kl)), tid, false);
-        RegTile ql, qi, qj;
-        float hq[16];
-        unsigned long long neg6;
-        {
-            RegTile pi6, pj6;
-            float h6[16];
-            pi6.request(bL, (unsigned)(k6 * PB) * (unsigned)ldl + (unsigned)(iy * PB), ldl, tid);
-            if (gk6) pj6.request(bL, (unsigned)(k6 * PB) * (unsigned)ldl + (unsigned)(iz * PB), ldl, tid);
-#pragma unroll
-            for (int ps = 0; ps < 16; ps++)
-                h6[ps] = __builtin_bit_cast(float, __builtin_amdgcn_raw_buffer_load_b32(bL, ((unsigned)(k6 * PB + wave + 4 * ps) * (unsigned)ldl + (unsigned)(mb * PB) + sqc) * 4u, 0, 16));
-            neg6 = ld_sign_sc1(a.Lsign + k6);
-            pi6.put(Ti, tid);
-            if (gk6) pj6.put(Tj, tid);
-#pragma unroll
-            for (int ps = 0; ps < 16; ps++) Th[(wave + 4 * ps) * PLD + lane] = (sq >= 0) ? h6[ps] : 0.f;
-        }
-        persist_wait(a, a.ready + kl, nullptr, nullptr, tid, 4, false);
-        ql.request(bL, (unsigned)(kl * PB) * (unsigned)ldl + (unsigned)(kl * PB), ldl, tid);
-        qi.request(bS, (unsigned)(kl * PB) * (unsigned)a.lds + (unsigned)(iy * PB), a.lds, tid);
-        if (!zi) qj.request(bS, (unsigned)(kl * PB) * (unsigned)a.lds + (unsigned)(iz * PB), a.lds, tid);
-        const float4 qv = ld_sc1(bI, (unsigned)(kl * PB * PB) + tid * 4);
-        const unsigned long long neg7 = ld_sign_sc1(a.Lsign + kl);
-#pragma unroll
-        for (int ps = 0; ps < 16; ps++)
-            hq[ps] = __builtin_bit_cast(float, __builtin_amdgcn_raw_buffer_load_b32(bS, ((unsigned)(kl * PB + wave + 4 * ps) * (unsigned)a.lds + (unsigned)(mb * PB) + sqc) * 4u, 0, 16));
-        products(mb - 2, neg6, false);
-        __syncthreads();
-        ql.put(Tl, tid);
-        qi.put(Ti, tid);
-        if (zi) identity_tile(Tj, tid);
-        else qj.put(Tj, tid);
-        inv_put(qv, Tinv, tid);
-#pragma unroll
-        for (int ps = 0; ps < 16; ps++) Th[(wave + 4 * ps) * PLD + lane] = (sq >= 0) ? hq[ps] : 0.f;
-        __syncthreads();
-        float* const t3[3] = {Ti, Tj, Th};
-        tri_solve_fwd_n<3>(t3, Tl, Tinv, wave, lane);
-        __syncthreads();
-        products(kl, neg7, true);
-    }
+}
+template <bool INTILE>
+__device__ __forceinline__ void gain_tile2_finish(const PersistArgs& a, const GatherArgs& ga, float (&kv)[16], const float (&w2)[16], float* part, const float* tab,
+                                                  int ib, int cb, int m, int tid) {
+    const int lane = tid & 63, wave = tid >> 6, wr = wave & 1, wc = wave >> 1;
+    const int r = wr * 32 + (lane & 31);
 #pragma unroll
     for (int q = 0; q < 16; q++) kv[q] = (fabsf(kv[q]) > EKF_FLUSH_THRESH) ? kv[q] : 0.f;
     float* Kt = a.K + (size_t)(cb * PB) * a.ldk + (size_t)ib * PB;
     float* Gt = ga.G + (size_t)(cb * PB) * ga.ld + (size_t)ib * PB;
+    float* Wz = a.W + (size_t)(cb * PB) * a.ldw + (size_t)ib * PB;
     float acc = 0.f;
 #pragma unroll
     for (int q = 0; q < 16; q++) {
@@ -426,25 +285,106 @@
         if (cg < m) {
             const float x = kv[q] * tab[64 + c], y = kv[q ^ 1] * tab[128 + c];
             const float kr = ((cg ^ 1) < cg) ? (y + x) : (x + y);
-            g = kr - w2[q];
+            g = INTILE ? kr - w2[q] : kr;
             acc = acc + kv[q] * tab[c];
+        } else if (!INTILE) {
+            Wz[(size_t)c * a.ldw + r] = 0.f;
         }
         Gt[(size_t)c * ga.ld + r] = g;
     }
     __syncthreads();
-    float* part = Th;
     part[(wc * 2 + (lane >> 5)) * 64 + r] = acc;
     __syncthreads();
     if (tid < 64) ga.Wt[(size_t)cb * ga.ld + (size_t)ib * PB + tid] = ((part[tid] + part[64 + tid]) + part[128 + tid]) + part[192 + tid];
 }
 
 template <bool WAIT>
-__device__ __forceinline__ void t2_tile(const PersistArgs& a, float* Ti, float* Tj, float* Tl, float* Tinv, int ta, int tb, int tid, long long* dbg = nullptr) {
+__device__ __forceinline__ void gain_tile2(const PersistArgs& a, const GatherArgs& ga, float* Ti, float* Tj, float* Tl, float* Tinv, float* part, float* tab,
+                                           int ib, int cb, int tid) {
+    const int lane = tid & 63, wave = tid >> 6, wr = wave & 1, wc = wave >> 1;
+    const int mb = a.mb, ldl = a.ldl;
+    const int m = ga.m_dev ? *ga.m_dev : ga.m;
+    const __amdgpu_buffer_rsrc_t bL = persist_rsrc(a.L, (unsigned)ldl * (unsigned)(mb * PB));
+    const int iy = mb + ib, iz = a.idb0 + cb;
+    gain_tile2_tab(ga, tab, cb, m, tid);
+    float kv[16];
+#pragma unroll
+    for (int q = 0; q < 16; q++) kv[q] = 0.f;
+    auto product = [&](int kb, unsigned long long neg, bool z_unsigned) {
+        const f32x16 up = (z_unsigned && neg != 0ull) ? mma64_signed(Ti, 1, PLD, Tj, 1, PLD, wr, wc, lane, neg) : mma64(Ti, 1, PLD, Tj, 1, PLD, wr, wc, lane);
+#pragma unroll
+        for (int q = 0; q < 16; q++) kv[q] = kv[q] + up[q];
+        if (WAIT && a.dbg && tid == 0 && mb <= 8 && (ib == 0 || ib == 6) && (cb == 0 || cb == 3 || cb == 7))
+            a.dbg[100 + 8 * ((ib ? 3 : 0) + (cb == 0 ? 0 : cb == 3 ? 1 : 2)) + kb] = (long long)__builtin_amdgcn_s_memrealtime();
+    };
+    if constexpr (WAIT) {
+        for (int kb = cb; kb < mb - 2; kb++) {
+            __syncthreads();
+            persist_wait(a, nullptr, a.pan + iy * mb + kb, a.pan + iz * mb + kb, tid, 1, true);
+            load_tile_sc1(Ti, bL, (unsigned)(kb * PB) * (unsigned)ldl + (unsigned)(iy * PB), ldl, tid);
+            load_tile_sc1(Tj, bL, (unsigned)(kb * PB) * (unsigned)ldl + (unsigned)(iz * PB), ldl, tid);
+            __syncthreads();
+            product(kb, 0ull, false);
+        }
+        if (cb > mb - 3) persist_wait(a, nullptr, a.pan + iy * mb + (mb - 3), nullptr, tid, 1, true);
+    } else {
+        for (int kb = cb; kb < mb; kb++) {
+            __syncthreads();
+            load_tile(Ti, a.L + (size_t)kb * PB * ldl + (size_t)iy * PB, ldl, tid);
+            load_tile(Tj, a.L + (size_t)kb * PB * ldl + (size_t)iz * PB, ldl, tid);
+            __syncthreads();
+            product(kb, 0ull, false);
+        }
+    }
+    if constexpr (WAIT) {
+        const int kl = mb - 1, k6 = mb - 2;
+        const bool gk6 = k6 >= cb;
+        const __amdgpu_buffer_rsrc_t bS = persist_rsrc(a.S, (unsigned)a.lds * (unsigned)(mb * PB));
+        const __amdgpu_buffer_rsrc_t bI = persist_rsrc(a.Linv, (unsigned)(mb * PB * PB));
+        const bool zi = a.grid.compact() && cb == kl;
+        __syncthreads();
+        RegTile ql, qi, qj;
+        if (gk6) {
+            persist_wait(a, nullptr, a.pan + iy * mb + k6, a.pan + iz * mb + k6, tid, 1, false);
+            RegTile pi6, pj6;
+            pi6.request(bL, (unsigned)(k6 * PB) * (unsigned)ldl + (unsigned)(iy * PB), ldl, tid);
+            pj6.request(bL, (unsigned)(k6 * PB) * (unsigned)ldl + (unsigned)(iz * PB), ldl, tid);
+            pi6.put(Ti, tid);
+            pj6.put(Tj, tid);
+        }
+        persist_wait(a, a.ready + kl, gk6 ? nullptr : a.fin + iy * mb + kl, (gk6 || zi) ? nullptr : a.fin + iz * mb + kl, tid, 4, false);
+        ql.request(bL, (unsigned)(kl * PB) * (unsigned)ldl + (unsigned)(kl * PB), ldl, tid);
+        qi.request(bS, (unsigned)(kl * PB) * (unsigned)a.lds + (unsigned)(iy * PB), a.lds, tid);
+        if (!zi) qj.request(bS, (unsigned)(kl * PB) * (unsigned)a.lds + (unsigned)(iz * PB), a.lds, tid);
+        const float4 qv = ld_sc1(bI, (unsigned)(kl * PB * PB) + tid * 4);
+        const unsigned long long neg7 = ld_sign_sc1(a.Lsign + kl);
+        if (gk6) product(k6, 0ull, false);
+        __syncthreads();
+        ql.put(Tl, tid);
+        qi.put(Ti, tid);
+        if (zi) identity_tile(Tj, tid);
+        else qj.put(Tj, tid);
+        inv_put(qv, Tinv, tid);
+        __syncthreads();
+        tri_solve_fwd2(Ti, Tj, Tl, Tinv, wave, lane);
+        __syncthreads();
+        product(kl, neg7, true);
+    }
+    const float no_w2[16] = {};
+    gain_tile2_finish<false>(a, ga, kv, no_w2, part, tab, ib, cb, m, tid);
+}
+
+#include "chol_persist_w2_intile.inc"
+
+template <bool WAIT>
+__device__ __forceinline__ void t2_tile(const PersistArgs& a, float* Ti, float* Tj, float* Tl, float* Tinv, int* qtab, int ta, int tb, int tid, long long* dbg = nullptr) {
     const int lane = tid & 63, wave = tid >> 6, wr = wave & 1, wc = wave >> 1;
     const int r = wr * 32 + (lane & 31);
     const int mb = a.mb, ldl = a.ldl;
     const bool diag = ta == tb;
     const __amdgpu_buffer_rsrc_t bL = persist_rsrc(a.L, (unsigned)ldl * (unsigned)(mb * PB));
+    const int qs = (tid < PB ? ta : tb) * PB + (tid & (PB - 1));
+    int qrow = a.w2_in_tile ? -1 : a.inv_idx[min(qs, a.nstate - 1)];
     float tab[16], tba[16];
     {
         const float* sab = a.Sg + (size_t)tb * PB * a.ldsg + (size_t)ta * PB;
@@ -456,6 +396,7 @@
             tba[q] = diag ? 0.f : sba[(size_t)c * a.ldsg + r];
         }
     }
+    if (!a.w2_in_tile && tid < 2 * PB) qtab[tid] = (qs < a.nstate) ? qrow : -1;
     const int ia = mb + ta, ib = mb + tb;
     auto apply = [&](int kb, unsigned long long neg) {
         const float* Bj = diag ? Ti : Tj;
@@ -541,6 +482,20 @@
     __syncthreads();
     store_tile(Ti, a.T2 + (size_t)tb * PB * a.ldt + (size_t)ta * PB, a.ldt, tid);
     if (!diag) store_tile(Tj, a.T2 + (size_t)ta * PB * a.ldt + (size_t)tb * PB, a.ldt, tid);
+    if (!a.w2_in_tile) {
+        const int c4 = (tid & 15) * 4;
+#pragma unroll
+        for (int it = 0; it < 4; it++) {
+            const int rr = (tid >> 4) + 16 * it;
+            const int qa = qtab[rr], qb = diag ? -1 : qtab[PB + rr];
+            if (qa >= 0)
+                *reinterpret_cast<float4*>(a.W + (size_t)qa * a.ldw + tb * PB + c4) =
+                    make_float4(Ti[c4 * PLD + rr], Ti[(c4 + 1) * PLD + rr], Ti[(c4 + 2) * PLD + rr], Ti[(c4 + 3) * PLD + rr]);
+            if (qb >= 0)
+                *reinterpret_cast<float4*>(a.W + (size_t)qb * a.ldw + ta * PB + c4) =
+                    make_float4(Tj[c4 * PLD + rr], Tj[(c4 + 1) * PLD + rr], Tj[(c4 + 2) * PLD + rr], Tj[(c4 + 3) * PLD + rr]);
+        }
+    }
     if (dbg && tid == 0) dbg[15] = (long long)__builtin_amdgcn_s_memrealtime();
 }
 
@@ -900,7 +855,10 @@
             const int tb = role.n;
             __syncthreads();
             if (role.a < a.idb0 - mb) {
-                if (a.t2) gain_tile2<true>(a, ga, Ti, Tj, Tl, Tinv, persist_dyn_lds, persist_dyn_lds + PB * PLD, role.a, role.b, tid);
+                if (a.t2) {
+                    if (a.w2_in_tile) gain_tile2_intile<true>(a, ga, Ti, Tj, Tl, Tinv, persist_dyn_lds, persist_dyn_lds + PB * PLD, role.a, role.b, tid);
+                    else gain_tile2<true>(a, ga, Ti, Tj, Tl, Tinv, persist_dyn_lds, persist_dyn_lds + PB * PLD, role.a, role.b, tid);
+                }
                 else gain_tile(a, Ti, Tj, Tl, Tinv, role.a, role.b, tid);
                 if (a.dbg && tid == 0 && tb < 104) a.dbg[200 + tb] = (long long)__builtin_amdgcn_s_memrealtime();
             }
@@ -1049,7 +1007,7 @@
                 td = a.dbg + 840 + 16 * (p == 0 ? 0 : p == np_ - 1 ? 2 : 1);
                 if (tid == 0) td[14] = (long long)__builtin_amdgcn_s_memrealtime();
             }
-            t2_tile<true>(a, Ti, Tj, Tl, Tinv, ta, tb, tid, td);
+            t2_tile<true>(a, Ti, Tj, Tl, Tinv, reinterpret_cast<int*>(persist_dyn_lds), ta, tb, tid, td);
             if (a.dbg && tid == 0 && p < 91) a.dbg[304 + p] = (long long)__builtin_amdgcn_s_memrealtime();
         }
         PEXIT();
@@ -1142,10 +1100,11 @@
     __shared__ __attribute__((aligned(16))) float Th[PB * PLD];
     __shared__ float tab[192];
     if ((int)blockIdx.x < gain_wgs) {
-        gain_tile2<false>(a, ga, Ti, Tj, nullptr, nullptr, Th, tab, (int)blockIdx.x / a.mb, (int)blockIdx.x % a.mb, threadIdx.x);
+        if (a.w2_in_tile) gain_tile2_intile<false>(a, ga, Ti, Tj, nullptr, nullptr, Th, tab, (int)blockIdx.x / a.mb, (int)blockIdx.x % a.mb, threadIdx.x);
+        else gain_tile2<false>(a, ga, Ti, Tj, nullptr, nullptr, Th, tab, (int)blockIdx.x / a.mb, (int)blockIdx.x % a.mb, threadIdx.x);
     } else {
         int ta, tb;
         t2_pair((int)blockIdx.x - gain_wgs, ta, tb);
-        t2_tile<false>(a, Ti, Tj, Th, nullptr, ta, tb, threadIdx.x);
-    }
-}
+        t2_tile<false>(a, Ti, Tj, Th, nullptr, reinterpret_cast<int*>(tab), ta, tb, threadIdx.x);
+    }
+}
diff --git a/ekf_vio_amd/csrc/chol_persist_w2_intile.inc b/ekf_vio_amd/csrc/chol_persist_w2_intile.inc
--- /dev/null
+++ b/ekf_vio_amd/csrc/chol_persist_w2_intile.inc
@@ -0,0 +1,158 @@
+template <bool WAIT>
+__device__ __forceinline__ void gain_tile2_intile(const PersistArgs& a, const GatherArgs& ga, float* Ti, float* Tj, float* Tl, float* Tinv, float* Th, float* tab,
+                                           int ib, int cb, int tid) {
+    const int lane = tid & 63, wave = tid >> 6, wr = wave & 1, wc = wave >> 1;
+    const int r = wr * 32 + (lane & 31);
+    const int mb = a.mb, ldl = a.ldl;
+    const int m = ga.m_dev ? *ga.m_dev : ga.m;
+    const __amdgpu_buffer_rsrc_t bL = persist_rsrc(a.L, (unsigned)ldl * (unsigned)(mb * PB));
+    const __amdgpu_buffer_rsrc_t bS = persist_rsrc(a.S, (unsigned)a.lds * (unsigned)(mb * PB));
+    const int iy = mb + ib, iz = a.idb0 + cb;
+    const int cq = cb * PB + lane;
+    const int sq = (cq < m) ? ga.idx[cq] : -1;
+    const unsigned sqc = (unsigned)max(sq, 0);
+    int alo = 0, ahi = -1;
+    if (cb * PB < m) {
+        alo = ga.idx[cb * PB] / PB;
+        ahi = ga.idx[min(cb * PB + PB - 1, m - 1)] / PB;
+    }
+    gain_tile2_tab(ga, tab, cb, m, tid);
+    auto column_flags = [&](int kb, const int* zflag) -> PollLane {
+        const int ax = alo + tid - 2;
+        return {tid == 0 ? a.pan + iy * mb + kb : tid == 1 ? zflag : (tid >= 2 && ax <= ahi) ? a.pan + (mb + ax) * mb + kb : nullptr, 1};
+    };
+    float kv[16], w2[16];
+    {
+        float wv[16];
+        const int scl = max(sq, 0);
+#pragma unroll
+        for (int ps = 0; ps < 16; ps++) wv[ps] = ga.P[(size_t)min(ib * PB + wave + 4 * ps, ga.n - 1) * ga.ld + scl];
+#pragma unroll
+        for (int ps = 0; ps < 16; ps++) asm volatile("" : "+v"(wv[ps]));
+#pragma unroll
+        for (int ps = 0; ps < 16; ps++) Th[(wave + 4 * ps) * 65 + lane] = (sq >= 0 && ib * PB + wave + 4 * ps < ga.n) ? wv[ps] : 0.f;
+        __syncthreads();
+#pragma unroll
+        for (int q = 0; q < 16; q++) {
+            kv[q] = 0.f;
+            w2[q] = Th[r * 65 + mma64_col(wc, lane, q)];
+        }
+    }
+    auto fetch = [&](int kb) -> unsigned long long {
+        const bool gk = kb >= cb;
+        float hv[16];
+        unsigned long long neg;
+        if constexpr (WAIT) {
+            persist_wait(a, column_flags(kb, gk ? a.pan + iz * mb + kb : nullptr), tid, kb < mb - 2);
+            load_tile_sc1(Ti, bL, (unsigned)(kb * PB) * (unsigned)ldl + (unsigned)(iy * PB), ldl, tid);
+            if (gk) load_tile_sc1(Tj, bL, (unsigned)(kb * PB) * (unsigned)ldl + (unsigned)(iz * PB), ldl, tid);
+#pragma unroll
+            for (int ps = 0; ps < 16; ps++)
+                hv[ps] = __builtin_bit_cast(float, __builtin_amdgcn_raw_buffer_load_b32(bL, ((unsigned)(kb * PB + wave + 4 * ps) * (unsigned)ldl + (unsigned)(mb * PB) + sqc) * 4u, 0, 16));
+#pragma unroll
+            for (int ps = 0; ps < 16; ps++) hv[ps] = (sq >= 0) ? hv[ps] : 0.f;
+#pragma unroll
+            for (int ps = 0; ps < 16; ps++) Th[(wave + 4 * ps) * PLD + lane] = hv[ps];
+            neg = ld_sign_sc1(a.Lsign + kb);
+        } else {
+            load_tile(Ti, a.L + (size_t)kb * PB * ldl + (size_t)iy * PB, ldl, tid);
+            if (gk) load_tile(Tj, a.L + (size_t)kb * PB * ldl + (size_t)iz * PB, ldl, tid);
+#pragma unroll
+            for (int ps = 0; ps < 16; ps++) hv[ps] = a.L[(size_t)(kb * PB + wave + 4 * ps) * ldl + (size_t)(mb * PB) + sqc];
+#pragma unroll
+            for (int ps = 0; ps < 16; ps++) hv[ps] = (sq >= 0) ? hv[ps] : 0.f;
+#pragma unroll
+            for (int ps = 0; ps < 16; ps++) Th[(wave + 4 * ps) * PLD + lane] = hv[ps];
+            neg = a.Lsign[kb];
+        }
+        return neg;
+    };
+    auto products = [&](int kb, unsigned long long neg, bool z_unsigned) {
+        if (kb >= cb) {
+            const f32x16 up = (z_unsigned && neg != 0ull) ? mma64_signed(Ti, 1, PLD, Tj, 1, PLD, wr, wc, lane, neg) : mma64(Ti, 1, PLD, Tj, 1, PLD, wr, wc, lane);
+#pragma unroll
+            for (int q = 0; q < 16; q++) kv[q] = kv[q] + up[q];
+        }
+        if (alo <= ahi) {
+            f32x16 up;
+            if constexpr (WAIT) {
+                up = (neg == 0ull) ? mma64(Ti, 1, PLD, Th, 1, PLD, wr, wc, lane) : mma64_signed(Ti, 1, PLD, Th, 1, PLD, wr, wc, lane, neg);
+            } else {
+                if (__builtin_amdgcn_readfirstlane((int)(neg != 0ull))) {
+                    __syncthreads();
+                    sign_cols(Ti, Ti, neg, tid);
+                    __syncthreads();
+                }
+                up = mma64(Ti, 1, PLD, Th, 1, PLD, wr, wc, lane);
+            }
+#pragma unroll
+            for (int q = 0; q < 16; q++) w2[q] = w2[q] - up[q];
+        }
+        if (WAIT && a.dbg && tid == 0 && mb <= 8 && (ib == 0 || ib == 6) && (cb == 0 || cb == 3 || cb == 7))
+            a.dbg[100 + 8 * ((ib ? 3 : 0) + (cb == 0 ? 0 : cb == 3 ? 1 : 2)) + kb] = (long long)__builtin_amdgcn_s_memrealtime();
+    };
+    if constexpr (WAIT) {
+        for (int kb = 0; kb < mb - 2; kb++) {
+            __syncthreads();
+            const unsigned long long neg = fetch(kb);
+            __syncthreads();
+            products(kb, neg, false);
+        }
+    } else {
+        for (int kb = 0; kb < mb; kb++) {
+            __syncthreads();
+            const unsigned long long neg = fetch(kb);
+            __syncthreads();
+            products(kb, neg, false);
+        }
+    }
+    if constexpr (WAIT) {
+        const int kl = mb - 1, k6 = mb - 2;
+        const bool gk6 = k6 >= cb;
+        const __amdgpu_buffer_rsrc_t bI = persist_rsrc(a.Linv, (unsigned)(mb * PB * PB));
+        const bool zi = a.grid.compact() && cb == kl;
+        __syncthreads();
+        persist_wait(a, column_flags(k6, gk6 ? a.pan + iz * mb + k6 : (zi ? nullptr : a.fin + iz * mb + kl)), tid, false);
+        RegTile ql, qi, qj;
+        float hq[16];
+        unsigned long long neg6;
+        {
+            RegTile pi6, pj6;
+            float h6[16];
+            pi6.request(bL, (unsigned)(k6 * PB) * (unsigned)ldl + (unsigned)(iy * PB), ldl, tid);
+            if (gk6) pj6.request(bL, (unsigned)(k6 * PB) * (unsigned)ldl + (unsigned)(iz * PB), ldl, tid);
+#pragma unroll
+            for (int ps = 0; ps < 16; ps++)
+                h6[ps] = __builtin_bit_cast(float, __builtin_amdgcn_raw_buffer_load_b32(bL, ((unsigned)(k6 * PB + wave + 4 * ps) * (unsigned)ldl + (unsigned)(mb * PB) + sqc) * 4u, 0, 16));
+            neg6 = ld_sign_sc1(a.Lsign + k6);
+            pi6.put(Ti, tid);
+            if (gk6) pj6.put(Tj, tid);
+#pragma unroll
+            for (int ps = 0; ps < 16; ps++) Th[(wave + 4 * ps) * PLD + lane] = (sq >= 0) ? h6[ps] : 0.f;
+        }
+        persist_wait(a, a.ready + kl, nullptr, nullptr, tid, 4, false);
+        ql.request(bL, (unsigned)(kl * PB) * (unsigned)ldl + (unsigned)(kl * PB), ldl, tid);
+        qi.request(bS, (unsigned)(kl * PB) * (unsigned)a.lds + (unsigned)(iy * PB), a.lds, tid);
+        if (!zi) qj.request(bS, (unsigned)(kl * PB) * (unsigned)a.lds + (unsigned)(iz * PB), a.lds, tid);
+        const float4 qv = ld_sc1(bI, (unsigned)(kl * PB * PB) + tid * 4);
+        const unsigned long long neg7 = ld_sign_sc1(a.Lsign + kl);
+#pragma unroll
+        for (int ps = 0; ps < 16; ps++)
+            hq[ps] = __builtin_bit_cast(float, __builtin_amdgcn_raw_buffer_load_b32(bS, ((unsigned)(kl * PB + wave + 4 * ps) * (unsigned)a.lds + (unsigned)(mb * PB) + sqc) * 4u, 0, 16));
+        products(mb - 2, neg6, false);
+        __syncthreads();
+        ql.put(Tl, tid);
+        qi.put(Ti, tid);
+        if (zi) identity_tile(Tj, tid);
+        else qj.put(Tj, tid);
+        inv_put(qv, Tinv, tid);
+#pragma unroll
+        for (int ps = 0; ps < 16; ps++) Th[(wave + 4 * ps) * PLD + lane] = (sq >= 0) ? hq[ps] : 0.f;
+        __syncthreads();
+        float* const t3[3] = {Ti, Tj, Th};
+        tri_solve_fwd_n<3>(t3, Tl, Tinv, wave, lane);
+        __syncthreads();
+        products(kl, neg7, true);
+    }
+    gain_tile2_finish<true>(a, ga, kv, w2, Th, tab, ib, cb, m, tid);
+}
diff --git a/ekf_vio_amd/csrc/common.h b/ekf_vio_amd/csrc/common.h
--- a/ekf_vio_amd/csrc/common.h
+++ b/ekf_vio_amd/csrc/common.h
@@ -120,6 +120,7 @@
     int sweep_stall_wg = -1;
 #ifdef EKFVIO_TEST_HOOKS
     int sweep_delay_wg = -1, sweep_delay_point = 0, sweep_delay_ticks = 0;
+    int w2_force = -1;
 #endif
     bool sweep_retry_armed = false;
     double sweep_retry_pause_s = 0.0;
@@ -140,6 +141,7 @@
     float* Km = nullptr;
     float* Wt = nullptr;
     float* Gm = nullptr;
+    float* Wm = nullptr;
     int* info = nullptr;
     float gate_chi2 = 0.f;
     float* gate_d2 = nullptr;
@@ -255,6 +257,8 @@
     float* C = nullptr;
     int lda = 0, ldb = 0, ldcin = 0, ldc = 0;
     GemmEpi epi;
+    const float* W = nullptr;
+    int ldw = 0;
     int variant = 0;
 };
 inline GemmShape gemm_shape(const GemmCall& c) {
@@ -352,7 +356,11 @@
     return s;
 }
 inline UpdatePlan plan_update(const ekfvio_filter* f, int m, bool m_on_device = false, float next_dt = -1.f, bool recoverable = true) {
-    return plan_update(f->tune, plan_shape(f), m, m_on_device, next_dt, recoverable);
+    UpdatePlan p = plan_update(f->tune, plan_shape(f), m, m_on_device, next_dt, recoverable);
+#ifdef EKFVIO_TEST_HOOKS
+    if (f->w2_force >= 0 && p.tail == TAIL_T2 && p.w_on_load_ok) p.w_on_load = f->w2_force == 0;
+#endif
+    return p;
 }
 int launch_update_gemms_scratch(ekfvio_filter* f, const UpdatePlan& p, int reps, double* last_flops);
 const int* launch_chol_sweep(ekfvio_filter* f, const UpdatePlan& p, float* Saug, float* Laug, float* Linv, int ld, bool zero_flags);
diff --git a/ekf_vio_amd/csrc/ekf_kernels.hip b/ekf_vio_amd/csrc/ekf_kernels.hip
--- a/ekf_vio_amd/csrc/ekf_kernels.hip
+++ b/ekf_vio_amd/csrc/ekf_kernels.hip
@@ -703,6 +703,7 @@
         t.count = 1;
         GemmCall& g = t.g[0];
         g.A = f->Km, g.B = f->Gm, g.flush = true, g.epi.mode = EPI_MEAN;
+        if (p.tail == TAIL_T2 && p.w_on_load) g.W = f->Wm, g.ldw = ld;
         return t;
     }
     t.count = 2;
@@ -785,6 +786,7 @@
 
 int launch_update_gemms_scratch(ekfvio_filter* f, const UpdatePlan& p, int reps, double* last_flops) {
     TailGemms tail = update_tail_gemms(f, p, f->P, f->P2);
+    if (tail.last().W) tail.last().epi.mode = EPI_MEAN_PARTIAL;
     for (int r = 0; r < reps; r++)
         for (int k = 0; k < tail.count; k++) launch_gemm(f, tail.g[k]);
     const GemmShape sh = gemm_shape(tail.last());
diff --git a/ekf_vio_amd/csrc/gemm.hip b/ekf_vio_amd/csrc/gemm.hip
--- a/ekf_vio_amd/csrc/gemm.hip
+++ b/ekf_vio_amd/csrc/gemm.hip
@@ -409,11 +409,11 @@
     for (int e = threadIdx.x; e < epi.n_zero; e += 256) epi.zero_words[e] = 0;
 }
 
-template <int BMt, int WPS, int EPI>
+template <int BMt, int WPS, int EPI, bool WSUB = false>
 __global__ __launch_bounds__(256 * WPS) void gemm16_kernel(int M, int N, int K, float alpha, const float* __restrict__ A, int lda,
                                                      const float* __restrict__ B, int ldb, float beta, const float* Cin,
                                                      int ldcin, float* C, int ldc, int flush, int lowerB, GemmEpi epi,
-                                                     int tiles_x, int tiles_y) {
+                                                     int tiles_x, int tiles_y, const float* __restrict__ W, int ldw) {
     constexpr int RB = BMt / 16;
     constexpr int SA = (BMt % 32 == 16) ? BMt : BMt + 16;
     constexpr int SB = 80;
@@ -499,6 +499,10 @@
     const int a_step = BKK * lda * 4, b_step = BKK * ldb * 4, b_rows = BKS * ldb * 4;
     const int a_base = kbeg * lda * 4, b_base = kbeg * ldb * 4;
     static_assert((BV == 4 || BV == 2) && AV >= 1 && AV <= 4, "staging is written for 1..4 float4 of A and 2 or 4 of B per thread");
+    static_assert(!WSUB || (EPI == 3 && AV + 2 * BV <= NS), "the on-load subtraction: one more load per B piece, one load per k-step");
+    const __amdgpu_buffer_rsrc_t rsW = __builtin_amdgcn_make_buffer_rsrc(const_cast<float*>(WSUB ? W : B), 0, WSUB ? K * ldw * 4 : 0, 0x00020000);
+    const int wo = WSUB ? ((tid >> 4) * ldw + j0 + (tid & 15) * 4) * 4 : 0;
+    const int w_step = WSUB ? BKK * ldw * 4 : 0, w_rows = WSUB ? BKS * ldw * 4 : 0, w_base = WSUB ? kbeg * ldw * 4 : 0;
 
     f32x4 acc[RB];
 #pragma unroll
@@ -534,6 +538,10 @@
     }
     float4 Xa0, Xa1, Xa2, Xa3, Xb0, Xb1, Xb2, Xb3, Ya0, Ya1, Ya2, Ya3, Yb0, Yb1, Yb2, Yb3;
     float4 Za0, Za1, Za2, Za3, Zb0, Zb1, Zb2, Zb3;
+    float4 Xw0, Xw1, Xw2, Xw3, Yw0, Yw1, Yw2, Yw3, Zw0, Zw1, Zw2, Zw3;
+    Xw0 = Xw1 = Xw2 = Xw3 = Yw0 = Yw1 = Yw2 = Yw3 = Zw0 = Zw1 = Zw2 = Zw3 = make_float4(0.f, 0.f, 0.f, 0.f);
+#define G16_LDW(r) __builtin_bit_cast(float4, __builtin_amdgcn_raw_buffer_load_b128(rsW, wo + (r) * w_rows, sw_, 0))
+#define G16_BW(S, r) (WSUB ? make_float4(S##b##r.x - S##w##r.x, S##b##r.y - S##w##r.y, S##b##r.z - S##w##r.z, S##b##r.w - S##w##r.w) : S##b##r)
     Xa0 = Xa1 = Xa2 = Xa3 = Xb0 = Xb1 = Xb2 = Xb3 = make_float4(0.f, 0.f, 0.f, 0.f);
     Ya0 = Ya1 = Ya2 = Ya3 = Yb0 = Yb1 = Yb2 = Yb3 = make_float4(0.f, 0.f, 0.f, 0.f);
     Za0 = Za1 = Za2 = Za3 = Zb0 = Zb1 = Zb2 = Zb3 = make_float4(0.f, 0.f, 0.f, 0.f);
@@ -548,6 +556,13 @@
         S##b1 = __builtin_bit_cast(float4, __builtin_amdgcn_raw_buffer_load_b128(rsB, bo + b_rows, sb_, 0));                                                       \
         if constexpr (BV > 2) S##b2 = __builtin_bit_cast(float4, __builtin_amdgcn_raw_buffer_load_b128(rsB, bo + 2 * b_rows, sb_, 0));                             \
         if constexpr (BV > 2) S##b3 = __builtin_bit_cast(float4, __builtin_amdgcn_raw_buffer_load_b128(rsB, bo + 3 * b_rows, sb_, 0));                             \
+        if constexpr (WSUB) {                                                                          \
+            const int sw_ = w_base + (kt) * w_step;                                                    \
+            S##w0 = G16_LDW(0);                                                                        \
+            S##w1 = G16_LDW(1);                                                                        \
+            if constexpr (BV > 2) S##w2 = G16_LDW(2);                                                  \
+            if constexpr (BV > 2) S##w3 = G16_LDW(3);                                                  \
+        }                                                                                              \
     } while (0)
 #define G16_LOADI(S, j, kt)                                                                            \
     do {                                                                                               \
@@ -560,6 +575,13 @@
         if ((j) == AV + 1) S##b1 = __builtin_bit_cast(float4, __builtin_amdgcn_raw_buffer_load_b128(rsB, bo + b_rows, sb_, 0));                                    \
         if ((j) == AV + 2 && BV > 2) S##b2 = __builtin_bit_cast(float4, __builtin_amdgcn_raw_buffer_load_b128(rsB, bo + 2 * b_rows, sb_, 0));                      \
         if ((j) == AV + 3 && BV > 2) S##b3 = __builtin_bit_cast(float4, __builtin_amdgcn_raw_buffer_load_b128(rsB, bo + 3 * b_rows, sb_, 0));                      \
+        if constexpr (WSUB) {                                                                          \
+            const int sw_ = w_base + (kt) * w_step;                                                    \
+            if ((j) == AV + BV) S##w0 = G16_LDW(0);                                                    \
+            if ((j) == AV + BV + 1) S##w1 = G16_LDW(1);                                                \
+            if ((j) == AV + BV + 2 && BV > 2) S##w2 = G16_LDW(2);                                      \
+            if ((j) == AV + BV + 3 && BV > 2) S##w3 = G16_LDW(3);                                      \
+        }                                                                                              \
     } while (0)
 #define G16_STAGEI(S, j, buf)                                                                          \
     do {                                                                                               \
@@ -567,10 +589,10 @@
         if ((j) == 1 && AV > 1) *reinterpret_cast<float4*>(&As[buf][al1]) = S##a1;                     \
         if ((j) == 2 && AV > 2) *reinterpret_cast<float4*>(&As[buf][al2]) = S##a2;                     \
         if ((j) == 3 && AV > 3) *reinterpret_cast<float4*>(&As[buf][al3]) = S##a3;                     \
-        if ((j) == AV) *reinterpret_cast<float4*>(&Bs[buf][bl]) = S##b0;                               \
-        if ((j) == AV + 1) *reinterpret_cast<float4*>(&Bs[buf][bl + BKS * SB]) = S##b1;                \
-        if ((j) == AV + 2 && BV > 2) *reinterpret_cast<float4*>(&Bs[buf][bl + 2 * BKS * SB]) = S##b2;  \
-        if ((j) == AV + 3 && BV > 2) *reinterpret_cast<float4*>(&Bs[buf][bl + 3 * BKS * SB]) = S##b3;  \
+        if ((j) == AV) *reinterpret_cast<float4*>(&Bs[buf][bl]) = G16_BW(S, 0);                        \
+        if ((j) == AV + 1) *reinterpret_cast<float4*>(&Bs[buf][bl + BKS * SB]) = G16_BW(S, 1);         \
+        if ((j) == AV + 2 && BV > 2) *reinterpret_cast<float4*>(&Bs[buf][bl + 2 * BKS * SB]) = G16_BW(S, 2);  \
+        if ((j) == AV + 3 && BV > 2) *reinterpret_cast<float4*>(&Bs[buf][bl + 3 * BKS * SB]) = G16_BW(S, 3);  \
     } while (0)
 #define G16_STAGE_A(S, buf)                                                                            \
     do {                                                                                               \
@@ -581,10 +603,10 @@
     } while (0)
 #define G16_STAGE_B(S, buf)                                                                            \
     do {                                                                                               \
-        *reinterpret_cast<float4*>(&Bs[buf][bl]) = S##b0;                                              \
-        *reinterpret_cast<float4*>(&Bs[buf][bl + BKS * SB]) = S##b1;                                   \
-        if constexpr (BV > 2) *reinterpret_cast<float4*>(&Bs[buf][bl + 2 * BKS * SB]) = S##b2;         \
-        if constexpr (BV > 2) *reinterpret_cast<float4*>(&Bs[buf][bl + 3 * BKS * SB]) = S##b3;         \
+        *reinterpret_cast<float4*>(&Bs[buf][bl]) = G16_BW(S, 0);                                       \
+        *reinterpret_cast<float4*>(&Bs[buf][bl + BKS * SB]) = G16_BW(S, 1);                            \
+        if constexpr (BV > 2) *reinterpret_cast<float4*>(&Bs[buf][bl + 2 * BKS * SB]) = G16_BW(S, 2);  \
+        if constexpr (BV > 2) *reinterpret_cast<float4*>(&Bs[buf][bl + 3 * BKS * SB]) = G16_BW(S, 3);  \
     } while (0)
 #define G16_MFMA(c, b, a) c = __builtin_amdgcn_mfma_f32_16x16x4f32(b, a, c, 0, 0, 0)
 #ifndef G16X_NOLOAD
@@ -670,6 +692,8 @@
 #undef G16_STAGEI
 #undef G16_STAGE_A
 #undef G16_STAGE_B
+#undef G16_LDW
+#undef G16_BW
     if constexpr (WPS > 1) {
         float* red = &As[0][0];
         static_assert(3 * BKK * SA >= RB * 4 * 256, "reduction scratch");
@@ -741,18 +765,23 @@
     e.lin_blocks = p.lin_blocks, e.mean_keep = p.mean_keep;
     const dim3 grid(p.grid_x, p.grid_y), block(p.threads());
     const int flush = c.flush, lowerB = c.lowerB;
+    if (c.W && !(p.k16 && e.mode == EPI_MEAN_PARTIAL)) {
+        fprintf(stderr, "launch_gemm: the on-load subtraction (GemmCall::W) exists in gemm16_kernel's EPI_MEAN_PARTIAL form only\n");
+        abort();
+    }
     if (p.k16) {
-#define GEMM16_GO(BMv, W, EP)                                                                                                     \
-    hipLaunchKernelGGL((gemm16_kernel<BMv, W, EP>), grid, block, 0, s, M, N, K, c.alpha, c.A, c.lda, c.B, c.ldb, c.beta, c.Cin, c.ldcin, \
-                       c.C, c.ldc, flush, lowerB, e, p.tiles_x, p.tiles_y)
-#define GEMM16_BM(W, EP)                            \
-    do {                                            \
-        if (p.bm == 32) GEMM16_GO(32, W, EP);       \
-        else if (p.bm == 48) GEMM16_GO(48, W, EP);  \
-        else GEMM16_GO(64, W, EP);                  \
+#define GEMM16_GO(BMv, WP, EP, ...)                                                                                                \
+    hipLaunchKernelGGL((gemm16_kernel<BMv, WP, EP, ##__VA_ARGS__>), grid, block, 0, s, M, N, K, c.alpha, c.A, c.lda, c.B, c.ldb, c.beta, c.Cin, c.ldcin, \
+                       c.C, c.ldc, flush, lowerB, e, p.tiles_x, p.tiles_y, c.W, c.ldw)
+#define GEMM16_BM(WP, EP, ...)                                      \
+    do {                                                           \
+        if (p.bm == 32) GEMM16_GO(32, WP, EP, ##__VA_ARGS__);       \
+        else if (p.bm == 48) GEMM16_GO(48, WP, EP, ##__VA_ARGS__);  \
+        else GEMM16_GO(64, WP, EP, ##__VA_ARGS__);                  \
     } while (0)
         if (e.mode == EPI_JOSEPH1) GEMM16_BM(2, 1);
         else if (e.mode == EPI_MEAN) GEMM16_BM(2, 2);
+        else if (e.mode == EPI_MEAN_PARTIAL && c.W) GEMM16_BM(2, 3, true);
         else if (e.mode == EPI_MEAN_PARTIAL) GEMM16_BM(2, 3);
         else if (p.wps == 2) GEMM16_BM(2, 0);
         else GEMM16_BM(1, 0);
diff --git a/ekf_vio_amd/csrc/plan.h b/ekf_vio_amd/csrc/plan.h
--- a/ekf_vio_amd/csrc/plan.h
+++ b/ekf_vio_amd/csrc/plan.h
@@ -241,6 +241,8 @@
     UpdateTail tail = TAIL_NONE;
     int t2_skip = -1;
     bool t2_by_sweep = false, compact = false;
+    bool w_on_load = false;
+    bool w_on_load_ok = false;
     int lin_blocks = 0;
     bool persistent() const { return sweep == SWEEP_PERSIST_FUSED || sweep == SWEEP_PERSIST; }
 };
@@ -346,6 +348,12 @@
     g.M = g.N = n, g.K = m_pad, g.transB = true, g.epi = EPI_MEAN_PARTIAL, g.mean = true, g.lin_blocks = lin_blocks;
     return g;
 }
+inline int t2_late_pairs(const PersistGrid& g) {
+    int early = 0;
+    for (int j = 1; j + 1 < g.mb; j++) early += g.column_owners(j);
+    return std::max(0, t2_pairs(g.nX) - std::max(0, early - g.t2_skip));
+}
+#define T2_ON_LOAD_MAX_LATE_PAIRS 2
 inline UpdatePlan plan_update(const Tuning& t, const PlanShape& s, int m, bool m_on_device = false, float next_dt = -1.f, bool recoverable = true) {
     UpdatePlan p;
     if (m_on_device) m = 2 * s.N;
@@ -366,6 +374,8 @@
     p.tail = TAIL_T2;
     p.t2_by_sweep = p.compact = fused;
     p.gain = fused ? GAIN_SWEEP : GAIN2_T2_TILES;
+    p.w_on_load_ok = plan_gemm(t, s.num_cus, tail_gemm_shape(n, m_pad, 0)).k16;
+    p.w_on_load = p.w_on_load_ok && t2_late_pairs(PersistGrid{GRID_COMPACT, m_pad / EKF_TILE, n_pad / EKF_TILE, ld / 64, p.t2_skip}) <= T2_ON_LOAD_MAX_LATE_PAIRS;
     const int lin_blocks = (s.N + LIN_LM - 1) / LIN_LM + 1;
     if (next_dt >= 0.f && t.lin_overlap && !s.dense_predict && t.fuse_linearize)
         p.lin_blocks = plan_gemm(t, s.num_cus, tail_gemm_shape(n, m_pad, lin_blocks)).lin_blocks;
diff --git a/ekf_vio_amd/filter.py b/ekf_vio_amd/filter.py
--- a/ekf_vio_amd/filter.py
+++ b/ekf_vio_amd/filter.py
@@ -276,6 +276,10 @@
         self._need_hooks()
         self._chk(self.lib.ekfvio_test_sweep_delay(self.h, int(workgroup), int(point), int(ticks)))
 
+    def w2_in_tile(self, on):
+        self._need_hooks()
+        self._chk(self.lib.ekfvio_test_w2_in_tile(self.h, -1 if on is None else 1 if on else 0))
+
     def test_cholesky_solve(self, S, Crhs):
         self._need_hooks()
         S = np.asarray(S, np.float32)
diff --git a/include/ekfvio_test_hooks.h b/include/ekfvio_test_hooks.h
--- a/include/ekfvio_test_hooks.h
+++ b/include/ekfvio_test_hooks.h
@@ -16,6 +16,7 @@
 EKFVIO_API int ekfvio_test_sweep_fault(ekfvio_filter* f, int32_t spin_limit, int32_t stall_workgroup);
 #define EKFVIO_TEST_SWEEP_DELAY_MAX_TICKS 100000
 EKFVIO_API int ekfvio_test_sweep_delay(ekfvio_filter* f, int32_t workgroup, int32_t point, int32_t ticks);
+EKFVIO_API int ekfvio_test_w2_in_tile(ekfvio_filter* f, int32_t on);
 EKFVIO_API int ekfvio_test_cholesky_solve(ekfvio_filter* f, int32_t m, int32_t nrhs, const float* S, const float* Crhs,
                                float* L_out, float* X_out, int32_t* info);
 EKFVIO_API int ekfvio_test_plan(int32_t num_cus, int32_t max_features, int32_t N, int32_t m, int32_t m_on_device, int32_t sole_handle,
```

Result: faster. 11270, median of 6 (+2.1%).
